# stckvrflw/pem-spgemm

Hardware: AMD Instinct MI355X
Metric: SpGEMM GFLOP/s (2*flop / t(step1+step2+step3)) (higher is better)
Workload: dtype f64

## Files before the change

### include/pem_spgemm.h

```cpp
#ifndef PEM_SPGEMM_H
#define PEM_SPGEMM_H
#include <stdint.h>

#ifdef __cplusplus
extern "C" {
#endif

typedef int pem_status;
enum {
    PEM_OK = 0,
    PEM_E_INVALID = -1,
    PEM_E_DUPLICATE = -2,
    PEM_E_NOMEM = -3,
    PEM_E_OVERFLOW = -4,
    PEM_E_HIP = -5,
    PEM_E_STATE = -6,
    PEM_E_NODEVICE = -7,
    PEM_E_IO = -8,
    PEM_E_STALE = -9
};

typedef struct pem_ctx pem_ctx;
typedef struct pem_tiled pem_tiled;
typedef struct pem_cplan pem_cplan;
// ... 80 lines not shown

pem_status pem_cplan_create(pem_ctx *ctx, const pem_tiled *A, const pem_tiled *B,
                            int32_t tile_row_begin, int32_t tile_row_end, pem_cplan **out);
pem_status pem_cplan_destroy(pem_ctx *ctx, pem_cplan *plan);

typedef enum { PEM_MASK_STRUCTURE = 0, PEM_MASK_COMPLEMENT = 1 } pem_mask_flags;
pem_status pem_cplan_create_masked(pem_ctx *ctx, const pem_tiled *A, const pem_tiled *B, const pem_tiled *M, int mask_flags,
                                   int32_t tile_row_begin, int32_t tile_row_end, pem_cplan **out);

typedef enum {
    PEM_SEMIRING_PLUS_TIMES = 0,
    PEM_SEMIRING_MIN_PLUS = 1,
    PEM_SEMIRING_MAX_PLUS = 2,
    PEM_SEMIRING_MAX_TIMES = 3,
    PEM_SEMIRING_PLUS_PAIR = 4,
    PEM_SEMIRING_LOR_LAND = 5
} pem_semiring;
pem_status pem_cplan_set_semiring(pem_cplan *plan, int semiring);
pem_status pem_cplan_get_semiring(const pem_cplan *plan, int *semiring);

pem_status pem_tiled_from_cplan(pem_ctx *ctx, const pem_cplan *plan, int transpose, pem_tiled **out);
pem_status pem_tiled_set_values_from_cplan(pem_ctx *ctx, pem_tiled *t, const pem_cplan *plan);

typedef enum { PEM_EWISE_UNION = 0, PEM_EWISE_INTERSECT = 1 } pem_ewise_pattern;
typedef enum {
    PEM_BINOP_PLUS = 0,
    PEM_BINOP_TIMES = 1,
    PEM_BINOP_MIN = 2,
    PEM_BINOP_MAX = 3,
    PEM_BINOP_LOR = 4,
    PEM_BINOP_LAND = 5
} pem_binop;
pem_status pem_tiled_ewise(pem_ctx *ctx, const pem_tiled *A, const pem_tiled *B, int pattern, int op, double alpha, double beta,
                           pem_tiled **out);
pem_status pem_tiled_set_values_from_ewise(pem_ctx *ctx, pem_tiled *t, const pem_tiled *A, const pem_tiled *B);

typedef enum {
    PEM_SELECT_TRIL = 0,
    PEM_SELECT_TRIU = 1,
    PEM_SELECT_DIAG = 2,
    PEM_SELECT_OFFDIAG = 3,
    PEM_SELECT_ROW_LE = 4,
    PEM_SELECT_ROW_GT = 5,
    PEM_SELECT_COL_LE = 6,
    PEM_SELECT_COL_GT = 7,
    PEM_SELECT_VALUE_EQ = 8, PEM_SELECT_VALUE_NE = 9, PEM_SELECT_VALUE_LT = 10,
    PEM_SELECT_VALUE_LE = 11, PEM_SELECT_VALUE_GT = 12, PEM_SELECT_VALUE_GE = 13,
    PEM_SELECT_ABS_GT = 14
} pem_select_op;
pem_status pem_tiled_select(pem_ctx *ctx, const pem_tiled *A, int op, double thunk, pem_tiled **out);
pem_status pem_tiled_set_values_from_select(pem_ctx *ctx, pem_tiled *t, const pem_tiled *A);

typedef enum { PEM_REDUCE_ROWS = 0, PEM_REDUCE_COLS = 1 } pem_reduce_dim;
pem_status pem_tiled_mxv(pem_ctx *ctx, const pem_tiled *A, int semiring, int transpose, const double *dx, double *dy, int accumulate);
pem_status pem_tiled_mxv_f32(pem_ctx *ctx, const pem_tiled *A, int semiring, int transpose, const float *dx, float *dy, int accumulate);
pem_status pem_tiled_reduce(pem_ctx *ctx, const pem_tiled *A, int op, int dim, double *dy, int accumulate);
pem_status pem_tiled_reduce_f32(pem_ctx *ctx, const pem_tiled *A, int op, int dim, float *dy, int accumulate);

pem_status pem_tiled_spmm(pem_ctx *ctx, const pem_tiled *A, int semiring, int transpose, int64_t k, const double *dX, int64_t ldx,
                          double *dY, int64_t ldy, int accumulate);
pem_status pem_tiled_spmm_f32(pem_ctx *ctx, const pem_tiled *A, int semiring, int transpose, int64_t k, const float *dX, int64_t ldx,
                              float *dY, int64_t ldy, int accumulate);

pem_status pem_tiled_set_values_sddmm(pem_ctx *ctx, pem_tiled *t, int semiring, int64_t k, const double *dX, int64_t ldx, const double *dY,
                                      int64_t ldy, int accumulate);
pem_status pem_tiled_set_values_sddmm_f32(pem_ctx *ctx, pem_tiled *t, int semiring, int64_t k, const float *dX, int64_t ldx, const float *dY,
                                          int64_t ldy, int accumulate);
pem_status pem_tiled_sddmm(pem_ctx *ctx, const pem_tiled *S, int semiring, int64_t k, const double *dX, int64_t ldx, const double *dY,
                           int64_t ldy, pem_tiled **out);
pem_status pem_tiled_sddmm_f32(pem_ctx *ctx, const pem_tiled *S, int semiring, int64_t k, const float *dX, int64_t ldx, const float *dY,
                               int64_t ldy, pem_tiled **out);

pem_status pem_tiled_export_csr(pem_ctx *ctx, const pem_tiled *t, int64_t *nnz, int32_t *rowptr, int32_t *colidx, double *vals);
pem_status pem_tiled_export_csr_f32(pem_ctx *ctx, const pem_tiled *t, int64_t *nnz, int32_t *rowptr, int32_t *colidx, float *vals);

typedef enum {
    PEM_OPT_PRUNE = 0,
    PEM_OPT_STEP1_GLOBAL_SORT = 1,
    PEM_OPT_WIDE = 2,
    PEM_OPT_WARM = 3,
    PEM_OPT_S3_BAND = 4,
    PEM_OPT_EXPORT_ROWS = 7,
    PEM_OPT__TEST_FIRST = 5,
    PEM_OPT__LAST = 18
} pem_option;
pem_status pem_cplan_set_option(pem_cplan *plan, pem_option which, int64_t value);
pem_status pem_cplan_get_option(const pem_cplan *plan, pem_option which, int64_t *value);

pem_status pem_spgemm_step1(pem_ctx *ctx, pem_cplan *plan);
pem_status pem_spgemm_step2(pem_ctx *ctx, pem_cplan *plan);
pem_status pem_spgemm_step3(pem_ctx *ctx, pem_cplan *plan);
pem_status pem_spgemm(pem_ctx *ctx, pem_cplan *plan);

typedef struct {
    int32_t tile_row_begin, tile_row_end;
    int32_t row_begin, row_end;
    int64_t ntiles_c;
    int64_t npairs;
    int64_t nnz_c;
    int64_t npairs_all;
} pem_cplan_info;
pem_status pem_cplan_get_info(const pem_cplan *plan, pem_cplan_info *info);

typedef enum {
    PEM_C_TILE_ROWPTR = 0,
    PEM_C_TILE_ROWIDX,
    PEM_C_TILE_COLIDX,
    PEM_C_PAIRS_OFFSET,
    PEM_C_PAIRS_A,
    PEM_C_PAIRS_B,
    PEM_C_MASK,
    PEM_C_TILE_NNZ_PTR,
    PEM_C_ROWPTR,
    PEM_C_ROWCOLIDX,
    PEM_C_VALS
} pem_cplan_array;
pem_status pem_cplan_get_array(pem_ctx *ctx, const pem_cplan *plan, pem_cplan_array which, void *host_dst, int64_t bytes);

pem_status pem_set_graph_replay(pem_ctx *ctx, int on);

pem_status pem_c_export_csr(pem_ctx *ctx, const pem_cplan *plan, int64_t *nnz, int32_t *rowptr,
                            int32_t *colidx, double *vals);
pem_status pem_c_export_csr_device(pem_ctx *ctx, const pem_cplan *plan, int32_t *d_rowptr,
                                   int32_t *d_colidx, double *d_vals);
pem_status pem_c_export_coo(pem_ctx *ctx, const pem_cplan *plan, int64_t *nnz, int32_t *rows,
                            int32_t *cols, double *vals);
pem_status pem_c_export_csr_f32(pem_ctx *ctx, const pem_cplan *plan, int64_t *nnz, int32_t *rowptr,
                                int32_t *colidx, float *vals);
pem_status pem_c_export_csr_device_f32(pem_ctx *ctx, const pem_cplan *plan, int32_t *d_rowptr,
                                       int32_t *d_colidx, float *d_vals);
pem_status pem_c_export_coo_f32(pem_ctx *ctx, const pem_cplan *plan, int64_t *nnz, int32_t *rows,
                                int32_t *cols, float *vals);

pem_status pem_split_tile_rows(pem_ctx *ctx, const pem_tiled *A, const pem_tiled *B, int nparts, int32_t *bounds);
pem_status pem_tile_row_weights(pem_ctx *ctx, const pem_tiled *A, const pem_tiled *B, double *weights);

typedef struct {
    double step1_ms, step2_ms, step3_ms;
    double spgemm_wall_ms;
    double export_ms;
} pem_timings;
pem_status pem_get_timings(pem_ctx *ctx, pem_timings *t);

pem_status pem_set_kernel_profiling(pem_ctx *ctx, int enabled);
pem_status pem_reset_kernel_stats(pem_ctx *ctx);
pem_status pem_kernel_stats_count(pem_ctx *ctx, int *n);
pem_status pem_kernel_stats_get(pem_ctx *ctx, int idx, char *name, int name_cap, int64_t *calls, double *total_ms);

#ifdef __cplusplus
}
#endif
#endif
```

### pem-spgemm_amd/__init__.py

```python
import ctypes as C
import os
import subprocess

import numpy as np

_HERE = os.path.dirname(os.path.abspath(__file__))
LIB_PATH = os.path.join(_HERE, "libpemspgemm_hip.so")

PEM_OK = 0
STATUS_NAMES = {0: "PEM_OK", -1: "PEM_E_INVALID", -2: "PEM_E_DUPLICATE", -3: "PEM_E_NOMEM", -4: "PEM_E_OVERFLOW",
                -5: "PEM_E_HIP", -6: "PEM_E_STATE", -7: "PEM_E_NODEVICE", -8: "PEM_E_IO", -9: "PEM_E_STALE"}

T_ARRAYS = dict(tile_keys=(0, np.int64), tile_nnz_ptr=(1, np.int32), masks=(2, np.uint16), rowptr=(3, np.uint8),
                rowcolidx=(4, np.uint8), vals=(5, np.float64), masks_t=(6, np.uint16), tile_rowptr=(7, np.int32),
                tile_colidx=(8, np.int32), tile_colptr=(9, np.int32), tile_rowidx=(10, np.int32), tile_offsets=(11, np.int32))
C_ARRAYS = dict(c_tile_rowptr=(0, np.int32), c_tile_rowidx=(1, np.int32), c_tile_colidx=(2, np.int32), pairs_offset=(3, np.int32),
                pairs_a=(4, np.int32), pairs_b=(5, np.int32), c_mask=(6, np.uint32), c_tile_nnz_ptr=(7, np.int32),
                c_rowptr=(8, np.uint8), c_rowcolidx=(9, np.uint8), c_vals=(10, np.float64))
C_TEST_ARRAYS = dict(c_mtile=(11, np.int32))

MASK_STRUCTURE, MASK_COMPLEMENT = 0, 1

SEMIRINGS = dict(plus_times=0, min_plus=1, max_plus=2, max_times=3, plus_pair=4, lor_land=5)

ABI_SYMBOLS = [
    "pem_last_error", "pem_version", "pem_ctx_create", "pem_ctx_create_on_stream", "pem_ctx_destroy", "pem_ctx_synchronize",
    "pem_tiled_from_coo", "pem_tiled_from_coo_device", "pem_tiled_from_csr", "pem_tiled_destroy", "pem_tiled_get_info",
    "pem_tiled_get_array", "pem_flop_count", "pem_cplan_create", "pem_cplan_destroy", "pem_spgemm_step1", "pem_spgemm_step2",
    "pem_spgemm_step3", "pem_spgemm", "pem_cplan_get_info", "pem_cplan_get_array", "pem_c_export_csr", "pem_c_export_csr_device",
    "pem_c_export_coo", "pem_split_tile_rows", "pem_tile_row_weights", "pem_get_timings", "pem_set_kernel_profiling", "pem_reset_kernel_stats",
    "pem_kernel_stats_count", "pem_kernel_stats_get", "pem_tiled_save", "pem_tiled_load",
    "pem_tiled_from_coo_f32", "pem_tiled_from_coo_device_f32", "pem_tiled_from_csr_f32", "pem_c_export_csr_f32",
    "pem_c_export_csr_device_f32", "pem_c_export_coo_f32", "pem_set_graph_replay",
    "pem_ctx_reserve", "pem_ctx_trim", "pem_ctx_memory_stats", "pem_cplan_set_option", "pem_cplan_get_option", "pem_debug_scan_i32",
    "pem_debug_refused_launch", "pem_tiled_set_values", "pem_tiled_set_values_device", "pem_tiled_set_values_f32",
    "pem_tiled_set_values_device_f32", "pem_cplan_create_masked", "pem_cplan_set_semiring", "pem_cplan_get_semiring",
    "pem_tiled_from_cplan", "pem_tiled_set_values_from_cplan", "pem_tiled_ewise", "pem_tiled_set_values_from_ewise",
    "pem_tiled_export_csr", "pem_tiled_export_csr_f32", "pem_tiled_select", "pem_tiled_set_values_from_select",
    "pem_tiled_mxv", "pem_tiled_mxv_f32", "pem_tiled_reduce", "pem_tiled_reduce_f32", "pem_tiled_spmm", "pem_tiled_spmm_f32",
    "pem_tiled_set_values_sddmm", "pem_tiled_set_values_sddmm_f32", "pem_tiled_sddmm", "pem_tiled_sddmm_f32",
]

EWISE_PATTERNS = dict(union=0, intersect=1)
BINOPS = dict(plus=0, times=1, min=2, max=3, lor=4, land=5)

SELECT_OPS = ("tril", "triu", "diag", "offdiag", "row_le", "row_gt", "col_le", "col_gt", "value_eq", "value_ne", "value_lt", "value_le",
              "value_gt", "value_ge", "abs_gt")
POSITIONAL_SELECT_OPS = SELECT_OPS[:8]

REDUCE_DIMS = dict(rows=0, cols=1)

VALUE_ORDERS = dict(row=0, col=1)

OPTIONS = dict(prune=0, step1_global_sort=1, wide=2, warm=3, s3_band=4, s1_force_key64=5, s1_xlcap=6, export_rows=7, s1_serial=8, s3_decode=9, s1_xl_global=10, s3_epw=11, s3_idx64=12, s3_mark=13, s3_xcd=14, s1_segments=15, s2_transposed=16, s3_poison=17)


class PemError(RuntimeError):
    def __init__(self, status, msg):
        super().__init__(f"{STATUS_NAMES.get(status, status)}: {msg}")
        self.status = status


class TiledInfo(C.Structure):
    _fields_ = [("rows", C.c_int32), ("cols", C.c_int32), ("nnz", C.c_int64), ("tile_rows", C.c_int32), ("tile_cols", C.c_int32),
                ("ntiles", C.c_int64), ("conv_ms", C.c_double), ("conv_tile_kernel_ms", C.c_double), ("value_bytes", C.c_int32),
                ("reserved", C.c_int32)]


class CPlanInfo(C.Structure):
    _fields_ = [("tile_row_begin", C.c_int32), ("tile_row_end", C.c_int32), ("row_begin", C.c_int32), ("row_end", C.c_int32),
                ("ntiles_c", C.c_int64), ("npairs", C.c_int64), ("nnz_c", C.c_int64), ("npairs_all", C.c_int64)]


class CacheKey(C.Structure):
    _fields_ = [("source_size", C.c_uint64), ("source_mtime_ns", C.c_int64), ("transpose", C.c_uint32), ("reserved", C.c_uint32)]

    @classmethod
    def of_file(cls, path, transpose=False):
        st = os.stat(path)
        return cls(st.st_size, st.st_mtime_ns, int(bool(transpose)), 0)


class MemoryStats(C.Structure):
    _fields_ = [("slab_bytes", C.c_int64), ("in_use_bytes", C.c_int64), ("peak_in_use_bytes", C.c_int64), ("largest_free_bytes", C.c_int64),
                ("driver_allocs", C.c_int64), ("block_allocs", C.c_int64)]


class Timings(C.Structure):
    _fields_ = [("step1_ms", C.c_double), ("step2_ms", C.c_double), ("step3_ms", C.c_double), ("spgemm_wall_ms", C.c_double),
                ("export_ms", C.c_double)]


def build(verbose=False):
    out = None if verbose else subprocess.DEVNULL
    subprocess.check_call(["make", "-C", os.path.join(_HERE, "csrc"), "-j4"], stdout=out)
    return LIB_PATH


_lib = None


def lib():
    global _lib
    if _lib is None:
        if not os.path.exists(LIB_PATH):
            raise ImportError(f"{LIB_PATH} is missing: run `python -c 'import __graft_entry__ as g; g.build()'` "
                              "(the product path has no CPU fallback)")
        L = C.CDLL(LIB_PATH)
        L.pem_last_error.restype = C.c_char_p
        L.pem_version.restype = C.c_char_p
        _lib = L
    return _lib


def _check(status):
    if status != PEM_OK:
        raise PemError(status, lib().pem_last_error().decode(errors="replace"))


def _p(a, ctype):
    return a.ctypes.data_as(C.POINTER(ctype))


class Context:

    def __init__(self, device=0, stream=None):
        self._h = C.c_void_p()
        _check(lib().pem_ctx_create_on_stream(int(device), C.c_void_p(stream or 0), C.byref(self._h)))
        self.device = device

    def synchronize(self):
        _check(lib().pem_ctx_synchronize(self._h))

    def timings(self):
        t = Timings()
        _check(lib().pem_get_timings(self._h, C.byref(t)))
        return {k: getattr(t, k) for k, _ in Timings._fields_}
# ... 406 lines not shown
```

### pem-spgemm_amd/csrc/pem_internal.h

```cpp
#pragma once
#include <hip/hip_runtime.h>
#include <atomic>
#include <cstdint>
#include <cstdio>
#include <cstring>
#include <initializer_list>
#include <map>
#include <memory>
#include <mutex>
#include <string>
#include <vector>
#include "../../include/pem_spgemm.h"
#include "../../include/pem_test.h"

namespace pem {

void set_error(const char *fmt, ...);

#define PEM_HIP(expr)                                                                          \
    do {                                                                                       \
        hipError_t _e = (expr);                                                                \
        if (_e != hipSuccess) {                                                                \
            pem::set_error("%s:%d: %s -> %s", __FILE__, __LINE__, #expr, hipGetErrorString(_e)); \
            return PEM_E_HIP;                                                                  \
// ... 243 lines not shown
    std::vector<int> h_tile_rowptr;
    pem::DevBuf vmap[2];
    pem::DevBuf vmap_t;
    bool vmap_ready[2] = {false, false}, vmap_t_ready = false;
    uint64_t value_version = 0;
    uint64_t serial = pem::next_tiled_serial();
    pem::Derivation derived;
    mutable pem::DevBuf mx_csc_off, mx_csc_base, mx_rci_t;
    mutable bool mx_cols_ready = false;
};

struct pem_cplan {
    const pem_tiled *A = nullptr, *B = nullptr;
    uint64_t serial = 0;
    const pem_tiled *M = nullptr;
    int mask_complement = 0;
    pem::DevBuf c_mtile;
    pem::DevBuf mf_tile_off, mf_tile_mt, mf_keep_t, mf_keep_p;
    pem::DevBuf mf_pair_col, mf_pairs_a, mf_pairs_b, mf_blk_heads;
    bool mf_swapped = false;
    int64_t w_Pm = 0, w_TCm = 0;
    int tr_lo = 0, tr_hi = 0;
    int a_lo = 0, a_hi = 0;
    int max_row_tiles = 0;
    int state = 0;
    int opt_prune = 1, opt_key64 = 0, opt_xlcap = 0;
    int opt_band = 1;
    int opt_step1_esc = 0, opt_wide = 1, opt_warm = 1, opt_export_rows = 0, opt_s1_serial = 0;
    int opt_xl_global = 0;
    int opt_idx64 = 0;
    int opt_mark = 1;
    int opt_s3_xcd = 1;
    int opt_epw = 0;
    int opt_decode = 1;
    int opt_s3_poison = 0;
    int64_t ntiles_c = 0, npairs = 0, nnz_c = 0;
    pem::DevBuf c_tile_rowptr, c_tile_colidx;
    mutable pem::DevBuf c_tile_rowidx;
    mutable bool c_rowidx_valid = false;
    pem::DevBuf pairs_offset, pairs_a, pairs_b;
    pem::DevBuf c_mask, c_tile_nnz_ptr, c_vals;
    mutable pem::DevBuf c_rowcolidx;
    mutable bool c_rowcolidx_valid = false;
    pem::DevBuf c_tile_cnt;
    bool s3_decode = false;
    pem::DevBuf s3_chunk_tile;
    mutable pem::DevBuf c_rowptr;
    mutable bool c_rowptr_valid = false;
    pem::DevBuf prod_a, prod_b, aprod_off;
    pem::DevBuf lprod_off;
    pem::DevBuf row_lbase;
    pem::DevBuf live_j, live_ab;
    pem::DevBuf aseg;
    pem::DevBuf chunk_seg, chunk_n;
    pem::DevBuf row_desc;
    int64_t w_ntotal = 0;
    int64_t npairs_all = 0;
    pem::DevBuf sk0, sk1, sv0, sv1;
    uint32_t *sorted_perm = nullptr;
    pem::DevBuf row_list, bin_count, xl_base, xl_rowstart;
    pem::DevBuf pair_col;
    pem::DevBuf blk_heads;
    bool pairs_ready = false;
    bool flags_mirrored = false;
    bool verify_folded = false;
    bool group_nnz_cleared = false;
    bool wide = true;
    bool compact_valid = false;
    pem::DevBuf group_nnz;
    uint64_t a_version = 0, b_version = 0;
    int semiring = 0;
    int c_semiring = 0;
    pem_ctx *owner = nullptr;
    hipGraphExec_t graph_exec = nullptr;
    unsigned long long graph_gen = 0;
    bool graph_failed = false;
    bool warm = false, warm_pass = false;
    int64_t w_P = 0, w_Pall = 0, w_TC = 0, w_nnz = 0;
    int w_counts[5] = {0, 0, 0, 0, 0};
    int w_nsegs = 0;
    pem::DevBuf seg_list;
    int opt_s2_transposed = 2;
    int opt_s1_segments = 0;
    int64_t w_nxl = 0;
    int w_nrows_xl = 0, w_max_xl = 0;
};
```

### pem-spgemm_amd/csrc/primitives.hip

```cpp
#include "pem_internal.h"
#include <algorithm>
#include <cstdarg>

namespace pem {

static thread_local char g_err[512] = "";
void set_error(const char *fmt, ...)
{
    va_list ap;
    va_start(ap, fmt);
    vsnprintf(g_err, sizeof g_err, fmt, ap);
    va_end(ap);
}
const char *last_error() { return g_err; }

std::shared_ptr<Arena> &current_arena()
{
    static thread_local std::shared_ptr<Arena> a;
    return a;
}

static constexpr size_t ARENA_ALIGN = 256;
static constexpr size_t ARENA_MIN_SLAB = size_t(64) << 20;
static constexpr size_t ARENA_MAX_GROWTH = size_t(4) << 30;

Arena::~Arena()
{
    (void)hipSetDevice(device);
    (void)hipDeviceSynchronize();
    for (auto &s : slabs) (void)hipFree(s.base);
}

pem_status Arena::add_slab(size_t bytes)
{
    void *p = nullptr;
    hipError_t e = hipMalloc(&p, bytes);
    if (e != hipSuccess) {
        (void)hipGetLastError();
        set_error("hipMalloc(%zu bytes) failed: %s (arena holds %zu bytes, %zu in use)", bytes, hipGetErrorString(e), slab_bytes, in_use);
        return PEM_E_NOMEM;
    }
    slabs.push_back(Slab{static_cast<char *>(p), bytes});
    slab_bytes += bytes;
    ++n_driver;
    free_blocks[static_cast<char *>(p)] = bytes;
    return PEM_OK;
}

void *Arena::take(size_t bytes)
{
    auto best = free_blocks.end();
    for (auto it = free_blocks.begin(); it != free_blocks.end(); ++it)
        if (it->second >= bytes && (best == free_blocks.end() || it->second < best->second)) best = it;
    if (best == free_blocks.end()) return nullptr;
    char *p = best->first;
    const size_t have = best->second;
    free_blocks.erase(best);
    if (have > bytes) free_blocks[p + bytes] = have - bytes;
    used_blocks[p] = bytes;
    in_use += bytes;
    if (in_use > peak) peak = in_use;
    ++n_block;
    return p;
}

void *Arena::alloc(size_t bytes)
{
    bytes = (bytes + ARENA_ALIGN - 1) & ~(ARENA_ALIGN - 1);
    if (bytes == 0) bytes = ARENA_ALIGN;
    std::lock_guard<std::mutex> lock(mu);
    if (void *p = take(bytes)) return p;
    size_t pad = slab_bytes / 2;
    if (pad > ARENA_MAX_GROWTH) pad = ARENA_MAX_GROWTH;
    size_t want = bytes + pad;
    if (want < ARENA_MIN_SLAB) want = ARENA_MIN_SLAB;
    if (add_slab(want) != PEM_OK) {
        if (want == bytes || add_slab(bytes) != PEM_OK) return nullptr;
    }
    return take(bytes);
}

void Arena::free(void *vp)
{
// ... 99 lines not shown
        ctx->event_pool.pop_back();
        return e;
    }
    hipEvent_t e = nullptr;
    (void)hipEventCreate(&e);
    return e;
}

KernelSpan::KernelSpan(pem_ctx *c, const char *name) : ctx(c)
{
    if (!ctx->profiling) return;
    for (size_t i = 0; i < ctx->stats.size(); ++i)
        if (ctx->stats[i].name == name) { stat = (int)i; break; }
    if (stat < 0) {
        ctx->stats.push_back(KernelStat{name, 0, 0.0});
        stat = (int)ctx->stats.size() - 1;
    }
    e0 = take_event(ctx);
    e1 = take_event(ctx);
    (void)hipEventRecord(e0, ctx->stream);
}
KernelSpan::~KernelSpan()
{
    if (stat < 0) return;
    (void)hipEventRecord(e1, ctx->stream);
    ctx->pending.push_back(PendingSpan{stat, e0, e1});
}

pem_status resolve_kernel_spans(pem_ctx *ctx)
{
    if (ctx->pending.empty()) return PEM_OK;
    PEM_HIP(hipStreamSynchronize(ctx->stream));
    for (auto &s : ctx->pending) {
        float ms = 0.f;
        if (hipEventElapsedTime(&ms, s.e0, s.e1) == hipSuccess) {
            ctx->stats[s.stat].calls += 1;
            ctx->stats[s.stat].total_ms += ms;
        }
        ctx->event_pool.push_back(s.e0);
        ctx->event_pool.push_back(s.e1);
    }
    ctx->pending.clear();
    return PEM_OK;
}

pem_status zero_flags(pem_ctx *ctx)
{
    PEM_HIP(hipMemsetAsync(ctx->d_flags, 0, sizeof(int) * NUM_FLAGS, ctx->stream));
    return PEM_OK;
}

pem_status launch_status(pem_ctx *ctx)
{
    if (ctx->launch_err == hipSuccess) return PEM_OK;
    set_error("kernel launch refused by the runtime: %s: %s", ctx->launch_name ? ctx->launch_name : "?", hipGetErrorString(ctx->launch_err));
    ctx->launch_err = hipSuccess;
    ctx->launch_name = nullptr;
    return PEM_E_HIP;
}

pem_status read_flags(pem_ctx *ctx, int *host_flags)
{
    PEM_TRY(launch_status(ctx));
    int *h = reinterpret_cast<int *>(ctx->h_scalars + 48);
    PEM_HIP(hipMemcpyAsync(h, ctx->d_flags, sizeof(int) * NUM_FLAGS, hipMemcpyDeviceToHost, ctx->stream));
    PEM_HIP(hipStreamSynchronize(ctx->stream));
    for (int i = 0; i < NUM_FLAGS; ++i) host_flags[i] = h[i];
    return PEM_OK;
}

pem_status read_scalars(pem_ctx *ctx, const int64_t *d_src, int count, int64_t *host_dst)
{
    PEM_HIP(hipMemcpyAsync(ctx->h_scalars, d_src, sizeof(int64_t) * count, hipMemcpyDeviceToHost, ctx->stream));
    PEM_HIP(hipStreamSynchronize(ctx->stream));
    for (int i = 0; i < count; ++i) host_dst[i] = ctx->h_scalars[i];
    return PEM_OK;
}

constexpr int SCAN_THREADS = 256;
constexpr int SCAN_TILE = SCAN_THREADS * 4;
constexpr int SCAN_TILES_PER_BLOCK = 8;
constexpr int SCAN_BLOCK_ITEMS = SCAN_TILE * SCAN_TILES_PER_BLOCK;

template <typename T> __device__ __forceinline__ T wave_inclusive_scan(T v)
{
    const int lane = threadIdx.x & 63;
#pragma unroll
    for (int d = 1; d < 64; d <<= 1) {
        T t = __shfl_up(v, d, 64);
        if (lane >= d) v += t;
    }
    return v;
}

template <typename T> __device__ __forceinline__ T wave_reduce_sum(T v)
{
#pragma unroll
    for (int d = 32; d > 0; d >>= 1) v += __shfl_xor(v, d, 64);
    return v;
}

__global__ void __launch_bounds__(SCAN_THREADS) scan_reduce_kernel(const int *__restrict__ in, size_t n,
                                                                   long long *__restrict__ bsum)
{
    __shared__ long long wsum[SCAN_THREADS / 64];
    size_t base = (size_t)blockIdx.x * SCAN_BLOCK_ITEMS;
    size_t end = base + SCAN_BLOCK_ITEMS < n ? base + SCAN_BLOCK_ITEMS : n;
    long long s = 0;
    if (end - base == (size_t)SCAN_BLOCK_ITEMS && (reinterpret_cast<uintptr_t>(in) & 15) == 0) {
        const int4 *in4 = reinterpret_cast<const int4 *>(in + base);
#pragma unroll
        for (int k = 0; k < SCAN_BLOCK_ITEMS / 4 / SCAN_THREADS; ++k) {
            const int4 q = in4[k * SCAN_THREADS + threadIdx.x];
            s += (long long)q.x + q.y + q.z + q.w;
        }
    } else {
        for (size_t i = base + threadIdx.x; i < end; i += SCAN_THREADS) s += in[i];
    }
    s = wave_reduce_sum(s);
    if ((threadIdx.x & 63) == 0) wsum[threadIdx.x >> 6] = s;
    __syncthreads();
    if (threadIdx.x == 0) {
        long long t = 0;
        for (int w = 0; w < SCAN_THREADS / 64; ++w) t += wsum[w];
        bsum[blockIdx.x] = t;
    }
}

__global__ void __launch_bounds__(1024) scan_bsums_kernel(long long *__restrict__ bsum, int nblk,
                                                          long long *__restrict__ total64, int *__restrict__ flags)
{
    __shared__ long long wsum[16];
    __shared__ long long carry_s;
    if (threadIdx.x == 0) carry_s = 0;
    __syncthreads();
    for (int base = 0; base < nblk; base += 1024) {
        int i = base + threadIdx.x;
        long long v = i < nblk ? bsum[i] : 0;
        long long inc = wave_inclusive_scan(v);
        if ((threadIdx.x & 63) == 63) wsum[threadIdx.x >> 6] = inc;
        __syncthreads();
        long long woff = 0;
        for (int w = 0; w < (int)(threadIdx.x >> 6); ++w) woff += wsum[w];
        long long carry = carry_s;
        if (i < nblk) bsum[i] = carry + woff + inc - v;
        __syncthreads();
        if (threadIdx.x == 1023) carry_s = carry + woff + inc;
        __syncthreads();
    }
    if (threadIdx.x == 0) {
        long long t = carry_s;
        bsum[nblk] = t;
        if (total64) *total64 = t;
        if (t > 0x7FFFFFFFLL) flags[FLAG_OVERFLOW] = 1;
    }
}

__global__ void __launch_bounds__(SCAN_THREADS) scan_apply_kernel(const int *in, int *out, size_t n,
                                                                  const long long *__restrict__ bsum, int nblk)
{
    __shared__ int wsum[SCAN_THREADS / 64];
    const int lane = threadIdx.x & 63, wave = threadIdx.x >> 6;
    long long carry = bsum[blockIdx.x];
    size_t base = (size_t)blockIdx.x * SCAN_BLOCK_ITEMS;
    for (int tile = 0; tile < SCAN_TILES_PER_BLOCK; ++tile, base += SCAN_TILE) {
        if (base >= n) break;
        size_t i0 = base + (size_t)threadIdx.x * 4;
        int v[4];
        if (i0 + 4 <= n) {
            int4 q = *reinterpret_cast<const int4 *>(in + i0);
            v[0] = q.x; v[1] = q.y; v[2] = q.z; v[3] = q.w;
        } else {
#pragma unroll
            for (int k = 0; k < 4; ++k) v[k] = (i0 + k < n) ? in[i0 + k] : 0;
        }
        int tsum = v[0] + v[1] + v[2] + v[3];
        int inc = wave_inclusive_scan(tsum);
        if (lane == 63) wsum[wave] = inc;
        __syncthreads();
        int woff = 0, btotal = 0;
#pragma unroll
        for (int w = 0; w < SCAN_THREADS / 64; ++w) {
            int s = wsum[w];
            if (w < wave) woff += s;
            btotal += s;
        }
        int ex = (int)carry + woff + inc - tsum;
        int o0 = ex, o1 = o0 + v[0], o2 = o1 + v[1], o3 = o2 + v[2];
        if (i0 + 4 <= n) {
            *reinterpret_cast<int4 *>(out + i0) = make_int4(o0, o1, o2, o3);
        } else {
            if (i0 < n) out[i0] = o0;
            if (i0 + 1 < n) out[i0 + 1] = o1;
            if (i0 + 2 < n) out[i0 + 2] = o2;
        }
        carry += btotal;
        __syncthreads();
    }
    if (blockIdx.x == nblk - 1 && threadIdx.x == 0) out[n] = (int)bsum[nblk];
}

__global__ void scan_empty_kernel(int *out, long long *total64)
{
    out[0] = 0;
    if (total64) *total64 = 0;
}

__global__ void __launch_bounds__(1024) scan_small_kernel(const int *in, int *out, size_t n, long long *__restrict__ total64,
                                                          int *__restrict__ flags)
{
    __shared__ long long wsum[16];
    const int lane = threadIdx.x & 63, wave = threadIdx.x >> 6;
    long long carry = 0;
    for (size_t base = 0; base < n; base += 8192) {
        const size_t i0 = base + (size_t)threadIdx.x * 8;
        int v[8];
        if (i0 + 8 <= n) {
            const int4 q0 = *reinterpret_cast<const int4 *>(in + i0), q1 = *reinterpret_cast<const int4 *>(in + i0 + 4);
            v[0] = q0.x; v[1] = q0.y; v[2] = q0.z; v[3] = q0.w;
            v[4] = q1.x; v[5] = q1.y; v[6] = q1.z; v[7] = q1.w;
        } else {
#pragma unroll
            for (int k = 0; k < 8; ++k) v[k] = (i0 + k < n) ? in[i0 + k] : 0;
        }
        long long tsum = 0;
#pragma unroll
        for (int k = 0; k < 8; ++k) tsum += v[k];
        const long long inc = wave_inclusive_scan(tsum);
        if (lane == 63) wsum[wave] = inc;
        __syncthreads();
        long long woff = 0, btotal = 0;
#pragma unroll
        for (int w = 0; w < 16; ++w) {
            const long long c = wsum[w];
            if (w < wave) woff += c;
            btotal += c;
        }
        int o[8];
        o[0] = (int)(carry + woff + inc - tsum);
#pragma unroll
        for (int k = 1; k < 8; ++k) o[k] = o[k - 1] + v[k - 1];
        if (i0 + 8 <= n) {
            *reinterpret_cast<int4 *>(out + i0) = make_int4(o[0], o[1], o[2], o[3]);
            *reinterpret_cast<int4 *>(out + i0 + 4) = make_int4(o[4], o[5], o[6], o[7]);
        } else {
#pragma unroll
            for (int k = 0; k < 8; ++k)
                if (i0 + k < n) out[i0 + k] = o[k];
        }
        carry += btotal;
        __syncthreads();
    }
    if (threadIdx.x == 0) {
        out[n] = (int)carry;
        if (total64) *total64 = carry;
        if (carry > 0x7FFFFFFFLL) flags[FLAG_OVERFLOW] = 1;
    }
}

constexpr int SCAN_MID_ITEMS = 2048, SCAN_MID_BLOCKS = 128;
constexpr unsigned long long SCAN_MID_VALID = 1ull << 63;

struct ScanMidArgs {
    const int *in[2];
    int *out[2];
    size_t n[2];
    long long *total64[2];
    int nblk[2];
};
__global__ void __launch_bounds__(256) scan_mid_kernel(ScanMidArgs args, unsigned long long *state_all, int *__restrict__ flags, int stall_ticket)
{
    __shared__ long long wsum[4];
    __shared__ long long s_excl;
    __shared__ int s_ticket;
    const int y = blockIdx.y;
    const int nblk = args.nblk[y];
    if ((int)blockIdx.x >= nblk) return;
    const int *in = args.in[y];
    int *out = args.out[y];
    const size_t n = args.n[y];
    long long *total64 = args.total64[y];
    unsigned long long *state = state_all + (size_t)y * (SCAN_MID_BLOCKS + 2);
    int *ctl = reinterpret_cast<int *>(state + SCAN_MID_BLOCKS);
    const int tid = threadIdx.x, lane = tid & 63, wave = tid >> 6;
    if (tid == 0) s_ticket = atomicAdd(&ctl[1], 1);
    __syncthreads();
    const int blk = s_ticket;
    const size_t i0 = (size_t)blk * SCAN_MID_ITEMS + (size_t)tid * 8;
    int v[8];
    if (i0 + 8 <= n) {
        const int4 q0 = *reinterpret_cast<const int4 *>(in + i0), q1 = *reinterpret_cast<const int4 *>(in + i0 + 4);
        v[0] = q0.x; v[1] = q0.y; v[2] = q0.z; v[3] = q0.w;
        v[4] = q1.x; v[5] = q1.y; v[6] = q1.z; v[7] = q1.w;
    } else {
#pragma unroll
        for (int k = 0; k < 8; ++k) v[k] = (i0 + k < n) ? in[i0 + k] : 0;
    }
    long long tsum = 0;
#pragma unroll
    for (int k = 0; k < 8; ++k) tsum += v[k];
    const long long inc = wave_inclusive_scan(tsum);
    if (lane == 63) wsum[wave] = inc;
    __syncthreads();
    long long woff = 0, btotal = 0;
#pragma unroll
    for (int w = 0; w < 4; ++w) {
        if (w < wave) woff += wsum[w];
        btotal += wsum[w];
    }
    if (wave == 0) {
        if (blk == stall_ticket)
            for (int k = 0; k < 50; ++k) __builtin_amdgcn_s_sleep(127);
        if (lane == 0) __hip_atomic_store(&state[blk], SCAN_MID_VALID | (unsigned long long)btotal, __ATOMIC_RELAXED, __HIP_MEMORY_SCOPE_AGENT);
        long long excl = 0;
        bool ok = false;
        for (long long polls = 0; polls < (1ll << 24) && !ok; ++polls) {
            const unsigned long long a = lane < blk ? __hip_atomic_load(&state[lane], __ATOMIC_RELAXED, __HIP_MEMORY_SCOPE_AGENT) : SCAN_MID_VALID;
            const unsigned long long b = 64 + lane < blk ? __hip_atomic_load(&state[64 + lane], __ATOMIC_RELAXED, __HIP_MEMORY_SCOPE_AGENT) : SCAN_MID_VALID;
            if (__ballot(!(a & SCAN_MID_VALID) || !(b & SCAN_MID_VALID)) == 0) {
                excl = wave_reduce_sum((long long)(a & ~SCAN_MID_VALID) + (long long)(b & ~SCAN_MID_VALID));
                ok = true;
            } else {
                __builtin_amdgcn_s_sleep(1);
            }
        }
        if (!ok && lane == 0) flags[FLAG_INTERNAL] = 1;
        if (lane == 0) s_excl = excl;
    }
    __syncthreads();
    const long long carry = s_excl;
    int o[8];
    o[0] = (int)(carry + woff + inc - tsum);
#pragma unroll
    for (int k = 1; k < 8; ++k) o[k] = o[k - 1] + v[k - 1];
    if (i0 + 8 <= n) {
        *reinterpret_cast<int4 *>(out + i0) = make_int4(o[0], o[1], o[2], o[3]);
        *reinterpret_cast<int4 *>(out + i0 + 4) = make_int4(o[4], o[5], o[6], o[7]);
    } else {
#pragma unroll
        for (int k = 0; k < 8; ++k)
            if (i0 + k < n) out[i0 + k] = o[k];
    }
    if (tid == 0) {
        if (blk == nblk - 1) {
            const long long total = carry + btotal;
            out[n] = (int)total;
            if (total64) *total64 = total;
            if (total > 0x7FFFFFFFLL) flags[FLAG_OVERFLOW] = 1;
        }
        if (atomicAdd(&ctl[0], 1) == nblk - 1) {
            for (int b = 0; b < nblk; ++b) __hip_atomic_store(&state[b], 0ull, __ATOMIC_RELAXED, __HIP_MEMORY_SCOPE_AGENT);
            __hip_atomic_store(&ctl[0], 0, __ATOMIC_RELAXED, __HIP_MEMORY_SCOPE_AGENT);
            __hip_atomic_store(&ctl[1], 0, __ATOMIC_RELAXED, __HIP_MEMORY_SCOPE_AGENT);
        }
    }
}

static pem_status scan_mid_state(pem_ctx *ctx)
{
    if (!ctx->scan_state.p) {
        PEM_TRY(ctx->scan_state.reserve(sizeof(unsigned long long) * 2 * (SCAN_MID_BLOCKS + 2)));
        PEM_HIP(hipMemsetAsync(ctx->scan_state.p, 0, sizeof(unsigned long long) * 2 * (SCAN_MID_BLOCKS + 2), ctx->stream));
    }
    return PEM_OK;
}

pem_status exclusive_scan_i32_two(pem_ctx *ctx, const int *in_a, int *out_a, size_t na, int64_t *d_total_a, const int *in_b, int *out_b, size_t nb,
                                  int64_t *d_total_b)
{
    auto mid = [](size_t n) { return n > 8192 && n <= (size_t)SCAN_MID_ITEMS * SCAN_MID_BLOCKS; };
    const bool aligned = !((reinterpret_cast<uintptr_t>(in_a) | reinterpret_cast<uintptr_t>(out_a) | reinterpret_cast<uintptr_t>(in_b) |
                            reinterpret_cast<uintptr_t>(out_b)) & 15);
    if (ctx->dbg_scan_force || !aligned || !mid(na) || !mid(nb)) {
        PEM_TRY(exclusive_scan_i32(ctx, in_a, out_a, na, d_total_a));
        return exclusive_scan_i32(ctx, in_b, out_b, nb, d_total_b);
    }
    PEM_TRY(scan_mid_state(ctx));
    ScanMidArgs a = {};
    a.in[0] = in_a;
    a.out[0] = out_a;
    a.n[0] = na;
    a.total64[0] = reinterpret_cast<long long *>(d_total_a);
    a.nblk[0] = (int)((na + SCAN_MID_ITEMS - 1) / SCAN_MID_ITEMS);
    a.in[1] = in_b;
    a.out[1] = out_b;
    a.n[1] = nb;
    a.total64[1] = reinterpret_cast<long long *>(d_total_b);
    a.nblk[1] = (int)((nb + SCAN_MID_ITEMS - 1) / SCAN_MID_ITEMS);
    PEM_LAUNCH(ctx, scan_mid_kernel, dim3((unsigned)std::max(a.nblk[0], a.nblk[1]), 2), 256, a, ctx->scan_state.as<unsigned long long>(), ctx->d_flags, -1);
    return PEM_OK;
}

pem_status exclusive_scan_i32(pem_ctx *ctx, const int *in, int *out, size_t n, int64_t *d_total64)
{
    if (n == 0) {
        PEM_LAUNCH(ctx, scan_empty_kernel, 1, 1, out, reinterpret_cast<long long *>(d_total64));
        return PEM_OK;
    }
    if ((reinterpret_cast<uintptr_t>(in) & 15) || (reinterpret_cast<uintptr_t>(out) & 15)) {
        set_error("exclusive_scan_i32: unaligned pointer");
        return PEM_E_INVALID;
    }
    const int force = ctx->dbg_scan_force;
    if (force == 2 && n > (size_t)SCAN_MID_ITEMS * SCAN_MID_BLOCKS) {
        set_error("exclusive_scan_i32: the chained scan takes at most %d items", SCAN_MID_ITEMS * SCAN_MID_BLOCKS);
        return PEM_E_INVALID;
    }
    if (force ? force == 1 : n <= 8192) {
        PEM_LAUNCH(ctx, scan_small_kernel, 1, 1024, in, out, n, reinterpret_cast<long long *>(d_total64), ctx->d_flags);
        return PEM_OK;
    }
    if (force ? force == 2 : n <= (size_t)SCAN_MID_ITEMS * SCAN_MID_BLOCKS) {
        PEM_TRY(scan_mid_state(ctx));
        ScanMidArgs a = {};
        a.in[0] = in;
        a.out[0] = out;
        a.n[0] = n;
        a.total64[0] = reinterpret_cast<long long *>(d_total64);
        a.nblk[0] = (int)((n + SCAN_MID_ITEMS - 1) / SCAN_MID_ITEMS);
        PEM_LAUNCH(ctx, scan_mid_kernel, (unsigned)a.nblk[0], 256, a, ctx->scan_state.as<unsigned long long>(), ctx->d_flags, ctx->dbg_scan_stall_ticket);
        return PEM_OK;
    }
    int nblk = (int)((n + SCAN_BLOCK_ITEMS - 1) / SCAN_BLOCK_ITEMS);
    PEM_TRY(ctx->scan_bsum.reserve(sizeof(long long) * ((size_t)nblk + 1)));
    long long *bsum = ctx->scan_bsum.as<long long>();
    PEM_LAUNCH(ctx, scan_reduce_kernel, nblk, SCAN_THREADS, in, n, bsum);
    PEM_LAUNCH(ctx, scan_bsums_kernel, 1, 1024, bsum, nblk, reinterpret_cast<long long *>(d_total64), ctx->d_flags);
    PEM_LAUNCH(ctx, scan_apply_kernel, nblk, SCAN_THREADS, in, out, n, bsum, nblk);
    return PEM_OK;
}

struct ScanPair {
    const int *in[2];
    int *out[2];
    long long *bsum[2];
    long long *total64[2];
};

__global__ void __launch_bounds__(SCAN_THREADS) scan2_reduce_kernel(ScanPair sp, size_t n)
{
    __shared__ long long wsum[SCAN_THREADS / 64];
    const int *in = sp.in[blockIdx.y];
    size_t base = (size_t)blockIdx.x * SCAN_BLOCK_ITEMS;
    size_t end = base + SCAN_BLOCK_ITEMS < n ? base + SCAN_BLOCK_ITEMS : n;
    long long s = 0;
// ... 323 lines not shown
```

### pem-spgemm_amd/csrc/spgemm.hip

```cpp
#include "spgemm_internal.h"

using namespace pem;

__global__ void warm_verify_kernel(const long long *__restrict__ d_scalars, const int *__restrict__ bin_count, WarmCheck wc, int *__restrict__ flags)
{
    warm_check(wc, d_scalars, bin_count, flags);
}

extern "C" pem_status pem_cplan_create(pem_ctx *ctx, const pem_tiled *A, const pem_tiled *B, int32_t tr_lo, int32_t tr_hi, pem_cplan **out)
{
    if (!ctx || !A || !B || !out) return PEM_E_INVALID;
    *out = nullptr;
    if (A->cols != B->rows) {
        set_error("pem_cplan_create: A is %d x %d but B is %d x %d", A->rows, A->cols, B->rows, B->cols);
        return PEM_E_INVALID;
    }
    if (A->value_bytes != B->value_bytes) {
        set_error("pem_cplan_create: A holds %s values, B %s; both operands must share one value type", A->value_bytes == 4 ? "fp32" : "fp64",
                  B->value_bytes == 4 ? "fp32" : "fp64");
        return PEM_E_INVALID;
    }
    if (tr_hi < 0) tr_hi = A->tile_rows;
    if (tr_lo < 0 || tr_lo > tr_hi || tr_hi > A->tile_rows) {
        set_error("pem_cplan_create: tile-row range [%d, %d) outside [0, %d]", tr_lo, tr_hi, A->tile_rows);
        return PEM_E_INVALID;
    }
    static std::atomic<uint64_t> s_plan_serial{0};
    pem_cplan *p = new pem_cplan();
    p->serial = ++s_plan_serial;
    p->owner = ctx;
    p->A = A;
    p->B = B;
    p->tr_lo = tr_lo;
    p->tr_hi = tr_hi;
    p->a_lo = A->h_tile_rowptr[(size_t)tr_lo];
    p->a_hi = A->h_tile_rowptr[(size_t)tr_hi];
    for (int i = tr_lo; i < tr_hi; ++i)
        p->max_row_tiles = std::max(p->max_row_tiles, A->h_tile_rowptr[(size_t)i + 1] - A->h_tile_rowptr[(size_t)i]);
    auto env_is = [](const char *name, const char *val) {
        const char *e = getenv(name);
        return e && !strcmp(e, val);
    };
    p->opt_prune = !env_is("PEM_PRUNE", "0");
    p->opt_key64 = env_is("PEM_S1_FORCE_KEY64", "1");
    {
        const char *e = getenv("PEM_S1_XLCAP");
        p->opt_xlcap = e ? atoi(e) : 0;
    }
    p->opt_band = !env_is("PEM_S3_BAND", "0");
    p->opt_step1_esc = env_is("PEM_STEP1", "esc");
    p->opt_wide = !env_is("PEM_WIDE", "0");
    p->opt_warm = !env_is("PEM_NO_WARM", "1");
    p->opt_export_rows = env_is("PEM_EXPORT", "rows");
    p->opt_s1_serial = getenv("PEM_S1_SERIAL") != nullptr;
    p->opt_decode = !env_is("PEM_S3_DECODE", "0");
    p->opt_xl_global = env_is("PEM_S1_XL_GLOBAL", "1");
    p->opt_s3_xcd = !env_is("PEM_S3_XCD", "0");
    p->opt_idx64 = env_is("PEM_S3_IDX64", "1");
    p->opt_mark = !env_is("PEM_S3_MARK", "0");
    p->opt_s1_segments = env_is("PEM_S1_SEGMENTS", "1");
    {
        const char *e = getenv("PEM_S3_EPW");
        p->opt_epw = e ? atoi(e) : 0;
    }
    *out = p;
    return PEM_OK;
}

extern "C" pem_status pem_cplan_create_masked(pem_ctx *ctx, const pem_tiled *A, const pem_tiled *B, const pem_tiled *M, int mask_flags, int32_t tr_lo,
                                              int32_t tr_hi, pem_cplan **out)
{
    if (!ctx || !A || !B || !out) return PEM_E_INVALID;
    *out = nullptr;
    if (!M) {
        set_error("pem_cplan_create_masked: the mask M is null");
        return PEM_E_INVALID;
    }
    if (mask_flags != PEM_MASK_STRUCTURE && mask_flags != PEM_MASK_COMPLEMENT) {
        set_error("pem_cplan_create_masked: unknown mask flags %d (PEM_MASK_STRUCTURE = 0 or PEM_MASK_COMPLEMENT = 1)", mask_flags);
        return PEM_E_INVALID;
    }
    PEM_TRY(pem_cplan_create(ctx, A, B, tr_lo, tr_hi, out));
    if (M->rows != A->rows || M->cols != B->cols) {
        set_error("pem_cplan_create_masked: M is %d x %d but C = A*B is %d x %d", M->rows, M->cols, A->rows, B->cols);
        delete *out;
        *out = nullptr;
        return PEM_E_INVALID;
    }
    pem_cplan *p = *out;
    p->M = M;
    p->mask_complement = mask_flags == PEM_MASK_COMPLEMENT;
    p->opt_step1_esc = 0;
    p->opt_wide = 1;
    return PEM_OK;
}

constexpr size_t S_RETIRE_MAX = 32;
void pem::retire_graph(pem_ctx *ctx, pem_cplan *plan)
{
    if (!plan->graph_exec) return;
    if (ctx && !ctx->dbg_destroy_graphs) {
        ctx->retired_graphs.push_back(plan->graph_exec);
        if (ctx->retired_graphs.size() >= S_RETIRE_MAX && !ctx->capturing) {
            (void)hipDeviceSynchronize();
            for (auto ge : ctx->retired_graphs) (void)hipGraphExecDestroy(ge);
            ctx->retired_graphs.clear();
        }
    } else {
        (void)hipGraphExecDestroy(plan->graph_exec);
    }
    plan->graph_exec = nullptr;
}

extern "C" pem_status pem_cplan_destroy(pem_ctx *ctx, pem_cplan *plan)
{
    if (ctx) {
        (void)hipSetDevice(ctx->device);
        (void)hipStreamSynchronize(ctx->stream);
    } else {
        (void)hipDeviceSynchronize();
    }
    if (plan) retire_graph(ctx, plan);
    delete plan;
    return PEM_OK;
}

extern "C" pem_status pem_cplan_get_info(const pem_cplan *p, pem_cplan_info *info)
{
    if (!p || !info) return PEM_E_INVALID;
    info->tile_row_begin = p->tr_lo;
    info->tile_row_end = p->tr_hi;
    info->row_begin = p->tr_lo * 16;
    info->row_end = p->tr_hi * 16 < p->A->rows ? p->tr_hi * 16 : p->A->rows;
    info->ntiles_c = p->ntiles_c;
    info->npairs = p->npairs;
    info->nnz_c = p->nnz_c;
    info->npairs_all = p->npairs_all;
    return PEM_OK;
}

static int *plan_option_slot(pem_cplan *p, pem_option which)
{
    switch ((int)which) {
    case PEM_OPT_PRUNE: return &p->opt_prune;
    case PEM_OPT_STEP1_GLOBAL_SORT: return &p->opt_step1_esc;
    case PEM_OPT_WIDE: return &p->opt_wide;
    case PEM_OPT_WARM: return &p->opt_warm;
    case PEM_OPT_S3_BAND: return &p->opt_band;
    case PEM_OPT_S1_FORCE_KEY64: return &p->opt_key64;
    case PEM_OPT_S1_XLCAP: return &p->opt_xlcap;
    case PEM_OPT_EXPORT_ROWS: return &p->opt_export_rows;
    case PEM_OPT_S1_SERIAL: return &p->opt_s1_serial;
    case PEM_OPT_S3_DECODE: return &p->opt_decode;
    case PEM_OPT_S1_XL_GLOBAL: return &p->opt_xl_global;
    case PEM_OPT_S3_EPW: return &p->opt_epw;
    case PEM_OPT_S3_XCD: return &p->opt_s3_xcd;
    case PEM_OPT_S3_IDX64: return &p->opt_idx64;
    case PEM_OPT_S3_MARK: return &p->opt_mark;
    case PEM_OPT_S1_SEGMENTS: return &p->opt_s1_segments;
    case PEM_OPT_S2_TRANSPOSED: return &p->opt_s2_transposed;
    case PEM_OPT_S3_POISON: return &p->opt_s3_poison;
    default: return nullptr;
    }
}

extern "C" pem_status pem_cplan_set_option(pem_cplan *plan, pem_option which, int64_t value)
{
    if (!plan) return PEM_E_INVALID;
    int *slot = plan_option_slot(plan, which);
    if (!slot || value < 0 || value > 0x7FFFFFFF) {
        set_error("pem_cplan_set_option: unknown option %d or value %lld out of range", (int)which, (long long)value);
        return PEM_E_INVALID;
    }
    if (plan->M && ((which == PEM_OPT_STEP1_GLOBAL_SORT && value != 0) || (which == PEM_OPT_WIDE && value == 0))) {
        set_error("pem_cplan_set_option: a masked plan runs the row-local step 1 and the fused step 2 (%s = %lld refused)",
                  which == PEM_OPT_WIDE ? "PEM_OPT_WIDE" : "PEM_OPT_STEP1_GLOBAL_SORT", (long long)value);
        return PEM_E_INVALID;
    }
    const int v = (which == PEM_OPT_S1_XLCAP || which == PEM_OPT_S3_EPW || which == PEM_OPT_S2_TRANSPOSED || which == PEM_OPT_S3_POISON) ? (int)value : (value != 0);
    if (*slot == v) return PEM_OK;
    *slot = v;
    plan->warm = false;
    int keep = 3;
    switch ((int)which) {
    case PEM_OPT_PRUNE: case PEM_OPT_STEP1_GLOBAL_SORT: case PEM_OPT_S1_FORCE_KEY64: case PEM_OPT_S1_XLCAP: case PEM_OPT_S1_XL_GLOBAL:
    case PEM_OPT_S1_SEGMENTS: keep = 0; break;
    case PEM_OPT_WIDE: case PEM_OPT_S3_DECODE: case PEM_OPT_S2_TRANSPOSED: keep = 1; break;
    case PEM_OPT_S3_BAND: case PEM_OPT_S3_EPW: case PEM_OPT_S3_IDX64: case PEM_OPT_S3_MARK: case PEM_OPT_S3_XCD:
    case PEM_OPT_S3_POISON: keep = 2; break;
    default: break;
    }
    if (plan->state > keep) plan->state = keep;
    if (keep == 0) {
        plan->pairs_ready = false;
        plan->compact_valid = plan->c_rowidx_valid = false;
    }
    if (keep <= 1) plan->c_rowptr_valid = plan->c_rowcolidx_valid = false;
    if (plan->graph_exec) {
        retire_graph(plan->owner, plan);
    }
    plan->graph_failed = false;
    return PEM_OK;
}

extern "C" pem_status pem_cplan_set_semiring(pem_cplan *plan, int semiring)
{
    if (!plan) return PEM_E_INVALID;
    if (semiring < PEM_SEMIRING_PLUS_TIMES || semiring > PEM_SEMIRING_LOR_LAND) {
        set_error("pem_cplan_set_semiring: unknown semiring %d (PEM_SEMIRING_PLUS_TIMES = 0 .. PEM_SEMIRING_LOR_LAND = 5)", semiring);
        return PEM_E_INVALID;
    }
    if (plan->semiring == semiring) return PEM_OK;
    plan->semiring = semiring;
    if (plan->graph_exec) retire_graph(plan->owner, plan);
    plan->graph_failed = false;
    return PEM_OK;
}

extern "C" pem_status pem_cplan_get_semiring(const pem_cplan *plan, int *semiring)
{
    if (!plan || !semiring) return PEM_E_INVALID;
    *semiring = plan->semiring;
    return PEM_OK;
}

extern "C" pem_status pem_cplan_get_option(const pem_cplan *plan, pem_option which, int64_t *value)
{
    if (!plan || !value) return PEM_E_INVALID;
    const int *slot = plan_option_slot(const_cast<pem_cplan *>(plan), which);
    if (!slot) {
        set_error("pem_cplan_get_option: unknown option %d", (int)which);
        return PEM_E_INVALID;
    }
    *value = *slot;
    return PEM_OK;
}

pem_status pem::check_internal(const int *hf)
{
    if (!hf[FLAG_INTERNAL]) return PEM_OK;
    set_error("internal: a device scan ran out of its poll budget; the pass's results are not valid");
    return PEM_E_HIP;
}

pem_status pem::step_elapsed(pem_ctx *ctx, int e0, int e1, double *dst)
{
    float ms = 0.f;
    PEM_HIP(hipEventElapsedTime(&ms, ctx->ev[e0], ctx->ev[e1]));
    *dst = ms;
    return PEM_OK;
}

extern "C" pem_status pem_spgemm_step1(pem_ctx *ctx, pem_cplan *plan)
{
    if (!ctx || !plan) return PEM_E_INVALID;
    PEM_ENTER(ctx);
    PEM_TRY(step1_impl(ctx, plan, false));
    PEM_TRY(ensure_compact(ctx, plan));
    PEM_HIP(hipStreamSynchronize(ctx->stream));
    PEM_TRY(launch_status(ctx));
    return step_elapsed(ctx, 0, 1, &ctx->timings.step1_ms);
}

extern "C" pem_status pem_spgemm_step2(pem_ctx *ctx, pem_cplan *plan)
{
    if (!ctx || !plan) return PEM_E_INVALID;
    PEM_ENTER(ctx);
    plan->warm_pass = false;
    PEM_TRY(step2_impl(ctx, plan));
    PEM_HIP(hipStreamSynchronize(ctx->stream));
    PEM_TRY(launch_status(ctx));
    return step_elapsed(ctx, 2, 3, &ctx->timings.step2_ms);
}

extern "C" pem_status pem_spgemm_step3(pem_ctx *ctx, pem_cplan *plan)
{
// ... 188 lines not shown
```

### pem-spgemm_amd/csrc/spgemm_internal.h

```cpp
#pragma once
#include "pem_internal.h"
#include <algorithm>
#include <chrono>

namespace pem {

constexpr int S3_CHUNK = 256;
constexpr int S2_GROUP = 256;

enum { BC_BIN0 = 0, BC_XL_ROWS = 5, BC_XL_TOTAL = 6, BC_XL_MAX = 7, BC_SEGS = 8 , BC_FAULT = 9, BC_BUMP = 10 , BC_INTS = 16 };

struct WarmCheck {
    int on;
    long long P, Pall, TC, nnz, nxl;
    int c[5];
    int nsegs;    int *host_flags;
    int masked;
    long long Pm, TCm;
};
__device__ __forceinline__ void warm_check(const WarmCheck &w, const long long *__restrict__ d_scalars, const int *__restrict__ bin_count,
                                           int *__restrict__ flags)
{
    if (d_scalars[0] != w.P || d_scalars[1] != w.TC || d_scalars[2] != w.nnz || d_scalars[3] != w.Pall || bin_count[0] != w.c[0] ||
        bin_count[1] != w.c[1] || bin_count[2] != w.c[2] || bin_count[3] != w.c[3] || bin_count[4] != w.c[4] || bin_count[BC_XL_TOTAL] != w.nxl || bin_count[BC_SEGS] != w.nsegs)
        flags[FLAG_CAPACITY] = 1;
    if (w.masked && (d_scalars[4] != w.Pm || d_scalars[5] != w.TCm)) flags[FLAG_CAPACITY] = 1;
    if (w.host_flags) {
        for (int i = 0; i < NUM_FLAGS; ++i) w.host_flags[i] = flags[i];
    }
}

inline WarmCheck warm_check_of(const pem_cplan *p)
{
    return WarmCheck{1, p->w_P, p->w_Pall, p->w_TC, p->w_nnz, p->w_nxl, {p->w_counts[0], p->w_counts[1], p->w_counts[2], p->w_counts[3], p->w_counts[4]},
                     p->w_nsegs, nullptr, p->M != nullptr, p->w_Pm, p->w_TCm};
}

__device__ __forceinline__ double pem_fma(double a, double b, double c) { return __builtin_fma(a, b, c); }
__device__ __forceinline__ float pem_fma(float a, float b, float c) { return __builtin_fmaf(a, b, c); }

template <typename VT> __device__ __forceinline__ VT pem_inf() { return sizeof(VT) == 8 ? (VT)__builtin_huge_val() : (VT)__builtin_huge_valf(); }
template <typename VT> __device__ __forceinline__ VT pem_fmin(VT x, VT y) { if constexpr (sizeof(VT) == 8) return __builtin_fmin(x, y); else return __builtin_fminf(x, y); }
template <typename VT> __device__ __forceinline__ VT pem_fmax(VT x, VT y) { if constexpr (sizeof(VT) == 8) return __builtin_fmax(x, y); else return __builtin_fmaxf(x, y); }
struct SrPlusTimes {
    static constexpr bool vals = true;
    template <typename VT> static __device__ __forceinline__ VT start() { return VT(0); }
    template <typename VT> static __device__ __forceinline__ VT combine(VT a, VT b, VT acc) { return pem_fma(a, b, acc); }
};
struct SrMinPlus {
    static constexpr bool vals = true;
    template <typename VT> static __device__ __forceinline__ VT start() { return pem_inf<VT>(); }
    template <typename VT> static __device__ __forceinline__ VT combine(VT a, VT b, VT acc) { return pem_fmin(acc, a + b); }
};
struct SrMaxPlus {
    static constexpr bool vals = true;
    template <typename VT> static __device__ __forceinline__ VT start() { return -pem_inf<VT>(); }
    template <typename VT> static __device__ __forceinline__ VT combine(VT a, VT b, VT acc) { return pem_fmax(acc, a + b); }
};
struct SrMaxTimes {
    static constexpr bool vals = true;
    template <typename VT> static __device__ __forceinline__ VT start() { return -pem_inf<VT>(); }
    template <typename VT> static __device__ __forceinline__ VT combine(VT a, VT b, VT acc) { return pem_fmax(acc, a * b); }
};
struct SrPlusPair {
    static constexpr bool vals = false;
    template <typename VT> static __device__ __forceinline__ VT start() { return VT(0); }
    template <typename VT> static __device__ __forceinline__ VT combine(VT, VT, VT acc) { return acc + VT(1); }
    template <typename VT> static __device__ __forceinline__ VT count(unsigned m, VT acc) { return acc + VT(__popc(m)); }
};
struct SrLorLand {
    static constexpr bool vals = true;
    template <typename VT> static __device__ __forceinline__ VT start() { return VT(0); }
    template <typename VT> static __device__ __forceinline__ VT combine(VT a, VT b, VT acc) { return (a != VT(0) && b != VT(0)) ? VT(1) : acc; }
};

pem_status step_elapsed(pem_ctx *ctx, int e0, int e1, double *dst);
void retire_graph(pem_ctx *ctx, pem_cplan *plan);
pem_status step1_impl(pem_ctx *ctx, pem_cplan *p, bool allow_warm);
pem_status step2_impl(pem_ctx *ctx, pem_cplan *p);
pem_status step3_impl(pem_ctx *ctx, pem_cplan *p);
void mask_restore_lists(pem_cplan *p);
pem_status mask_filter(pem_ctx *ctx, pem_cplan *p, int64_t *P, int64_t *TC);
pem_status ensure_compact(pem_ctx *ctx, const pem_cplan *cp);
pem_status ensure_c_rowidx(pem_ctx *ctx, const pem_cplan *p);
pem_status ensure_c_rowptr(pem_ctx *ctx, const pem_cplan *p);
pem_status ensure_c_rowcolidx(pem_ctx *ctx, const pem_cplan *cp);

inline pem_status c_values_current(const pem_cplan *p, const char *fn)
{
    if (p->c_semiring != p->semiring) {
        set_error("%s: the plan's semiring was changed (pem_cplan_set_semiring) after C was computed; run pem_spgemm_step3 or pem_spgemm first", fn);
        return PEM_E_STATE;
    }
    if (p->a_version == p->A->value_version && p->b_version == p->B->value_version) return PEM_OK;
    set_error("%s: the values of %s were refreshed (pem_tiled_set_values) after C was computed; run pem_spgemm_step3 or pem_spgemm first", fn,
              p->a_version != p->A->value_version ? "A" : "B");
    return PEM_E_STATE;
}
inline void note_c_values(pem_cplan *p)
{
    p->a_version = p->A->value_version;
    p->b_version = p->B->value_version;
    p->c_semiring = p->semiring;
}

}
```

### pem-spgemm_amd/csrc/step1.hip

```cpp
#include "spgemm_internal.h"

using namespace pem;

__global__ void __launch_bounds__(256) s1_aprod_kernel(const int *__restrict__ a_tile_colidx, const uint32_t *__restrict__ a_occ, int a_lo,
                                                       int nA, const int *__restrict__ b_tile_rowptr, const uint32_t *__restrict__ b_occ,
                                                       int prune, int *__restrict__ aprod, int *__restrict__ lprod)
{
    constexpr int G = 8;
    const int arel = (blockIdx.x * blockDim.x + threadIdx.x) / G;
    const int l = threadIdx.x & (G - 1);
    const bool in = arel < nA;
    int len = 0, cnt = 0;
    if (in) {
        const int k = a_tile_colidx[a_lo + arel];
        const int b0 = b_tile_rowptr[k];
        len = b_tile_rowptr[k + 1] - b0;
        if (prune) {
            const unsigned acol = a_occ[a_lo + arel] & 0xFFFFu;
#pragma unroll 4
            for (int q = l; q < len; q += G) cnt += (acol & (b_occ[b0 + q] >> 16)) != 0;
        }
    }
#pragma unroll
    for (int d = G / 2; d > 0; d >>= 1) cnt += __shfl_xor(cnt, d, G);
    if (!prune) cnt = len;
    if (in && l == 0) {
        aprod[arel] = len;
        lprod[arel] = cnt;
    }
}

__global__ void __launch_bounds__(256) s1_esc_expand_kernel(const long long *__restrict__ a_tile_keys, const uint32_t *__restrict__ a_occ, int a_lo,
                                                            int nA, int tr_lo, const int *__restrict__ lprod_off,
                                                            const int *__restrict__ b_tile_rowptr, const int *__restrict__ b_tile_colidx,
                                                            const uint32_t *__restrict__ b_occ, int prune, int bits_tc,
                                                            uint64_t *__restrict__ keys, uint32_t *__restrict__ perm, int *__restrict__ prod_a,
                                                            int *__restrict__ prod_b)
{
    const int arel = (blockIdx.x * blockDim.x + threadIdx.x) >> 4;
    const bool in = arel < nA;
    const int l = threadIdx.x & 15, grp = (threadIdx.x & 63) >> 4;
    int a = 0, i = 0, x0 = 0, b0 = 0, len = 0;
    unsigned acol = 0xFFFFu;
    if (in) {
        a = a_lo + arel;
        const long long ak = a_tile_keys[a];
        i = (int)(ak >> 32) - tr_lo;
        const int k = (int)(ak & 0xFFFFFFFFll);
        x0 = lprod_off[arel];
        b0 = b_tile_rowptr[k];
        len = b_tile_rowptr[k + 1] - b0;
        if (prune) acol = a_occ[a] & 0xFFFFu;
    }
    int maxlen = len;
#pragma unroll
    for (int d = 32; d > 0; d >>= 1) {
        const int o = __shfl_xor(maxlen, d, 64);
        maxlen = o > maxlen ? o : maxlen;
    }
    const uint64_t hi = (uint64_t)(unsigned)i << bits_tc;
    int run = 0;
    for (int q0 = 0; q0 < maxlen; q0 += 16) {
        const int q = q0 + l;
        const bool live = q < len && (!prune || (acol & (b_occ[b0 + q] >> 16)) != 0);
        const unsigned m16 = (unsigned)(__ballot(live) >> (16 * grp)) & 0xFFFFu;
        if (live) {
            const int x = x0 + run + __popc(m16 & ((1u << l) - 1u));
            keys[x] = hi | (uint64_t)(unsigned)b_tile_colidx[b0 + q];
            perm[x] = (uint32_t)x;
            prod_a[x] = a;
            prod_b[x] = b0 + q;
        }
        run += __popc(m16);
    }
}

__global__ void s1_heads_kernel(const uint64_t *__restrict__ keys, size_t n, int *__restrict__ head)
{
    size_t p = (size_t)blockIdx.x * blockDim.x + threadIdx.x;
    if (p >= n) return;
    head[p] = (p == 0) || (keys[p] != keys[p - 1]);
}

__global__ void s1_emit_ctiles_kernel(const uint64_t *__restrict__ keys, const int *__restrict__ headx, size_t n, int tr_lo, int bits_tc,
                                      int *__restrict__ c_rowidx, int *__restrict__ c_colidx, int *__restrict__ pairs_offset)
{
    size_t p = (size_t)blockIdx.x * blockDim.x + threadIdx.x;
    if (p >= n) return;
    int t = headx[p];
    if (headx[p + 1] != t) {
        uint64_t k = keys[p];
        c_rowidx[t] = (int)(k >> bits_tc) + tr_lo;
        c_colidx[t] = (int)(k & ((1ull << bits_tc) - 1ull));
        pairs_offset[t] = (int)p;
    }
    if (p == n - 1) pairs_offset[headx[n]] = (int)n;
}

__global__ void s1_c_rowptr_kernel(const int *__restrict__ c_rowidx, long long ntc, int tr_lo, int mt, int *__restrict__ c_rowptr)
{
    long long t = (long long)blockIdx.x * blockDim.x + threadIdx.x;
    if (t >= ntc) return;
    int tr = c_rowidx[t] - tr_lo;
    int prev = t > 0 ? c_rowidx[t - 1] - tr_lo : -1;
    for (int row = prev + 1; row <= tr; ++row) c_rowptr[row] = (int)t;
    if (t == ntc - 1)
        for (int row = tr + 1; row <= mt; ++row) c_rowptr[row] = (int)ntc;
}

constexpr int S1_CH = 512;
constexpr int S1_XW = 8;
constexpr int S1_XU = 4;
constexpr int S1_XTRIPS = 2048;
constexpr unsigned S1_SENT = 0xFFFFFFFFu;
constexpr int S1_CAP0 = 64, S1_CAP1 = 512, S1_CAP2 = 2048, S1_CAP3 = 8192, S1_CAP4 = 32768;
constexpr int S1_QB0 = 6, S1_QB1 = 9, S1_QB2 = 11, S1_QB3 = 13, S1_QB4 = 15;
constexpr int S1_NLIST = 6;
constexpr int S1_PC1 = 64, S1_PC2 = 256, S1_PC3 = 1024;
constexpr int S1_SEG_T = 1024;
constexpr int S1_XLL_MAX = 1 << 18;

__global__ void __launch_bounds__(256) s1_total_kernel(const int *__restrict__ a_tile_colidx, int a_lo, int nA, const int *__restrict__ b_tile_rowptr,
                                                       unsigned long long *__restrict__ total)
{
    const int arel = blockIdx.x * blockDim.x + threadIdx.x;
    long long len = 0;
    if (arel < nA) {
        const int k = a_tile_colidx[a_lo + arel];
        len = b_tile_rowptr[k + 1] - b_tile_rowptr[k];
    }
#pragma unroll
    for (int d = 32; d > 0; d >>= 1) len += __shfl_xor(len, d, 64);
    __shared__ long long wsum[4];
    if ((threadIdx.x & 63) == 0) wsum[threadIdx.x >> 6] = len;
    __syncthreads();
    if (threadIdx.x == 0) {
        const long long s = wsum[0] + wsum[1] + wsum[2] + wsum[3];
        if (s) atomicAdd(total, (unsigned long long)s);
    }
}

#ifdef PEM_S1_DEBUG
__device__ unsigned long long g_k1dbg[32768][8];
extern "C" void pem_debug_k1(unsigned long long *out) { (void)hipMemcpyFromSymbol(out, HIP_SYMBOL(g_k1dbg), sizeof(unsigned long long) * 32768 * 8); }
#endif

__device__ __forceinline__ int s1_wave_inclusive_scan_dpp(int v)
{
    v += __builtin_amdgcn_update_dpp(0, v, 0x111, 0xF, 0xF, true);
    v += __builtin_amdgcn_update_dpp(0, v, 0x112, 0xF, 0xF, true);
    v += __builtin_amdgcn_update_dpp(0, v, 0x114, 0xF, 0xF, true);
    v += __builtin_amdgcn_update_dpp(0, v, 0x118, 0xF, 0xF, true);
    v += __builtin_amdgcn_update_dpp(0, v, 0x142, 0xA, 0xF, false);
    v += __builtin_amdgcn_update_dpp(0, v, 0x143, 0xC, 0xF, false);
    return v;
}

__global__ void __launch_bounds__(64 * S1_XW, 8) s1_expand_kernel(const int *__restrict__ a_tile_colidx, const uint32_t *__restrict__ a_occ, int a_lo, int nA,
                                                               const int *__restrict__ b_tile_rowptr, const int2 *__restrict__ b_colocc, int prune,
                                                               int *__restrict__ bin_count, unsigned long long cap, int2 *__restrict__ aseg,
                                                               int2 *__restrict__ chunk_seg, long long *__restrict__ chunk_n, int *__restrict__ lj,
                                                               int2 *__restrict__ lab, int *__restrict__ flags, long long *__restrict__ scalars)
{
    static_assert(S1_CH == 64 * S1_XW, "one thread per A tile of the chunk");
    __shared__ unsigned t_end[S1_CH];
    __shared__ uint2 t_pay[S1_CH];
    __shared__ unsigned t_hist[S1_XW][64 * S1_XU];
    __shared__ unsigned long long t_bal[S1_XTRIPS];
    __shared__ unsigned t_cum[S1_XTRIPS + 1];
    __shared__ unsigned s_wsum[S1_XW];
    __shared__ unsigned long long s_base;
    const int tid = threadIdx.x, lane = tid & 63, wave = tid >> 6;
    const int c = (int)blockIdx.x;
    if (c == 0) {
        if (tid < NUM_FLAGS) flags[tid] = 0;
        if (tid < BC_FAULT) bin_count[tid] = 0;
        if (tid < 4) scalars[tid] = 0;
    }
#ifdef PEM_S1_DEBUG
    const unsigned long long dbg0 = wall_clock64();
#endif
    const int arel = c * S1_CH + tid;
    const bool in = arel < nA;
    int b0 = 0;
    unsigned len = 0, acol = 0xFFFFu;
    if (in) {
        const unsigned ao = a_occ[a_lo + arel];
        const int k = a_tile_colidx[a_lo + arel];
        b0 = b_tile_rowptr[k];
        len = (unsigned)(b_tile_rowptr[k + 1] - b0);
        if (prune) acol = ao & 0xFFFFu;
    }
    unsigned inc = len;
#pragma unroll
    for (int d = 1; d < 64; d <<= 1) {
        const unsigned o = (unsigned)__shfl_up((int)inc, d, 64);
        if (lane >= d) inc += o;
    }
    if (lane == 63) s_wsum[wave] = inc;
    __syncthreads();
    unsigned wpre = 0, N_b = 0;
#pragma unroll
// ... 64 lines not shown
            int2 co[S1_XU];
#pragma unroll
            for (int u = 0; u < S1_XU; ++u) co[u] = b_colocc[qb0 + 64u * (unsigned)u + (unsigned)lane < N_run ? bb[u] : 0];
            unsigned long long bal[S1_XU];
            int cnt[S1_XU];
#pragma unroll
            for (int u = 0; u < S1_XU; ++u) {
                const bool live = qb0 + 64u * (unsigned)u + (unsigned)lane < N_run && (!prune || (ac[u] & ((unsigned)co[u].y >> 16)) != 0);
                bal[u] = __ballot(live);
                cnt[u] = __popcll(bal[u]);
            }
#ifdef PEM_S1_DEBUG
            const unsigned long long dt2 = wall_clock64();
#endif
            unsigned before = 0;
            if (lane == 0) {
                while ((before = __hip_atomic_load(&t_cum[S1_XU * k], __ATOMIC_ACQUIRE, __HIP_MEMORY_SCOPE_WORKGROUP)) == S1_SENT) __builtin_amdgcn_s_sleep(1);
                unsigned run = before;
#pragma unroll
                for (int u = 0; u < S1_XU; ++u) {
                    if (S1_XU * k + u < ntr) {
                        t_bal[S1_XU * k + u] = bal[u];
                        run += (unsigned)cnt[u];
                        __hip_atomic_store(&t_cum[S1_XU * k + u + 1], run, __ATOMIC_RELEASE, __HIP_MEMORY_SCOPE_WORKGROUP);
                    }
                }
            }
            before = (unsigned)__builtin_amdgcn_readfirstlane((int)before);
#ifdef PEM_S1_DEBUG
            const unsigned long long dt3 = wall_clock64();
#endif
            unsigned x0 = base + before;
#pragma unroll
            for (int u = 0; u < S1_XU; ++u) {
                if ((bal[u] >> lane) & 1ull) {
                    const unsigned x = x0 + (unsigned)__popcll(bal[u] & lt);
                    lj[x] = co[u].x;
                    lab[x] = make_int2(a_lo + c * S1_CH + aa[u], bb[u]);
                }
                x0 += (unsigned)cnt[u];
            }
#ifdef PEM_S1_DEBUG
            if (lane == 0 && c < 32768) {
                const unsigned long long dt4 = wall_clock64();
                atomicAdd(&g_k1dbg[c][4], dt1 - dt0);
                atomicAdd(&g_k1dbg[c][5], dt2 - dt1);
                atomicAdd(&g_k1dbg[c][6], dt3 - dt2);
                atomicAdd(&g_k1dbg[c][7], dt4 - dt3);
            }
#endif
        }
        __syncthreads();
        const unsigned e1 = e0 + 64u * (unsigned)ntr;
        auto lp = [&](unsigned x) {
            const unsigned r = (x - e0) >> 6, o = (x - e0) & 63u;
            return t_cum[r] + (o ? (unsigned)__popcll(t_bal[r] & ((1ull << o) - 1ull)) : 0u);
        };
        const bool last_epoch = e1 >= N_run;
        if (st_a >= e0 && (st_a < e1 || (last_epoch && st_a == e1))) my_pos = lp(st_a < e1 ? st_a : e1);
        {
            const unsigned lo = st_a > e0 ? st_a : e0, hi = en_a < e1 ? en_a : e1;
            if (hi > lo) my_cnt += lp(hi) - lp(lo);
        }
        carry = t_cum[ntr];
        __syncthreads();
    }
    if (st_a > N_run) my_pos = carry;
    if (N_run == 0) my_pos = 0;
    if (in) aseg[arel] = make_int2((int)(base + my_pos), (int)my_cnt);
    if (tid == 0) {
        chunk_seg[c] = make_int2((int)base, (int)carry);
        chunk_n[c] = (long long)N_b;
#ifdef PEM_S1_DEBUG
        if (c < 32768) {
            g_k1dbg[c][0] = dbg0;
            g_k1dbg[c][1] = dbg1;
            g_k1dbg[c][2] = wall_clock64();
            g_k1dbg[c][3] = (unsigned long long)N_b;
        }
#endif
    }
}

__global__ void __launch_bounds__(256) s1_rowclass_kernel(const int *__restrict__ a_tile_rowptr, int tr_lo, int a_lo, int mt, int nchunks,
                                                          const int2 *__restrict__ aseg, const int2 *__restrict__ chunk_seg,
                                                          const long long *__restrict__ chunk_n, int tiny_ok, int cap4, int xlcap,
                                                          int *__restrict__ row_l, int4 *__restrict__ row_desc, int *__restrict__ row_list,
                                                          int *__restrict__ bin_count, int *__restrict__ xl_base, int *__restrict__ row_tc,
                                                          long long *__restrict__ scalars, int *__restrict__ flags, int *__restrict__ pairs_offset,
                                                          int *__restrict__ group_nnz, int ngroups, int *__restrict__ blk_heads, int nblk,
                                                          int seg_on, int2 *__restrict__ seg_list)
{
    const int i = blockIdx.x * blockDim.x + threadIdx.x;
    const int lane = threadIdx.x & 63;
    const unsigned long long lt = (1ull << lane) - 1ull;
    int nl = 0, np = 0;
    if (i < mt) {
        const int ra0 = a_tile_rowptr[tr_lo + i] - a_lo, ra1 = a_tile_rowptr[tr_lo + i + 1] - a_lo;
        unsigned pos0 = 0, pos1 = 0;
        int cnt0 = 0;
        if (ra1 > ra0) {
            const int c0 = ra0 / S1_CH, c1 = (ra1 - 1) / S1_CH;
            np = c1 - c0 + 1;
            const int2 f0 = aseg[ra0];
            pos0 = (unsigned)f0.x;
            if (np == 1) {
                const int2 e = aseg[ra1 - 1];
                cnt0 = (int)((unsigned)e.x + (unsigned)e.y - pos0);
                nl = cnt0;
            } else {
                const int2 e0 = aseg[c0 * S1_CH + S1_CH - 1], f1 = aseg[c1 * S1_CH], e1 = aseg[ra1 - 1];
                cnt0 = (int)((unsigned)e0.x + (unsigned)e0.y - pos0);
                pos1 = (unsigned)f1.x;
                long long tot = (long long)cnt0 + (long long)((unsigned)e1.x + (unsigned)e1.y - pos1);
                for (int c = c0 + 1; c < c1; ++c) tot += chunk_seg[c].y;
                nl = tot > 0x7FFFFFFFll ? 0x7FFFFFFF : (int)tot;
            }
        }
        row_l[i] = nl;
        row_desc[i] = make_int4((int)pos0, cnt0, (int)pos1, nl);
        xl_base[i] = -1;
        row_tc[i] = 0;
    }
    int bin = -1;
    if (nl > 0) {
        bin = 5;
        if (nl <= S1_CAP0 && np <= 2 && tiny_ok) bin = 0;
        else if (nl <= S1_CAP1 && np <= S1_PC1) bin = 1;
        else if (nl <= S1_CAP2 && np <= S1_PC2) bin = 2;
        else if (nl <= S1_CAP3 && np <= S1_PC3) bin = 3;
        else if (nl <= cap4 && np <= S1_PC3) bin = 4;
        if (seg_on && bin >= 4) bin = (nl <= S1_XLL_MAX && np <= S1_PC2) ? 4 : 5;
        if (nl > xlcap) bin = 5;
        if (seg_on && bin == 4) {
            const int G = (nl + S1_SEG_T - 1) / S1_SEG_T;
            const int s0 = atomicAdd(&bin_count[BC_SEGS], G);
            for (int g = 0; g < G; ++g) seg_list[s0 + g] = make_int2(i, g | (G << 16));
        }
    }
    __shared__ int blk_cnt[S1_NLIST], blk_base[S1_NLIST];
    __shared__ long long blk_all;
    if (threadIdx.x < S1_NLIST) blk_cnt[threadIdx.x] = 0;
    if (threadIdx.x == 0) blk_all = 0;
    __syncthreads();
    int wbase = 0, rank = 0;
#pragma unroll
    for (int b = 0; b < S1_NLIST; ++b) {
        const unsigned long long m = __ballot(bin == b);
        if (m == 0) continue;
        const int leader = __builtin_ctzll(m);
        int base = 0;
        if (lane == leader) base = atomicAdd(&blk_cnt[b], __popcll(m));
        base = __shfl(base, leader, 64);
        if (bin == b) {
            wbase = base;
            rank = __popcll(m & lt);
        }
    }
    {
        long long wn = i < nchunks ? chunk_n[i] : 0;
#pragma unroll
        for (int d = 32; d > 0; d >>= 1) wn += __shfl_xor(wn, d, 64);
        if (lane == 0 && wn) atomicAdd(reinterpret_cast<unsigned long long *>(&blk_all), (unsigned long long)wn);
    }
    __syncthreads();
    if (threadIdx.x < S1_NLIST) blk_base[threadIdx.x] = blk_cnt[threadIdx.x] ? atomicAdd(&bin_count[threadIdx.x], blk_cnt[threadIdx.x]) : 0;
    if (threadIdx.x == 0 && blk_all) atomicAdd(reinterpret_cast<unsigned long long *>(&scalars[3]), (unsigned long long)blk_all);
    __syncthreads();
    if (bin >= 0) row_list[(size_t)bin * mt + blk_base[bin] + wbase + rank] = i;
    if (bin == 5) {
        xl_base[i] = atomicAdd(&bin_count[BC_XL_TOTAL], nl);
        atomicMax(&bin_count[BC_XL_MAX], nl);
    }
    for (int g = i; g < ngroups; g += gridDim.x * blockDim.x) group_nnz[g] = 0;
    for (int g = i; g < nblk; g += gridDim.x * blockDim.x) blk_heads[g] = 0;
    if (i == 0) {
        pairs_offset[0] = 0;
        row_tc[mt] = 0;
        if (bin_count[BC_FAULT]) flags[FLAG_CAPACITY] = 1;
        bin_count[BC_FAULT] = 0;
        *reinterpret_cast<unsigned long long *>(bin_count + BC_BUMP) = 0ull;
    }
}

__device__ __forceinline__ int s1_find_a(const int *__restrict__ off, int lo, int hi, int x)
{
    while (hi - lo > 1) {
        int mid = (lo + hi) >> 1;
        if (off[mid] <= x) lo = mid; else hi = mid;
    }
    return lo;
}

template <typename KeyT> __device__ __forceinline__ KeyT s1_shfl_xor(KeyT v, int mask);
template <> __device__ __forceinline__ uint32_t s1_shfl_xor<uint32_t>(uint32_t v, int mask) { return (uint32_t)__shfl_xor((int)v, mask, 64); }
template <> __device__ __forceinline__ uint64_t s1_shfl_xor<uint64_t>(uint64_t v, int mask)
{
    return (uint64_t)__shfl_xor((unsigned long long)v, mask, 64);
}

template <typename KeyT, int THREADS, int EPT, int LOGT>
__device__ __forceinline__ void s1_bitonic_regs(KeyT (&v)[EPT], KeyT *lds, const int tid, const bool reverse = false)
{
    constexpr int LOGE = EPT == 1 ? 0 : EPT == 2 ? 1 : EPT == 4 ? 2 : EPT == 8 ? 3 : EPT == 16 ? 4 : 5;
    constexpr int LOGNP = LOGT + LOGE;
#pragma unroll
    for (int lk = 1; lk <= LOGNP; ++lk) {
        const int kk = 1 << lk;
#pragma unroll
        for (int lj = lk - 1; lj >= 0; --lj) {
            const int jj = 1 << lj;
            if (lj < LOGE) {
#pragma unroll
                for (int m = 0; m < EPT; ++m) {
                    if ((m & jj) == 0) {
                        const int m2 = m | jj;
                        const bool up = (((tid << LOGE) | m) & kk) == 0;
                        const KeyT x = v[m], y = v[m2];
                        const bool sw = (x > y) == up;
                        v[m] = sw ? y : x;
                        v[m2] = sw ? x : y;
                    }
                }
            } else if (lj < LOGE + 6) {
                const int lm = jj >> LOGE;
                const bool lower = (tid & lm) == 0;
                KeyT pv[EPT];
#pragma unroll
                for (int m = 0; m < EPT; ++m) pv[m] = s1_shfl_xor<KeyT>(v[m], lm);
#pragma unroll
                for (int m = 0; m < EPT; ++m) {
                    const bool up = (((tid << LOGE) | m) & kk) == 0;
                    v[m] = ((v[m] < pv[m]) == (lower == up)) ? v[m] : pv[m];
                }
            } else {
                const int tm = jj >> LOGE;
                const bool lower = (tid & tm) == 0;
#pragma unroll
                for (int m = 0; m < EPT; ++m) lds[m * THREADS + tid] = v[m];
                __syncthreads();
#pragma unroll
                for (int m = 0; m < EPT; ++m) {
                    const KeyT pv = lds[m * THREADS + (tid ^ tm)];
                    const bool up = (((tid << LOGE) | m) & kk) == 0;
                    v[m] = ((v[m] < pv) == (lower == up)) ? v[m] : pv;
                }
                __syncthreads();
            }
        }
    }
#pragma unroll
    for (int m = 0; m < EPT; ++m) lds[reverse ? (THREADS * EPT - 1 - ((tid << LOGE) | m)) : ((tid << LOGE) | m)] = v[m];
    __syncthreads();
}
__device__ __forceinline__ void s1_note_heads(int *__restrict__ blk_heads, const long long p0, const unsigned long long bal)
{
    if (!bal) return;
    const long long b0 = p0 >> 8;
    const int k = (int)(((b0 + 1) << 8) - p0);
    const unsigned long long m0 = k >= 64 ? ~0ull : (1ull << k) - 1ull;
    const int c0 = __popcll(bal & m0), c1 = __popcll(bal & ~m0);
    if (c0) atomicAdd(&blk_heads[b0], c0);
    if (c1) atomicAdd(&blk_heads[b0 + 1], c1);
}

__global__ void __launch_bounds__(256) s1_tiny_kernel(const int *__restrict__ row_list, int nrows_bin, const int4 *__restrict__ row_desc,
                                                      const int *__restrict__ row_lbase, const int *__restrict__ lj, const int2 *__restrict__ lab,
                                                      int *__restrict__ pairs_a, int *__restrict__ pairs_b, int *__restrict__ pair_col,
                                                      int *__restrict__ blk_heads, int *__restrict__ row_tc)
{
    const int lane = threadIdx.x & 63;
    const int li = (int)((blockIdx.x * blockDim.x + threadIdx.x) >> 6);
    if (li >= nrows_bin) return;
    const int i = __builtin_amdgcn_readfirstlane(row_list[li]);
    const int4 d = row_desc[i];
    const int lp0 = row_lbase[i], nl = d.w;
    const bool valid = lane < nl;
    unsigned key = 0xFFFFFFFFu;
    int2 ab = make_int2(0, 0);
    if (valid) {
        const unsigned src = lane < d.y ? (unsigned)d.x + (unsigned)lane : (unsigned)d.z + (unsigned)(lane - d.y);
        key = ((unsigned)lj[src] << S1_QB0) | (unsigned)lane;
        ab = lab[src];
    }
#pragma unroll
    for (int kk = 2; kk <= 64; kk <<= 1) {
#pragma unroll
        for (int jj = kk >> 1; jj > 0; jj >>= 1) {
            const unsigned o = (unsigned)__shfl_xor((int)key, jj, 64);
            const bool lower = (lane & jj) == 0, up = (lane & kk) == 0;
            key = ((key < o) == (lower == up)) ? key : o;
        }
    }
    const int j = (int)(key >> S1_QB0), from = (int)(key & 63u);
    const int a = __shfl(ab.x, from, 64), b = __shfl(ab.y, from, 64);
    const int jprev = __shfl_up(j, 1, 64);
    const bool head = valid && (lane == 0 || jprev != j);
    const unsigned long long bal = __ballot(head);
    if (valid) {
        pairs_a[lp0 + lane] = a;
        pairs_b[lp0 + lane] = b;
        pair_col[lp0 + lane] = j | (head ? (int)0x80000000 : 0);
    }
    if (lane == 0) {
        s1_note_heads(blk_heads, lp0, bal);
        row_tc[i] = __popcll(bal);
    }
}

template <typename KeyT, int CAP, int QB, int THREADS>
struct S1Row {
    KeyT *keys;
    static __device__ __forceinline__ unsigned long long match_digit(const bool valid, const unsigned d)
    {
        unsigned long long m = __ballot(valid);
#pragma unroll
        for (int b = 0; b < 8; ++b) {
            const bool bit = (d >> b) & 1u;
            const unsigned long long bal = __ballot(bit);
            m &= bit ? bal : ~bal;
        }
        return m;
    }
    template <int EPT> __device__ __forceinline__ void sort_radix(const int tid, const int n, unsigned *hist, int *wsum, const int first_bit,
                                                                  const int key_bits) const
    {
        static_assert(THREADS == 1024, "sized for 16 waves: 4096 counters, four per thread in the scan");
        constexpr int WAVES = THREADS / 64;
        const int lane = tid & 63, wave = tid >> 6;
        const unsigned long long lt = (1ull << lane) - 1ull;
        const int rpw = (n + THREADS - 1) / THREADS;
        const int e0 = wave * rpw * 64 + lane;
        unsigned *myhist = hist + wave * 256;
        for (int shift = first_bit; shift < key_bits; shift += 8) {
            for (int x = tid; x < WAVES * 256; x += THREADS) hist[x] = 0;
            __syncthreads();
#pragma unroll
            for (int r = 0; r < EPT; ++r) {
                const bool valid = r < rpw && e0 + r * 64 < n;
                const unsigned long long vm = __ballot(valid);
                if (vm != 0) {
                    const unsigned d = valid ? (unsigned)(keys[e0 + r * 64] >> shift) & 255u : 0u;
                    const unsigned d0 = (unsigned)__shfl((int)d, __builtin_ctzll(vm), 64);
                    if (__ballot(valid && d != d0) == 0) {
                        if (lane == 0) myhist[d0] += (unsigned)__popcll(vm);
                    } else if (valid) {
                        atomicAdd(&myhist[d], 1u);
                    }
                }
            }
            __syncthreads();
            {
                const int d = tid >> 2, w0 = (tid & 3) * 4;
                unsigned v[4];
#pragma unroll
                for (int j = 0; j < 4; ++j) v[j] = hist[(w0 + j) * 256 + d];
                const int tsum = (int)(v[0] + v[1] + v[2] + v[3]);
                int inc = tsum;
#pragma unroll
                for (int dd = 1; dd < 64; dd <<= 1) {
                    const int o = __shfl_up(inc, dd, 64);
                    if (lane >= dd) inc += o;
                }
                if (lane == 63) wsum[wave] = inc;
                __syncthreads();
                int ex = inc - tsum;
#pragma unroll
                for (int w = 0; w < WAVES; ++w)
                    if (w < wave) ex += wsum[w];
#pragma unroll
                for (int j = 0; j < 4; ++j) {
                    hist[(w0 + j) * 256 + d] = (unsigned)ex;
                    ex += (int)v[j];
                }
            }
            KeyT k[EPT];
#pragma unroll
            for (int r = 0; r < EPT; ++r) k[r] = (r < rpw && e0 + r * 64 < n) ? keys[e0 + r * 64] : KeyT(0);
            __syncthreads();
#pragma unroll
            for (int r = 0; r < EPT; ++r) {
                if (r < rpw) {
                    const bool valid = e0 + r * 64 < n;
                    const unsigned d = (unsigned)(k[r] >> shift) & 255u;
                    const unsigned long long m = match_digit(valid, d);
                    if (valid) {
                        const unsigned base = myhist[d];
                        const int rank = __popcll(m & lt);
                        keys[base + rank] = k[r];
                        if (rank == 0) myhist[d] = base + (unsigned)__popcll(m);
                    }
                }
                __builtin_amdgcn_sched_barrier(0);
            }
            __syncthreads();
        }
    }
    template <int EPT, int LOGT> __device__ __forceinline__ void sort_regs(const int tid) const
    {
        KeyT v[EPT];
#pragma unroll
        for (int m = 0; m < EPT; ++m) v[m] = keys[m * THREADS + tid];
        __syncthreads();
        s1_bitonic_regs<KeyT, THREADS, EPT, LOGT>(v, keys, tid);
    }
};

#ifdef PEM_S1_DEBUG
__device__ unsigned long long g_s1dbg[4][1024][8];
__device__ unsigned long long g_s1blk[4][1024][4];
extern "C" void pem_debug_s1_blocks(unsigned long long *out) { (void)hipMemcpyFromSymbol(out, HIP_SYMBOL(g_s1blk), sizeof(g_s1blk)); }
#define S1_DBG_MARK(k)                                                   \
    do {                                                                 \
        __syncthreads();                                                 \
        if (tid == 0) {                                                  \
            unsigned long long now = wall_clock64();                     \
            atomicAdd(&g_s1dbg[DBG_BIN][blockIdx.x & 1023][k], now - dbg_t); \
            dbg_t = now;                                                 \
        }                                                                \
    } while (0)
extern "C" void pem_debug_s1(unsigned long long *out32, int reset)
{
    static unsigned long long h[4][1024][8];
    if (reset) {
        memset(h, 0, sizeof(h));
        (void)hipMemcpyToSymbol(HIP_SYMBOL(g_s1dbg), h, sizeof(h));
    } else {
        (void)hipMemcpyFromSymbol(h, HIP_SYMBOL(g_s1dbg), sizeof(h));
        for (int b = 0; b < 4; ++b)
            for (int k = 0; k < 8; ++k) {
                unsigned long long acc = 0;
                for (int sl = 0; sl < 1024; ++sl) acc = k == 5 ? (h[b][sl][k] > acc ? h[b][sl][k] : acc) : acc + h[b][sl][k];
                out32[b * 8 + k] = acc;
            }
    }
}
#else
#define S1_DBG_MARK(k)
#endif

template <typename KeyT, int CAP, int QB, int THREADS>
__device__ __forceinline__ void s1_rowsort_row(KeyT *const keys, unsigned *const psrc, int *const pdst, int *const wsum, unsigned *const radix_hist,
                                               const int i, const int li, const int *__restrict__ a_tile_rowptr, const int tr_lo, const int a_lo,
                                               const int2 *__restrict__ aseg, const int *__restrict__ row_lbase, const int *__restrict__ lj,
                                               const int2 *__restrict__ lab, int *__restrict__ pairs_a, int *__restrict__ pairs_b,
                                               int *__restrict__ pair_col, int *__restrict__ blk_heads, int *__restrict__ row_tc, const int key_bits)
{
    constexpr int LOGT = THREADS == 64 ? 6 : THREADS == 256 ? 8 : 10;
    constexpr int EMAX = CAP / THREADS, WAVES = THREADS / 64;
    static_assert(EMAX == 8 || EMAX == 32, "a bin sorts up to 8 (or, for the largest, 32) keys per thread");
    static_assert(CAP <= (1 << QB), "the key's index field holds every position of the row's list");
    const int tid = threadIdx.x, lane = tid & 63, wave = tid >> 6;
    (void)li;
    (void)LOGT;
#ifdef PEM_S1_DEBUG
    constexpr int DBG_BIN = CAP == 512 ? 0 : CAP == 2048 ? 1 : CAP == 8192 ? 2 : 3;
    unsigned long long dbg_t = 0;
#endif
#ifdef PEM_S1_DEBUG
    if (tid == 0) dbg_t = wall_clock64();
    const unsigned long long dbg_row0 = dbg_t;
#endif
    const int ra0 = a_tile_rowptr[tr_lo + i] - a_lo, ra1 = a_tile_rowptr[tr_lo + i + 1] - a_lo;
    const int lp0 = row_lbase[i], nl = row_lbase[i + 1] - lp0;
    const int c0 = ra0 / S1_CH, np = (ra1 - 1) / S1_CH - c0 + 1;
    {
        unsigned src = 0;
        int cnt = 0;
        if (tid < np) {
            const int c = c0 + tid;
            const int first = ra0 > c * S1_CH ? ra0 : c * S1_CH, last = (ra1 < c * S1_CH + S1_CH ? ra1 : c * S1_CH + S1_CH) - 1;
            const int2 s = aseg[first], e = aseg[last];
            src = (unsigned)s.x;
            cnt = (int)((unsigned)e.x + (unsigned)e.y - src);
        }
        int inc = cnt;
#pragma unroll
        for (int d = 1; d < 64; d <<= 1) {
            const int o = __shfl_up(inc, d, 64);
            if (lane >= d) inc += o;
        }
        int ex = inc - cnt;
        if (THREADS > 64 && np > 64) {
            if (lane == 63) wsum[wave] = inc;
            __syncthreads();
#pragma unroll
            for (int w = 0; w < WAVES; ++w)
                if (w < wave) ex += wsum[w];
        }
        if (tid < np) {
            psrc[tid] = src;
            pdst[tid] = ex;
        }
        if (tid == 0) pdst[np] = nl;
    }
    __syncthreads();
    S1_DBG_MARK(0);
    for (int x0 = tid; x0 < nl; x0 += 4 * THREADS) {
        unsigned src[4];
#pragma unroll
        for (int u = 0; u < 4; ++u) {
            const int x = x0 + u * THREADS < nl ? x0 + u * THREADS : nl - 1;
            const int p = np == 1 ? 0 : s1_find_a(pdst, 0, np, x);
            src[u] = psrc[p] + (unsigned)(x - pdst[p]);
        }
        int jj[4];
#pragma unroll
        for (int u = 0; u < 4; ++u) jj[u] = lj[src[u]];
#pragma unroll
        for (int u = 0; u < 4; ++u)
            if (x0 + u * THREADS < nl) keys[x0 + u * THREADS] = (KeyT((unsigned)jj[u]) << QB) | KeyT(x0 + u * THREADS);
    }
    if constexpr (THREADS < 1024) {
        int upto = THREADS;
        while (upto < nl) upto <<= 1;
        for (int x = nl + tid; x < upto; x += THREADS) keys[x] = ~KeyT(0);
    }
    __syncthreads();
    S1_DBG_MARK(1);
    S1Row<KeyT, CAP, QB, THREADS> row;
    row.keys = keys;
    if constexpr (THREADS == 1024) {
        row.template sort_radix<EMAX>(tid, nl, radix_hist, wsum, QB, key_bits);
    } else if (nl <= THREADS)
        row.template sort_regs<1, LOGT>(tid);
    else if (nl <= THREADS * 2)
        row.template sort_regs<2, LOGT>(tid);
    else if (nl <= THREADS * 4)
        row.template sort_regs<4, LOGT>(tid);
    else
        row.template sort_regs<8, LOGT>(tid);
    S1_DBG_MARK(2);
    const int nseg = (nl + 63) >> 6;
    int mytiles = 0;

    for (int g0 = wave; g0 < nseg; g0 += 4 * WAVES) {
        int jv[4];
        int2 abv[4];
        bool hv[4];
#pragma unroll
        for (int u = 0; u < 4; ++u) {
            const int s = 64 * (g0 + u * WAVES) + lane;
            jv[u] = 0;
            abv[u] = make_int2(0, 0);
            hv[u] = false;
            if (s < nl) {
                const KeyT key = keys[s];
                const int idx = (int)(key & KeyT((1u << QB) - 1u));
                jv[u] = (int)(key >> QB);
                hv[u] = s == 0 || (int)(keys[s - 1] >> QB) != jv[u];
                const int p = np == 1 ? 0 : s1_find_a(pdst, 0, np, idx);
                abv[u] = lab[psrc[p] + (unsigned)(idx - pdst[p])];
            }
        }
#pragma unroll
        for (int u = 0; u < 4; ++u) {
            const int g = g0 + u * WAVES;
            if (g >= nseg) break;
            const int s = 64 * g + lane;
            const unsigned long long bal = __ballot(hv[u]);
            if (s < nl) {
                pairs_a[lp0 + s] = abv[u].x;
                pairs_b[lp0 + s] = abv[u].y;
                pair_col[lp0 + s] = jv[u] | (hv[u] ? (int)0x80000000 : 0);
            }
            if (lane == 0) {
                s1_note_heads(blk_heads, (long long)lp0 + 64 * g, bal);
                mytiles += __popcll(bal);
            }
        }
    }
    int base = mytiles;
    if constexpr (THREADS > 64) {
        if (lane == 0) wsum[wave] = mytiles;
        __syncthreads();
        base = 0;
#pragma unroll
        for (int w = 0; w < WAVES; ++w) base += wsum[w];
    }
    if (tid == 0) row_tc[i] = base;
    S1_DBG_MARK(3);
#ifdef PEM_S1_DEBUG
    if (tid == 0) {
        atomicAdd(&g_s1dbg[DBG_BIN][blockIdx.x & 1023][4], 1ull);
        atomicMax(&g_s1dbg[DBG_BIN][blockIdx.x & 1023][5], dbg_t - dbg_row0);
        if (li == (int)blockIdx.x && blockIdx.x < 1024) {
            unsigned hw, xcc;
            asm volatile("s_getreg_b32 %0, hwreg(HW_REG_HW_ID)" : "=s"(hw));
            asm volatile("s_getreg_b32 %0, hwreg(HW_REG_XCC_ID)" : "=s"(xcc));
            g_s1blk[DBG_BIN][blockIdx.x][0] = dbg_row0;
            g_s1blk[DBG_BIN][blockIdx.x][1] = dbg_t;
            g_s1blk[DBG_BIN][blockIdx.x][2] = hw;
            g_s1blk[DBG_BIN][blockIdx.x][3] = xcc;
        }
    }
#endif
    __syncthreads();
}

template <typename KeyT, int CAP, int QB, int THREADS>
__global__ void __launch_bounds__(THREADS, THREADS == 1024 ? (CAP > 8192 || sizeof(KeyT) == 8 ? 4 : 8) : (sizeof(KeyT) == 8 ? 1 : 8))
    s1_rowsort_kernel(const int *__restrict__ row_list, int nrows_bin, const int *__restrict__ a_tile_rowptr, int tr_lo, int a_lo,
                      const int2 *__restrict__ aseg, const int *__restrict__ row_lbase, const int *__restrict__ lj, const int2 *__restrict__ lab,
                      int *__restrict__ pairs_a, int *__restrict__ pairs_b, int *__restrict__ pair_col, int *__restrict__ blk_heads,
                      int *__restrict__ row_tc, int key_bits)
{
    __shared__ KeyT keys[CAP];
    __shared__ unsigned psrc[THREADS];
    __shared__ int pdst[THREADS + 1];
    __shared__ int wsum[THREADS / 64];
    __shared__ unsigned radix_hist[THREADS == 1024 ? (THREADS / 64) * 256 : 1];
    for (int li = blockIdx.x; li < nrows_bin; li += gridDim.x)
        s1_rowsort_row<KeyT, CAP, QB, THREADS>(keys, psrc, pdst, wsum, radix_hist, row_list[li], li, a_tile_rowptr, tr_lo, a_lo, aseg, row_lbase, lj, lab,
                                               pairs_a, pairs_b, pair_col, blk_heads, row_tc, key_bits);
}

__global__ void __launch_bounds__(1024, 4)
    s1_rowsort_big_kernel(const int *__restrict__ list4, int n4, const int *__restrict__ list3, int n3, const int *__restrict__ a_tile_rowptr, int tr_lo,
                          int a_lo, const int2 *__restrict__ aseg, const int *__restrict__ row_lbase, const int *__restrict__ lj,
                          const int2 *__restrict__ lab, int *__restrict__ pairs_a, int *__restrict__ pairs_b, int *__restrict__ pair_col,
                          int *__restrict__ blk_heads, int *__restrict__ row_tc, int key_bits4, int key_bits3)
{
    __shared__ uint32_t keys[S1_CAP4];
    __shared__ unsigned psrc[1024];
    __shared__ int pdst[1024 + 1];
    __shared__ int wsum[16];
    __shared__ unsigned radix_hist[16 * 256];
    const int b = blockIdx.x;
    if (b < n4)
        s1_rowsort_row<uint32_t, S1_CAP4, S1_QB4, 1024>(keys, psrc, pdst, wsum, radix_hist, list4[b], b, a_tile_rowptr, tr_lo, a_lo, aseg, row_lbase, lj, lab,
                                                        pairs_a, pairs_b, pair_col, blk_heads, row_tc, key_bits4);
    else if (b - n4 < n3)
        s1_rowsort_row<uint32_t, S1_CAP3, S1_QB3, 1024>(keys, psrc, pdst, wsum, radix_hist, list3[b - n4], b - n4, a_tile_rowptr, tr_lo, a_lo, aseg, row_lbase,
                                                        lj, lab, pairs_a, pairs_b, pair_col, blk_heads, row_tc, key_bits3);
}

template <typename KeyT>
__global__ void __launch_bounds__(1024) s1_rowseg_kernel(const int2 *__restrict__ seg_list, int nsegs, const int *__restrict__ a_tile_rowptr, int tr_lo,
                                                        int a_lo, const int2 *__restrict__ aseg, const int *__restrict__ row_lbase,
                                                        const int *__restrict__ lj, const int2 *__restrict__ lab, int tile_cols,
                                                        int *__restrict__ pairs_a, int *__restrict__ pairs_b, int *__restrict__ pair_col,
                                                        int *__restrict__ blk_heads, int *__restrict__ row_tc)
{
    constexpr int CAP = S1_CAP2, QB = S1_QB2, THREADS = 1024, WAVES = 16, LOGT = 10;
    __shared__ KeyT keys[CAP];
    __shared__ unsigned gidx[CAP];
    __shared__ unsigned psrc[S1_PC2];
    __shared__ int pdst[S1_PC2 + 1];
    __shared__ int wcnt[WAVES], wlow[WAVES], wsum[WAVES];
    const int tid = threadIdx.x, lane = tid & 63, wave = tid >> 6;
    const unsigned long long lt = (1ull << lane) - 1ull;
    for (int si = blockIdx.x; si < nsegs; si += gridDim.x) {
        const int2 sd = seg_list[si];
        const int i = sd.x, g = sd.y & 0xFFFF, G = sd.y >> 16;
        const int ra0 = a_tile_rowptr[tr_lo + i] - a_lo, ra1 = a_tile_rowptr[tr_lo + i + 1] - a_lo;
        const int lp0 = row_lbase[i], nl = row_lbase[i + 1] - lp0;
        const int c0 = ra0 / S1_CH, np = (ra1 - 1) / S1_CH - c0 + 1;
        {
            unsigned src = 0;
            int cnt = 0;
            if (tid < np) {
                const int c = c0 + tid;
                const int first = ra0 > c * S1_CH ? ra0 : c * S1_CH, last = (ra1 < c * S1_CH + S1_CH ? ra1 : c * S1_CH + S1_CH) - 1;
                const int2 s = aseg[first], e = aseg[last];
                src = (unsigned)s.x;
                cnt = (int)((unsigned)e.x + (unsigned)e.y - src);
            }
            int inc = cnt;
#pragma unroll
            for (int d = 1; d < 64; d <<= 1) {
                const int o = __shfl_up(inc, d, 64);
                if (lane >= d) inc += o;
            }
            int ex = inc - cnt;
            if (np > 64) {
                if (lane == 63) wsum[wave] = inc;
                __syncthreads();
#pragma unroll
                for (int w = 0; w < WAVES; ++w)
                    if (w < wave) ex += wsum[w];
            }
            if (tid < np) {
                psrc[tid] = src;
                pdst[tid] = ex;
            }
            if (tid == 0) pdst[np] = nl;
        }
        __syncthreads();
        auto list_src = [&](const int x) {
            const int p = np == 1 ? 0 : s1_find_a(pdst, 0, np, x);
            return psrc[p] + (unsigned)(x - pdst[p]);
        };
        const int per = (((nl + WAVES - 1) / WAVES) + 63) & ~63;
        const int x_lo = wave * per < nl ? wave * per : nl, x_hi = x_lo + per < nl ? x_lo + per : nl;
        int tiles = 0;
        const long long seg_lo = (long long)tile_cols * g / G, seg_hi = (long long)tile_cols * (g + 1) / G;
        long long r_lo = seg_lo, r_hi = seg_hi;
        while (r_lo < seg_hi) {
            int low = 0, cnt = 0;
            for (int x0 = x_lo; x0 < x_hi; x0 += 256) {
                int cc[4];
#pragma unroll
                for (int u = 0; u < 4; ++u) cc[u] = lj[list_src(x0 + 64 * u + lane < x_hi ? x0 + 64 * u + lane : x_lo)];
#pragma unroll
                for (int u = 0; u < 4; ++u) {
                    if (x0 + 64 * u + lane < x_hi) {
                        low += cc[u] < r_lo;
                        cnt += cc[u] >= r_lo && cc[u] < r_hi;
                    }
                }
            }
#pragma unroll
            for (int d = 32; d > 0; d >>= 1) {
                low += __shfl_xor(low, d, 64);
                cnt += __shfl_xor(cnt, d, 64);
            }
            __syncthreads();
            if (lane == 0) {
                wcnt[wave] = cnt;
                wlow[wave] = low;
            }
            __syncthreads();
            int below = 0, total = 0, wbase = 0;
#pragma unroll
            for (int w = 0; w < WAVES; ++w) {
                below += wlow[w];
                if (w < wave) wbase += wcnt[w];
                total += wcnt[w];
            }
            if (total > CAP && r_hi - r_lo > 1) {
                r_hi = r_lo + (r_hi - r_lo) / 2;
                continue;
            }
            if (total > 0) {
                const bool one_col = total > CAP;
                int run = wbase;
                for (int x0 = x_lo; x0 < x_hi; x0 += 256) {
                    unsigned ss[4];
                    int cc[4];
#pragma unroll
                    for (int u = 0; u < 4; ++u) ss[u] = list_src(x0 + 64 * u + lane < x_hi ? x0 + 64 * u + lane : x_lo);
#pragma unroll
                    for (int u = 0; u < 4; ++u) cc[u] = lj[ss[u]];
#pragma unroll
                    for (int u = 0; u < 4; ++u) {
                        const int x = x0 + 64 * u + lane;
                        const bool in = x < x_hi && cc[u] >= r_lo && cc[u] < r_hi;
                        const unsigned long long bal = __ballot(in);
                        if (in) {
                            const int pos = run + __popcll(bal & lt);
                            if (one_col) {
                                const int2 ab = lab[ss[u]];
                                const long long o = (long long)lp0 + below + pos;
                                pairs_a[o] = ab.x;
                                pairs_b[o] = ab.y;
                                pair_col[o] = cc[u] | (pos == 0 ? (int)0x80000000 : 0);
                            } else {
                                keys[pos] = (KeyT((unsigned)cc[u]) << QB) | KeyT(pos);
                                gidx[pos] = (unsigned)x;
                            }
                        }
                        run += __popcll(bal);
                    }
                }
                if (one_col) {
                    if (tid == 0) {
                        atomicAdd(&blk_heads[((long long)lp0 + below) >> 8], 1);
                        ++tiles;
                    }
                } else {
                    int upto = THREADS;
                    while (upto < total) upto <<= 1;
                    for (int x = total + tid; x < upto; x += THREADS) keys[x] = ~KeyT(0);
                    __syncthreads();
                    {
                        S1Row<KeyT, CAP, QB, THREADS> row;
                        row.keys = keys;
                        if (total <= THREADS)
                            row.template sort_regs<1, LOGT>(tid);
                        else
                            row.template sort_regs<2, LOGT>(tid);
                    }
                    const int nseg64 = (total + 63) >> 6;
                    for (int q = wave; q < nseg64; q += WAVES) {
                        const int s = 64 * q + lane;
                        const bool valid = s < total;
                        int j = 0;
                        int2 ab = make_int2(0, 0);
                        bool head = false;
                        if (valid) {
                            const KeyT key = keys[s];
                            j = (int)(key >> QB);
                            head = s == 0 || (int)(keys[s - 1] >> QB) != j;
                            ab = lab[list_src((int)gidx[(int)(key & KeyT((1u << QB) - 1u))])];
                        }
                        const unsigned long long bal = __ballot(head);
                        const long long o = (long long)lp0 + below + s;
                        if (valid) {
                            pairs_a[o] = ab.x;
                            pairs_b[o] = ab.y;
                            pair_col[o] = j | (head ? (int)0x80000000 : 0);
                        }
                        if (lane == 0) {
                            s1_note_heads(blk_heads, (long long)lp0 + below + 64 * q, bal);
                            tiles += __popcll(bal);
                        }
                    }
                }
            }
            r_lo = r_hi;
            r_hi = seg_hi;
        }
        if (lane == 0 && tiles) atomicAdd(&row_tc[i], tiles);
        __syncthreads();
    }
}

__global__ void __launch_bounds__(1024) s1_xl_gather_kernel(const int *__restrict__ xl_rows, int nrows_xl, const int *__restrict__ xl_base,
                                                            const int *__restrict__ a_tile_rowptr, int tr_lo, int a_lo,
                                                            const int2 *__restrict__ aseg, const int *__restrict__ lj, const int2 *__restrict__ lab,
                                                            int bits_tc, int local_keys, uint64_t *__restrict__ keys, uint32_t *__restrict__ perm,
                                                            int *__restrict__ prod_a, int *__restrict__ prod_b)
{
    constexpr int WAVES = 16;
    __shared__ unsigned psrc[1024];
    __shared__ int pdst[1025];
    __shared__ int wsum[WAVES];
    const int tid = threadIdx.x, lane = tid & 63, wave = tid >> 6;
    for (int li = blockIdx.x; li < nrows_xl; li += gridDim.x) {
        const int i = xl_rows[li];
        const int ra0 = a_tile_rowptr[tr_lo + i] - a_lo, ra1 = a_tile_rowptr[tr_lo + i + 1] - a_lo;
        const int c0 = ra0 / S1_CH, c1 = (ra1 - 1) / S1_CH;
        int run = xl_base[i];
        for (int pc0 = c0; pc0 <= c1; pc0 += 1024) {
            const int nb = c1 - pc0 + 1 < 1024 ? c1 - pc0 + 1 : 1024;
            unsigned src = 0;
            int cnt = 0;
            if (tid < nb) {
                const int c = pc0 + tid;
                const int first = ra0 > c * S1_CH ? ra0 : c * S1_CH, last = (ra1 < c * S1_CH + S1_CH ? ra1 : c * S1_CH + S1_CH) - 1;
                const int2 s = aseg[first], e = aseg[last];
                src = (unsigned)s.x;
                cnt = (int)((unsigned)e.x + (unsigned)e.y - src);
            }
            int inc = cnt;
#pragma unroll
            for (int d = 1; d < 64; d <<= 1) {
                const int o = __shfl_up(inc, d, 64);
                if (lane >= d) inc += o;
            }
            if (lane == 63) wsum[wave] = inc;
            __syncthreads();
            int ex = inc - cnt, tot = 0;
#pragma unroll
            for (int w = 0; w < WAVES; ++w) {
                if (w < wave) ex += wsum[w];
                tot += wsum[w];
            }
            if (tid < nb) {
                psrc[tid] = src;
                pdst[tid] = run + ex;
            }
            if (tid == 0) pdst[nb] = run + tot;
            __syncthreads();
            for (int p = wave; p < nb; p += WAVES) {
                const unsigned s = psrc[p];
                const int d0 = pdst[p], n = pdst[p + 1] - d0;
                for (int t = lane; t < n; t += 64) {
                    const int x = d0 + t;
                    const unsigned col = (unsigned)lj[s + (unsigned)t];
                    const int2 ab = lab[s + (unsigned)t];
                    keys[x] = local_keys ? ((uint64_t)col << 32) | (uint64_t)(unsigned)x : ((uint64_t)(unsigned)i << bits_tc) | (uint64_t)col;
                    perm[x] = (uint32_t)x;
                    prod_a[x] = ab.x;
                    prod_b[x] = ab.y;
                }
            }
            run += tot;
            __syncthreads();
        }
    }
}

__global__ void s1_xl_rowstart_kernel(const uint64_t *__restrict__ keys, size_t n, int bits_tc, int *__restrict__ xl_rowstart)
{
    size_t x = (size_t)blockIdx.x * blockDim.x + threadIdx.x;
    if (x >= n) return;
    int i = (int)(keys[x] >> bits_tc);
    if (x == 0 || (int)(keys[x - 1] >> bits_tc) != i) xl_rowstart[i] = (int)x;
}

__global__ void s1_xl_emit_kernel(const uint64_t *__restrict__ keys, const uint32_t *__restrict__ perm, const int *__restrict__ headx, size_t n,
                                  int bits_tc, const int *__restrict__ xl_rowstart, const int *__restrict__ row_lbase,
                                  const int *__restrict__ prod_a, const int *__restrict__ prod_b,
                                  int *__restrict__ pairs_a, int *__restrict__ pairs_b, int *__restrict__ pair_col, int *__restrict__ blk_heads,
                                  int *__restrict__ row_tc)
{
    size_t x = (size_t)blockIdx.x * blockDim.x + threadIdx.x;
    if (x >= n) return;
// ... 170 lines not shown
        PEM_LAUNCH(ctx, s1_aprod_kernel, grid_for((size_t)nA * 8, 256), 256, A->tile_colidx.as<int>(), A->tile_occ.as<uint32_t>(), p->a_lo, nA,
                   B->tile_rowptr.as<int>(), B->tile_occ.as<uint32_t>(), prune, p->aprod_off.as<int>(), p->lprod_off.as<int>());
    PEM_TRY(exclusive_scan_i32_pair(ctx, p->aprod_off.as<int>(), p->lprod_off.as<int>(), (size_t)nA, ctx->d_scalars + 3, ctx->d_scalars));
    int64_t P = 0, Pall = 0;
    {
        int64_t two[4];
        PEM_TRY(read_scalars(ctx, ctx->d_scalars, 4, two));
        P = two[0];
        Pall = two[3];
    }
    p->npairs_all = Pall;
    if (P > 0x7FFFFFFFll || Pall > 0x7FFFFFFFll) {
        set_error("step 1: %lld tile pairs exceed the int32 range of the reference's pair arrays", (long long)P);
        return PEM_E_OVERFLOW;
    }
    p->npairs = P;
    const size_t n = (size_t)P;
    PEM_TRY(p->pairs_offset.reserve(sizeof(int) * 4));
    int64_t TC = 0;
    if (n > 0) {
        PEM_TRY(p->prod_a.reserve(sizeof(int) * n));
        PEM_TRY(p->prod_b.reserve(sizeof(int) * n));
        PEM_TRY(p->sk0.reserve(sizeof(uint64_t) * n));
        PEM_TRY(p->sk1.reserve(sizeof(uint64_t) * n));
        PEM_TRY(p->sv0.reserve(sizeof(uint32_t) * n));
        PEM_TRY(p->sv1.reserve(sizeof(uint32_t) * n));
        PEM_LAUNCH(ctx, s1_esc_expand_kernel, grid_for((size_t)nA * 16, 256), 256, A->tile_keys.as<long long>(), A->tile_occ.as<uint32_t>(), p->a_lo,
                   nA, p->tr_lo, p->lprod_off.as<int>(), B->tile_rowptr.as<int>(), B->tile_colidx.as<int>(), B->tile_occ.as<uint32_t>(), prune,
                   bits_tc, p->sk0.as<uint64_t>(), p->sv0.as<uint32_t>(), p->prod_a.as<int>(), p->prod_b.as<int>());
        uint64_t *keys = nullptr;
        PEM_TRY(radix_sort_u64_u32(ctx, p->sk0.as<uint64_t>(), p->sk1.as<uint64_t>(), p->sv0.as<uint32_t>(), p->sv1.as<uint32_t>(), n,
                                   bits_tc + bits_row, &keys, &p->sorted_perm));
        DevBuf &head = ctx->tmp[2];
        PEM_TRY(head.reserve(sizeof(int) * (n + 4)));
        PEM_LAUNCH(ctx, s1_heads_kernel, grid_for(n, 256), 256, keys, n, head.as<int>());
        PEM_TRY(exclusive_scan_i32(ctx, head.as<int>(), head.as<int>(), n, ctx->d_scalars + 1));
        PEM_TRY(read_scalars(ctx, ctx->d_scalars + 1, 1, &TC));
        const size_t ntc = (size_t)TC;
        PEM_TRY(p->c_tile_rowidx.reserve(sizeof(int) * (ntc + 4)));
        PEM_TRY(p->c_tile_colidx.reserve(sizeof(int) * (ntc + 4)));
        PEM_TRY(p->pairs_offset.reserve(sizeof(int) * (ntc + 4)));
        PEM_LAUNCH(ctx, s1_emit_ctiles_kernel, grid_for(n, 256), 256, keys, head.as<int>(), n, p->tr_lo, bits_tc, p->c_tile_rowidx.as<int>(),
                   p->c_tile_colidx.as<int>(), p->pairs_offset.as<int>());
        p->c_rowidx_valid = true;
        p->compact_valid = true;
        PEM_LAUNCH(ctx, s1_c_rowptr_kernel, grid_for(ntc, 256), 256, p->c_tile_rowidx.as<int>(), (long long)TC, p->tr_lo, mt,
                   p->c_tile_rowptr.as<int>());
    } else {
        PEM_HIP(hipMemsetAsync(p->pairs_offset.p, 0, sizeof(int), st));
    }
    p->ntiles_c = TC;
    PEM_HIP(hipEventRecord(ctx->ev[1], st));
    p->state = 1;
    return PEM_OK;
}
struct S1Lanes {
    pem_ctx *ctx;
    hipStream_t main_stream;
    bool serial, forked[3] = {false, false, false};
    S1Lanes(pem_ctx *c, bool serial_) : ctx(c), main_stream(c->stream), serial(serial_) { (void)hipEventRecord(c->ev_fork, c->stream); }
    void on(int lane)
    {
        if (lane == 0 || serial) {
            ctx->stream = main_stream;
            return;
        }
        if (!forked[lane - 1]) {
            (void)hipStreamWaitEvent(ctx->aux[lane - 1], ctx->ev_fork, 0);
            forked[lane - 1] = true;
        }
        ctx->stream = ctx->aux[lane - 1];
    }
    void join()
    {
        ctx->stream = main_stream;
        for (int k = 0; k < 3; ++k)
            if (forked[k]) {
                (void)hipEventRecord(ctx->ev_join[k], ctx->aux[k]);
                (void)hipStreamWaitEvent(main_stream, ctx->ev_join[k], 0);
            }
    }
};

static void launch_rowsorts(pem_ctx *ctx, pem_cplan *p, S1Lanes &lanes, const int *counts, int mt, int bits_tc, bool force64, int nsegs)
{
    const pem_tiled *A = p->A;
    int *rl = p->row_list.as<int>();

#define PEM_ROWSORT_ARGS(BIN, QB)                                                                                                        \
    rl + (size_t)(BIN) * mt, counts[BIN], A->tile_rowptr.as<int>(), p->tr_lo, p->a_lo, p->aseg.as<int2>(), p->row_lbase.as<int>(),       \
        p->live_j.as<int>(), p->live_ab.as<int2>(), p->pairs_a.as<int>(), p->pairs_b.as<int>(), p->pair_col.as<int>(),                   \
        p->blk_heads.as<int>(), p->c_tile_rowptr.as<int>(), (QB) + bits_tc
#define PEM_ROWSORT(BIN, CAP, QB, THREADS)                                                                                               \
    do {                                                                                                                                 \
        if (bits_tc + (QB) <= 32 && !force64)                                                                                            \
            PEM_LAUNCH_NAMED(ctx, "s1_rowsort_kernel<" #CAP ">", (s1_rowsort_kernel<uint32_t, CAP, QB, THREADS>), counts[BIN], THREADS,    \
                             PEM_ROWSORT_ARGS(BIN, QB));                                                                                 \
        else                                                                                                                             \
            PEM_LAUNCH_NAMED(ctx, "s1_rowsort_kernel<" #CAP ",key64>", (s1_rowsort_kernel<uint64_t, CAP, QB, THREADS>), counts[BIN],      \
                             THREADS, PEM_ROWSORT_ARGS(BIN, QB));                                                                        \
    } while (0)
    const int ncu = ctx->cu_count > 0 ? ctx->cu_count : 256;
    const bool merge_big = !p->opt_s1_segments && !p->opt_s1_serial && counts[4] > 0 && counts[3] > 0 && counts[3] + counts[4] <= ncu &&
                           bits_tc + S1_QB4 <= 32 && !force64;
    if (p->opt_s1_segments) {
        if (nsegs > 0) {
            lanes.on(0);
            if (bits_tc + S1_QB2 <= 32 && !force64)
                PEM_LAUNCH_NAMED(ctx, "s1_rowseg_kernel", (s1_rowseg_kernel<uint32_t>), nsegs, 1024, p->seg_list.as<int2>(), nsegs, A->tile_rowptr.as<int>(),
                                 p->tr_lo, p->a_lo, p->aseg.as<int2>(), p->row_lbase.as<int>(), p->live_j.as<int>(), p->live_ab.as<int2>(),
                                 p->B->tile_cols, p->pairs_a.as<int>(), p->pairs_b.as<int>(), p->pair_col.as<int>(), p->blk_heads.as<int>(),
                                 p->c_tile_rowptr.as<int>());
            else
                PEM_LAUNCH_NAMED(ctx, "s1_rowseg_kernel<key64>", (s1_rowseg_kernel<uint64_t>), nsegs, 1024, p->seg_list.as<int2>(), nsegs,
                                 A->tile_rowptr.as<int>(), p->tr_lo, p->a_lo, p->aseg.as<int2>(), p->row_lbase.as<int>(), p->live_j.as<int>(),
                                 p->live_ab.as<int2>(), p->B->tile_cols, p->pairs_a.as<int>(), p->pairs_b.as<int>(), p->pair_col.as<int>(),
                                 p->blk_heads.as<int>(), p->c_tile_rowptr.as<int>());
        }
    } else if (merge_big) {
        lanes.on(0);
        PEM_LAUNCH_NAMED(ctx, "s1_rowsort_big_kernel", s1_rowsort_big_kernel, counts[4] + counts[3], 1024, rl + (size_t)4 * mt, counts[4],
                         rl + (size_t)3 * mt, counts[3], A->tile_rowptr.as<int>(), p->tr_lo, p->a_lo, p->aseg.as<int2>(), p->row_lbase.as<int>(),
                         p->live_j.as<int>(), p->live_ab.as<int2>(), p->pairs_a.as<int>(), p->pairs_b.as<int>(), p->pair_col.as<int>(),
                         p->blk_heads.as<int>(), p->c_tile_rowptr.as<int>(), S1_QB4 + bits_tc, S1_QB3 + bits_tc);
    } else if (counts[4] > 0) {
        lanes.on(0);
        PEM_LAUNCH_NAMED(ctx, "s1_rowsort_kernel<32768>", (s1_rowsort_kernel<uint32_t, S1_CAP4, S1_QB4, 1024>), counts[4], 1024,
                         PEM_ROWSORT_ARGS(4, S1_QB4));
    }
    if (counts[3] > 0 && !merge_big) {
        lanes.on(2);
        PEM_ROWSORT(3, 8192, S1_QB3, 1024);
    }
    if (counts[2] > 0) {
        lanes.on(3);
        PEM_ROWSORT(2, 2048, S1_QB2, 256);
    }
    if (counts[0] > 0) {
        lanes.on(1);
        PEM_LAUNCH(ctx, s1_tiny_kernel, grid_for((size_t)counts[0] * 64, 256), 256, rl, counts[0], p->row_desc.as<int4>(), p->row_lbase.as<int>(),
                   p->live_j.as<int>(), p->live_ab.as<int2>(), p->pairs_a.as<int>(), p->pairs_b.as<int>(), p->pair_col.as<int>(),
                   p->blk_heads.as<int>(), p->c_tile_rowptr.as<int>());
    }
    if (counts[1] > 0) {
        lanes.on(merge_big ? 2 : 1);
        PEM_ROWSORT(1, 512, S1_QB1, 64);
    }
    lanes.on(0);
#undef PEM_ROWSORT
#undef PEM_ROWSORT_ARGS
}

static pem_status step1_rows_impl(pem_ctx *ctx, pem_cplan *p)
{
    const pem_tiled *A = p->A, *B = p->B;
    hipStream_t st = ctx->stream;
    const int nA = p->a_hi - p->a_lo, mt = p->tr_hi - p->tr_lo;
    const int nchunks = (nA + S1_CH - 1) / S1_CH;
    const int bits_tc = bits_for((uint64_t)B->tile_cols), bits_row = bits_for((uint64_t)(mt > 0 ? mt : 1));
    const bool force64 = p->opt_key64 != 0;
    const int tiny_ok = bits_tc + S1_QB0 <= 32 && !force64;
    const int cap4 = (bits_tc + S1_QB4 <= 32 && !force64) ? S1_CAP4 : 0;
    const int xlcap = p->opt_xlcap > 0 ? p->opt_xlcap : 0x7FFFFFFF;
    p->state = 0;
    p->pairs_ready = false;
    p->c_rowidx_valid = false;
    p->compact_valid = false;
    p->ntiles_c = p->npairs = p->nnz_c = 0;
    if (p->M) mask_restore_lists(p);
    if (!ctx->capturing) PEM_HIP(hipEventRecord(ctx->ev[0], st));
    PEM_TRY(p->c_tile_rowptr.reserve(sizeof(int) * ((size_t)mt + 4)));
    PEM_TRY(p->row_list.reserve(sizeof(int) * (S1_NLIST * (size_t)mt + 4)));
    PEM_TRY(p->bin_count.reserve(sizeof(int) * BC_INTS));
    PEM_TRY(p->xl_base.reserve(sizeof(int) * ((size_t)mt + 4)));
    PEM_TRY(p->pairs_offset.reserve(sizeof(int) * 4));
    PEM_TRY(p->row_lbase.reserve(sizeof(int) * ((size_t)mt + 4)));
    PEM_TRY(p->row_desc.reserve(sizeof(int4) * ((size_t)mt + 1)));
    PEM_TRY(p->aseg.reserve(sizeof(int2) * ((size_t)nA + 4)));
    PEM_TRY(p->chunk_seg.reserve(sizeof(int2) * ((size_t)nchunks + 1)));
    PEM_TRY(p->chunk_n.reserve(sizeof(long long) * ((size_t)nchunks + 1)));
    if (!p->warm_pass) {
        PEM_HIP(hipMemsetAsync(p->bin_count.as<int>() + BC_FAULT, 0, sizeof(int) * (BC_INTS - BC_FAULT), st));
        PEM_HIP(hipMemsetAsync(ctx->d_scalars + 8, 0, sizeof(int64_t), st));
        if (nA > 0)
            PEM_LAUNCH(ctx, s1_total_kernel, grid_for((size_t)nA, 256), 256, A->tile_colidx.as<int>(), p->a_lo, nA, B->tile_rowptr.as<int>(),
                       reinterpret_cast<unsigned long long *>(ctx->d_scalars + 8));
        int64_t ntotal = 0;
        PEM_TRY(read_scalars(ctx, ctx->d_scalars + 8, 1, &ntotal));
        if (ntotal >= 0xFFFFFFFFll - 64) {
            set_error("step 1: %lld tile-level products in this row block exceed the 32-bit positions of the live-product list; split the rows "
                      "(pem_split_tile_rows) or use PEM_OPT_STEP1_GLOBAL_SORT", (long long)ntotal);
            return PEM_E_OVERFLOW;
        }
        p->w_ntotal = ntotal;
    }
    const size_t ncap = (size_t)p->w_ntotal;
    PEM_TRY(arena_phase(ctx->arena, {{&p->live_j, sizeof(int) * (ncap + 64)}, {&p->live_ab, sizeof(int2) * (ncap + 64)}}));
    PEM_TRY(p->live_j.reserve(sizeof(int) * (ncap + 64)));
    PEM_TRY(p->live_ab.reserve(sizeof(int2) * (ncap + 64)));
    int ngroups_reset = 0;
    p->group_nnz_cleared = false;
    if (p->warm_pass && p->w_TC > 0) {
        ngroups_reset = (int)((p->w_TC + S2_GROUP - 1) / S2_GROUP) + 4;
        PEM_TRY(p->group_nnz.reserve(sizeof(int) * (size_t)ngroups_reset));
        p->group_nnz_cleared = true;
    }
    const int nblk_reset = p->warm_pass ? (int)(p->w_P / 256 + 1) : 0;
    const int seg_on = p->opt_s1_segments != 0;
    PEM_TRY(p->seg_list.reserve(sizeof(int2) * (ncap / S1_SEG_T + (size_t)mt + 16)));
    const int prune = p->opt_prune;
    PEM_LAUNCH(ctx, s1_expand_kernel, (unsigned)(nchunks > 0 ? nchunks : 1), 64 * S1_XW, A->tile_colidx.as<int>(), A->tile_occ.as<uint32_t>(),
               p->a_lo, nA, B->tile_rowptr.as<int>(), B->tile_colocc.as<int2>(), prune, p->bin_count.as<int>(), (unsigned long long)ncap,
               p->aseg.as<int2>(), p->chunk_seg.as<int2>(), p->chunk_n.as<long long>(), p->live_j.as<int>(), p->live_ab.as<int2>(), ctx->d_flags,
               reinterpret_cast<long long *>(ctx->d_scalars));
    {
        const size_t span = std::max(std::max((size_t)mt, (size_t)nchunks), (size_t)1);
        PEM_LAUNCH(ctx, s1_rowclass_kernel, grid_for(span, 256), 256, A->tile_rowptr.as<int>(), p->tr_lo, p->a_lo, mt, nchunks, p->aseg.as<int2>(),
                   p->chunk_seg.as<int2>(), p->chunk_n.as<long long>(), tiny_ok, cap4, xlcap, p->row_lbase.as<int>(), p->row_desc.as<int4>(),
                   p->row_list.as<int>(), p->bin_count.as<int>(), p->xl_base.as<int>(), p->c_tile_rowptr.as<int>(),
                   reinterpret_cast<long long *>(ctx->d_scalars), ctx->d_flags, p->pairs_offset.as<int>(), p->group_nnz.as<int>(), ngroups_reset,
                   p->blk_heads.as<int>(), nblk_reset, seg_on, p->seg_list.as<int2>());
    }
    PEM_TRY(exclusive_scan_i32(ctx, p->row_lbase.as<int>(), p->row_lbase.as<int>(), (size_t)mt, ctx->d_scalars));
    int64_t P = 0, Pall = 0;
    int counts[5];
    size_t n_xl;
    int nrows_xl = 0, max_xl = 0, nsegs = 0;
    if (p->warm_pass) {
        nsegs = p->w_nsegs;
        max_xl = p->w_max_xl;
        P = p->w_P;
        Pall = p->w_Pall;
        for (int b = 0; b < 5; ++b) counts[b] = p->w_counts[b];
        n_xl = (size_t)p->w_nxl;
        nrows_xl = p->w_nrows_xl;
    } else {
        int *hb = reinterpret_cast<int *>(ctx->h_scalars + 32);
        PEM_HIP(hipMemcpyAsync(hb, p->bin_count.p, sizeof(int) * BC_FAULT, hipMemcpyDeviceToHost, st));
        int64_t sc[4];
        PEM_TRY(read_scalars(ctx, ctx->d_scalars, 4, sc));
        P = sc[0];
        Pall = sc[3];
        for (int b = 0; b < 5; ++b) counts[b] = p->w_counts[b] = hb[b];
        nrows_xl = p->w_nrows_xl = hb[BC_XL_ROWS];
        n_xl = (size_t)hb[BC_XL_TOTAL];
        max_xl = p->w_max_xl = hb[BC_XL_MAX];
        nsegs = p->w_nsegs = hb[BC_SEGS];
        p->w_nxl = (int64_t)n_xl;
        p->w_P = P;
        p->w_Pall = Pall;
    }
    p->npairs_all = Pall;
    if (P > 0x7FFFFFFFll) {
        set_error("step 1: %lld live tile pairs exceed the int32 range of the reference's pair arrays", (long long)P);
        return PEM_E_OVERFLOW;
    }
    p->npairs = P;
    const size_t n = (size_t)P;
    int64_t TC = 0;
    if (n > 0) {
        const size_t nblk = n / 256 + 1;
        PEM_TRY(arena_phase(ctx->arena, {{&p->pairs_a, sizeof(int) * (n + 4)}, {&p->pairs_b, sizeof(int) * (n + 4)},
                                         {&p->pair_col, sizeof(int) * (n + 4)}, {&p->blk_heads, sizeof(int) * (nblk + 4)}}));
        PEM_TRY(p->pairs_a.reserve(sizeof(int) * (n + 4)));
        PEM_TRY(p->pairs_b.reserve(sizeof(int) * (n + 4)));
        PEM_TRY(p->pair_col.reserve(sizeof(int) * (n + 4)));
        PEM_TRY(p->blk_heads.reserve(sizeof(int) * (nblk + 4)));
        if (!p->warm_pass) PEM_HIP(hipMemsetAsync(p->blk_heads.p, 0, sizeof(int) * (nblk + 4), st));
        const bool xl_local = n_xl > 0 && !p->opt_xl_global && max_xl <= S1_XLL_MAX;
        if (n_xl > 0) {
            PEM_TRY(p->prod_a.reserve(sizeof(int) * n_xl));
            PEM_TRY(p->prod_b.reserve(sizeof(int) * n_xl));
            PEM_TRY(p->sk0.reserve(sizeof(uint64_t) * n_xl));
            PEM_TRY(p->sk1.reserve(sizeof(uint64_t) * n_xl));
            PEM_TRY(p->sv0.reserve(sizeof(uint32_t) * n_xl));
            PEM_TRY(p->sv1.reserve(sizeof(uint32_t) * n_xl));
            PEM_TRY(p->xl_rowstart.reserve(sizeof(int) * ((size_t)mt + 4)));
        }
        const int *xl_rows = p->row_list.as<int>() + (size_t)5 * mt;
        auto xl_gather = [&](int local) {
            PEM_LAUNCH(ctx, s1_xl_gather_kernel, (unsigned)(nrows_xl > 0 ? nrows_xl : 1), 1024, xl_rows, nrows_xl, p->xl_base.as<int>(),
                       A->tile_rowptr.as<int>(), p->tr_lo, p->a_lo, p->aseg.as<int2>(), p->live_j.as<int>(), p->live_ab.as<int2>(), bits_tc, local,
                       p->sk0.as<uint64_t>(), p->sv0.as<uint32_t>(), p->prod_a.as<int>(), p->prod_b.as<int>());
        };
        S1Lanes lanes(ctx, p->opt_s1_serial != 0 || (ctx->capturing && ctx->hw_queues < 4));
        launch_rowsorts(ctx, p, lanes, counts, mt, bits_tc, force64, nsegs);
        if (xl_local) {
            lanes.on(3);
            xl_gather(1);
            PEM_LAUNCH(ctx, s1_xl_rowsort_kernel, (unsigned)(nrows_xl > 0 ? nrows_xl : 1), 1024, xl_rows, nrows_xl, p->xl_base.as<int>(),
                       p->row_lbase.as<int>(), p->sk0.as<uint64_t>(), p->sk1.as<uint64_t>(), bits_tc, p->prod_a.as<int>(), p->prod_b.as<int>(),
                       p->pairs_a.as<int>(), p->pairs_b.as<int>(), p->pair_col.as<int>(), p->blk_heads.as<int>(), p->c_tile_rowptr.as<int>());
        }
        lanes.join();
        if (n_xl > 0 && !xl_local) {
            xl_gather(0);
            uint64_t *keys = nullptr;
            uint32_t *perm = nullptr;
            PEM_TRY(radix_sort_u64_u32(ctx, p->sk0.as<uint64_t>(), p->sk1.as<uint64_t>(), p->sv0.as<uint32_t>(), p->sv1.as<uint32_t>(), n_xl,
                                       bits_tc + bits_row, &keys, &perm));
            DevBuf &head = ctx->tmp[2];
            PEM_TRY(head.reserve(sizeof(int) * (n_xl + 4)));
            PEM_LAUNCH(ctx, s1_heads_kernel, grid_for(n_xl, 256), 256, keys, n_xl, head.as<int>());
            PEM_TRY(exclusive_scan_i32(ctx, head.as<int>(), head.as<int>(), n_xl, nullptr));
            PEM_LAUNCH(ctx, s1_xl_rowstart_kernel, grid_for(n_xl, 256), 256, keys, n_xl, bits_tc, p->xl_rowstart.as<int>());
            PEM_LAUNCH(ctx, s1_xl_emit_kernel, grid_for(n_xl, 256), 256, keys, perm, head.as<int>(), n_xl, bits_tc, p->xl_rowstart.as<int>(),
                       p->row_lbase.as<int>(), p->prod_a.as<int>(), p->prod_b.as<int>(),
                       p->pairs_a.as<int>(), p->pairs_b.as<int>(), p->pair_col.as<int>(), p->blk_heads.as<int>(), p->c_tile_rowptr.as<int>());
        }
        PEM_TRY(exclusive_scan_i32_two(ctx, p->blk_heads.as<int>(), p->blk_heads.as<int>(), nblk, nullptr, p->c_tile_rowptr.as<int>(),
                                       p->c_tile_rowptr.as<int>(), (size_t)mt, ctx->d_scalars + 1));
        if (p->warm_pass) {
            TC = p->w_TC;
        } else {
            PEM_TRY(read_scalars(ctx, ctx->d_scalars + 1, 1, &TC));
            p->w_TC = TC;
        }
        p->pairs_ready = true;
    }
    if (p->M) {
        PEM_TRY(mask_filter(ctx, p, &P, &TC));
        p->npairs = P;
    }
    p->ntiles_c = TC;
    if (!ctx->capturing) PEM_HIP(hipEventRecord(ctx->ev[1], st));
    p->state = 1;
    return PEM_OK;
}


pem_status pem::ensure_compact(pem_ctx *ctx, const pem_cplan *cp)
{
    pem_cplan *p = const_cast<pem_cplan *>(cp);
    if (p->compact_valid || !p->pairs_ready || p->state < 1) return PEM_OK;
    const size_t ntc = (size_t)p->ntiles_c, n = (size_t)p->npairs;
    PEM_ENTER(ctx);
    PEM_TRY(p->c_tile_colidx.reserve(sizeof(int) * (ntc + 4)));
    PEM_TRY(p->pairs_offset.reserve(sizeof(int) * (ntc + 4)));
    if (n > 0)
        PEM_LAUNCH(ctx, s1_compact_kernel, (unsigned)((n + 255) / 256), 256, p->pair_col.as<int>(), (long long)n, p->blk_heads.as<int>(), (long long)ntc,
                   p->c_tile_colidx.as<int>(), p->pairs_offset.as<int>());
    p->compact_valid = true;
    return PEM_OK;
}

pem_status pem::step1_impl(pem_ctx *ctx, pem_cplan *p, bool allow_warm)
{
    p->warm_pass = false;
    if (p->opt_step1_esc) {
        p->warm = false;
        return step1_esc_impl(ctx, p);
    }
    p->warm_pass = allow_warm && p->warm && p->opt_warm;
    return step1_rows_impl(ctx, p);
}

pem_status pem::ensure_c_rowidx(pem_ctx *ctx, const pem_cplan *p)
{
    if (p->c_rowidx_valid || p->state < 1) return PEM_OK;
    const int mt = p->tr_hi - p->tr_lo;
    PEM_ENTER(ctx);
    PEM_TRY(p->c_tile_rowidx.reserve(sizeof(int) * ((size_t)p->ntiles_c + 4)));
    if (mt > 0 && p->ntiles_c > 0)
        PEM_LAUNCH(ctx, s1_crowidx_kernel, grid_for((size_t)mt * 64, 256), 256, p->c_tile_rowptr.as<int>(), mt, p->tr_lo, p->c_tile_rowidx.as<int>());
    p->c_rowidx_valid = true;
    return PEM_OK;
}
```

### pem-spgemm_amd/csrc/step2.hip

```cpp
#include "spgemm_internal.h"

using namespace pem;

__global__ void s2_pairs_kernel(const uint32_t *__restrict__ perm, const int *__restrict__ prod_a, const int *__restrict__ prod_b, size_t n,
                                int *__restrict__ pairs_a, int *__restrict__ pairs_b)
{
    size_t p = (size_t)blockIdx.x * blockDim.x + threadIdx.x;
    if (p >= n) return;
    uint32_t q = perm[p];
    pairs_a[p] = prod_a[q];
    pairs_b[p] = prod_b[q];
}

__global__ void __launch_bounds__(256) s2_cmask_kernel(const int *__restrict__ pairs_offset, const int *__restrict__ pairs_a,
                                                       const int *__restrict__ pairs_b, long long ntc,
                                                       const uint16_t *__restrict__ a_masks, const uint16_t *__restrict__ b_masks,
                                                       uint16_t *__restrict__ c_mask16, int *__restrict__ c_tile_nnz)
{
    long long t = ((long long)blockIdx.x * blockDim.x + threadIdx.x) >> 4;
    const int r = threadIdx.x & 15;
    const bool live = t < ntc;
    unsigned cm = 0;
    if (live) {
        int p0 = pairs_offset[t], p1 = pairs_offset[t + 1];
// ... 234 lines not shown
            c_j = __builtin_amdgcn_readlane(col, hl) & 0x7FFFFFFF;
            c_p0 = (int)(pb + hl);
#pragma unroll
            for (int q = 0; q < 8; ++q) ccw[q] = (unsigned)__builtin_amdgcn_readlane((int)cw[q], hl);
            open = true;
            t_next += __popcll(Hv);
        }
    };
    int pc[4], pia[4], pib[4];
#pragma unroll
    for (int j = 0; j < 4; ++j) {
        const long long p = p_lo + 64 * j + lane;
        const bool valid = p < npairs;
        pc[j] = valid ? pair_col[p] : (int)0x80000000;
        pia[j] = valid ? pairs_a[p] : 0;
        pib[j] = valid ? pairs_b[p] : 0;
    }
#pragma unroll
    for (int j = 0; j < 4; ++j)
        if (p_lo + 64 * j < npairs) trip(p_lo + 64 * j, pc[j], pia[j], pib[j], false);
    for (long long pb = p_lo + 256; pb < npairs && open; pb += 64) {
        const long long p = pb + lane;
        const bool valid = p < npairs;
        trip(pb, valid ? pair_col[p] : (int)0x80000000, valid ? pairs_a[p] : 0, valid ? pairs_b[p] : 0, true);
    }
    if (open && lane == 0) store_tile(c_t, c_j, c_p0, ccw);
#pragma unroll
    for (int d = 32; d > 0; d >>= 1) {
        gs0 += __shfl_xor(gs0, d, 64);
        gs1 += __shfl_xor(gs1, d, 64);
    }
    if (lane == 0) {
        if (gs0) atomicAdd(&group_nnz[g0], gs0);
        if (gs1) atomicAdd(&group_nnz[g0 + 1], gs1);
    }
}

__global__ void __launch_bounds__(S2_GROUP) s2_entries_kernel(const uint32_t *__restrict__ c_mask, long long ntc, const int *__restrict__ group_base,
                                                              long long cap_nnz, int *__restrict__ c_tile_nnz_ptr, uint8_t *__restrict__ c_rowcolidx,
                                                              int *__restrict__ chunk_tile, int *__restrict__ flags, WarmCheck wc,
                                                              const long long *__restrict__ d_scalars, const int *__restrict__ bin_count)
{
    __shared__ int w_nnz[S2_GROUP / 64];
    const int tid = threadIdx.x, lane = tid & 63, wave = tid >> 6;
    if (wc.on && blockIdx.x == 0 && tid == 0) warm_check(wc, d_scalars, bin_count, flags);
    const long long t = (long long)blockIdx.x * S2_GROUP + tid;
    unsigned cw[8] = {0, 0, 0, 0, 0, 0, 0, 0};
    if (t < ntc) {
        const uint4 M0 = *reinterpret_cast<const uint4 *>(c_mask + 8 * t);
        const uint4 M1 = *reinterpret_cast<const uint4 *>(c_mask + 8 * t + 4);
        const unsigned w[8] = {M0.x, M0.y, M0.z, M0.w, M1.x, M1.y, M1.z, M1.w};
#pragma unroll
        for (int q = 0; q < 8; ++q) cw[q] = (w[q] << 16) | (w[q] >> 16);
    }
    int nnz_t = 0;
#pragma unroll
    for (int q = 0; q < 8; ++q) nnz_t += __popc(cw[q]);
    int inc = nnz_t;
#pragma unroll
    for (int d = 1; d < 64; d <<= 1) {
        const int o = __shfl_up(inc, d, 64);
        if (lane >= d) inc += o;
    }
    if (lane == 63) w_nnz[wave] = inc;
    __syncthreads();
    long long off = (long long)group_base[blockIdx.x] + inc - nnz_t;
#pragma unroll
    for (int w = 0; w < S2_GROUP / 64; ++w)
        if (w < wave) off += w_nnz[w];
    if (t > ntc) return;
    if (t == ntc) {
        c_tile_nnz_ptr[ntc] = (int)off;
        return;
    }
    c_tile_nnz_ptr[t] = (int)off;
    if (off + nnz_t > cap_nnz) {
        flags[FLAG_CAPACITY] = 1;
        return;
    }
    for (long long ch = (off + S3_CHUNK - 1) / S3_CHUNK; ch * S3_CHUNK < off + nnz_t; ++ch) chunk_tile[ch] = (int)t;
    s2_emit_rowcol(cw, c_rowcolidx + off);
}

__global__ void __launch_bounds__(256) s2_offsets_kernel(const uint16_t *__restrict__ c_cnt, long long ntc, const int *__restrict__ group_base,
                                                         int *__restrict__ c_tile_nnz_ptr, int *__restrict__ chunk_tile, int *__restrict__ flags,
                                                         WarmCheck wc, const long long *__restrict__ d_scalars, const int *__restrict__ bin_count)
{
    static_assert(S2_GROUP == 256, "four tiles per lane of one wave");
    const int lane = threadIdx.x & 63;
    const long long g = ((long long)blockIdx.x * blockDim.x + threadIdx.x) >> 6;
    if (wc.on && g == 0 && lane == 0) warm_check(wc, d_scalars, bin_count, flags);
    const long long t = g * S2_GROUP + 4 * lane;
    if (t > ntc) return;
    int n[4] = {0, 0, 0, 0};
    if (t + 4 <= ntc) {
        const uint2 q = *reinterpret_cast<const uint2 *>(c_cnt + t);
        n[0] = (int)(q.x & 0xFFFFu);
        n[1] = (int)(q.x >> 16);
        n[2] = (int)(q.y & 0xFFFFu);
        n[3] = (int)(q.y >> 16);
    } else {
#pragma unroll
        for (int k = 0; k < 4; ++k) n[k] = t + k < ntc ? (int)c_cnt[t + k] : 0;
    }
    const int tsum = n[0] + n[1] + n[2] + n[3];
    int inc = tsum;
#pragma unroll
    for (int d = 1; d < 64; d <<= 1) {
        const int o = __shfl_up(inc, d, 64);
        if (lane >= d) inc += o;
    }
    int o4[4];
    o4[0] = group_base[g] + inc - tsum;
    o4[1] = o4[0] + n[0];
    o4[2] = o4[1] + n[1];
    o4[3] = o4[2] + n[2];
    if (t + 4 <= ntc) {
        *reinterpret_cast<int4 *>(c_tile_nnz_ptr + t) = make_int4(o4[0], o4[1], o4[2], o4[3]);
    } else {
#pragma unroll
        for (int k = 0; k < 4; ++k)
            if (t + k <= ntc) c_tile_nnz_ptr[t + k] = o4[k];
    }
#pragma unroll
    for (int k = 0; k < 4; ++k) {
        if (t + k >= ntc) break;
        const long long off = o4[k];
        for (long long ch = (off + S3_CHUNK - 1) / S3_CHUNK; ch * S3_CHUNK < off + n[k]; ++ch) chunk_tile[ch] = (int)(t + k);
    }
}

__global__ void __launch_bounds__(256) s2_crowptr_kernel(const uint32_t *__restrict__ c_mask, long long ntc, uint8_t *__restrict__ c_rowptr)
{
    long long t = (long long)blockIdx.x * blockDim.x + threadIdx.x;
    if (t >= ntc) return;
    const uint4 M0 = *reinterpret_cast<const uint4 *>(c_mask + 8 * t);
    const uint4 M1 = *reinterpret_cast<const uint4 *>(c_mask + 8 * t + 4);
    const unsigned w[8] = {M0.x, M0.y, M0.z, M0.w, M1.x, M1.y, M1.z, M1.w};
    unsigned rp[4] = {0, 0, 0, 0};
    int run = 0;
#pragma unroll
    for (int q = 0; q < 8; ++q) {
        rp[q >> 1] |= (unsigned)run << (16 * (q & 1));
        run += __popc(w[q] >> 16);
        rp[q >> 1] |= (unsigned)run << (16 * (q & 1) + 8);
        run += __popc(w[q] & 0xFFFFu);
    }
    *reinterpret_cast<uint4 *>(c_rowptr + 16 * t) = make_uint4(rp[0], rp[1], rp[2], rp[3]);
}

pem_status pem::step2_impl(pem_ctx *ctx, pem_cplan *p)
{
    if (p->state < 1) {
        set_error("pem_spgemm_step2 called before step 1");
        return PEM_E_STATE;
    }
    const pem_tiled *A = p->A, *B = p->B;
    hipStream_t st = ctx->stream;
    const size_t n = (size_t)p->npairs, ntc = (size_t)p->ntiles_c;
    if (!ctx->chain_events) PEM_HIP(hipEventRecord(ctx->ev[2], st));
    PEM_TRY(arena_phase(ctx->arena, {{&p->pairs_a, sizeof(int) * (n + 4)}, {&p->pairs_b, sizeof(int) * (n + 4)},
                                     {&p->c_mask, sizeof(uint32_t) * 8 * (ntc + 1)}, {&p->c_tile_nnz_ptr, sizeof(int) * (ntc + 4)},
                                     {&p->c_tile_colidx, sizeof(int) * (ntc + 4)}, {&p->pairs_offset, sizeof(int) * (ntc + 4)},
                                     {&p->group_nnz, sizeof(int) * ((ntc + S2_GROUP - 1) / S2_GROUP + 4)}}));
    PEM_TRY(p->pairs_a.reserve(sizeof(int) * (n + 4)));
    PEM_TRY(p->pairs_b.reserve(sizeof(int) * (n + 4)));
    PEM_TRY(p->c_mask.reserve(sizeof(uint32_t) * 8 * (ntc + 1)));
    PEM_TRY(p->c_tile_nnz_ptr.reserve(sizeof(int) * (ntc + 4)));
    p->c_rowptr_valid = false;
    const bool fused = p->pairs_ready && p->opt_wide;
    p->wide = fused;
    p->verify_folded = false;
    p->flags_mirrored = false;
    p->s3_decode = false;
    p->c_rowcolidx_valid = false;
    int64_t nnzc = 0;
    if (fused) {
        PEM_TRY(p->c_tile_colidx.reserve(sizeof(int) * (ntc + 4)));
        PEM_TRY(p->pairs_offset.reserve(sizeof(int) * (ntc + 4)));
        if (n > 0) {
            const size_t ngroups = (ntc + S2_GROUP - 1) / S2_GROUP;
            PEM_TRY(p->group_nnz.reserve(sizeof(int) * (ngroups + 4)));
            if (!p->group_nnz_cleared) PEM_HIP(hipMemsetAsync(p->group_nnz.p, 0, sizeof(int) * (ngroups + 4), st));
            p->group_nnz_cleared = false;
            int *group_nnz = p->group_nnz.as<int>();
            const bool deep = p->npairs >= 2 * p->ntiles_c;
            const bool decode = p->opt_decode && !deep;
            p->s3_decode = decode;
            if (decode) PEM_TRY(p->c_tile_cnt.reserve(sizeof(uint16_t) * (ntc + 8)));
            const bool transposed = p->opt_s2_transposed == 1 || (p->opt_s2_transposed == 2 && p->warm_pass && p->w_P >= 2 * p->w_TC);
            const uint16_t *a_m = transposed ? A->masks_t.as<uint16_t>() : A->masks.as<uint16_t>();
            uint16_t *c_cnt = decode ? p->c_tile_cnt.as<uint16_t>() : (uint16_t *)nullptr;
            const int *c_mtile = p->M ? p->c_mtile.as<int>() : (const int *)nullptr;
            const uint16_t *m_masks = p->M ? p->M->masks.as<uint16_t>() : (const uint16_t *)nullptr;
            const unsigned m_inv = p->mask_complement ? ~0u : 0u;
#define PEM_S2_TILES(NAME, ...)                                                                                                      \
    PEM_LAUNCH_NAMED(ctx, NAME, (s2_tiles_kernel<__VA_ARGS__>), (unsigned)((n + 1023) / 1024), 256, p->pair_col.as<int>(), p->pairs_a.as<int>(), \
                     p->pairs_b.as<int>(), (long long)n, p->blk_heads.as<int>(), a_m, B->masks.as<uint16_t>(), A->tile_occ.as<uint32_t>(),     \
                     B->tile_occ.as<uint32_t>(), (long long)ntc, p->c_tile_colidx.as<int>(), p->pairs_offset.as<int>(), p->c_mask.as<uint32_t>(), \
                     group_nnz, c_cnt, c_mtile, m_masks, m_inv)
            if (p->M && transposed)
                PEM_S2_TILES("s2_tiles_kernel<transposed, masked>", true, true);
            else if (p->M)
                PEM_S2_TILES("s2_tiles_kernel<masked>", false, true);
            else if (transposed)
                PEM_S2_TILES("s2_tiles_kernel<transposed>", true);
            else
                PEM_S2_TILES("s2_tiles_kernel", false);
#undef PEM_S2_TILES
            PEM_TRY(exclusive_scan_i32(ctx, group_nnz, group_nnz, ngroups, ctx->d_scalars + 2));
            if (p->warm_pass) {
                nnzc = p->w_nnz;
            } else {
                int64_t sc[1];
                PEM_TRY(read_scalars(ctx, ctx->d_scalars + 2, 1, sc));
                int hf[NUM_FLAGS];
                PEM_TRY(read_flags(ctx, hf));
                PEM_TRY(check_internal(hf));
                if (hf[FLAG_OVERFLOW] || sc[0] > 0x7FFFFFFFll) {
                    set_error("step 2: C has more than 2^31-1 nonzeros, beyond the int32 range of the reference's offsets");
                    return PEM_E_OVERFLOW;
                }
                nnzc = sc[0];
            }
            PEM_TRY(arena_phase(ctx->arena, {{&p->c_rowcolidx, decode ? (size_t)0 : (size_t)nnzc + 16},
                                             {&p->s3_chunk_tile, sizeof(int) * ((size_t)nnzc / S3_CHUNK + 4)},
                                             {&p->c_vals, (size_t)A->value_bytes * ((size_t)nnzc + 1)}}));
            PEM_TRY(p->s3_chunk_tile.reserve(sizeof(int) * ((size_t)nnzc / S3_CHUNK + 4)));
            WarmCheck wc = {};
            if (p->warm_pass) wc = warm_check_of(p);
            p->verify_folded = p->warm_pass;
            if (p->warm_pass && decode && ctx->h_flags_dev) {
                wc.host_flags = ctx->h_flags_dev;
                p->flags_mirrored = true;
            }
            if (decode) {
                PEM_LAUNCH(ctx, s2_offsets_kernel, grid_for(((ntc + S2_GROUP) / S2_GROUP) * 64, 256), 256, p->c_tile_cnt.as<uint16_t>(), (long long)ntc,
                           group_nnz, p->c_tile_nnz_ptr.as<int>(), p->s3_chunk_tile.as<int>(), ctx->d_flags, wc,
                           reinterpret_cast<const long long *>(ctx->d_scalars), p->bin_count.as<int>());
                p->c_rowcolidx_valid = false;
            } else {
                PEM_TRY(p->c_rowcolidx.reserve((size_t)nnzc + 16));
                PEM_LAUNCH(ctx, s2_entries_kernel, (unsigned)((ntc + S2_GROUP) / S2_GROUP), S2_GROUP, p->c_mask.as<uint32_t>(), (long long)ntc, group_nnz,
                           (long long)nnzc, p->c_tile_nnz_ptr.as<int>(), p->c_rowcolidx.as<uint8_t>(), p->s3_chunk_tile.as<int>(), ctx->d_flags, wc,
                           reinterpret_cast<const long long *>(ctx->d_scalars), p->bin_count.as<int>());
                p->c_rowcolidx_valid = true;
            }
            p->compact_valid = true;
        } else {
            PEM_TRY(exclusive_scan_i32(ctx, p->c_tile_nnz_ptr.as<int>(), p->c_tile_nnz_ptr.as<int>(), 0, ctx->d_scalars + 2));
            p->compact_valid = true;
            p->c_rowcolidx_valid = true;
        }
    } else {
        PEM_TRY(ensure_compact(ctx, p));
        if (n > 0 && !p->pairs_ready)
            PEM_LAUNCH(ctx, s2_pairs_kernel, grid_for(n, 256), 256, p->sorted_perm, p->prod_a.as<int>(), p->prod_b.as<int>(), n, p->pairs_a.as<int>(),
                       p->pairs_b.as<int>());
        if (ntc > 0)
            PEM_LAUNCH(ctx, s2_cmask_kernel, grid_for(ntc * 16, 256), 256, p->pairs_offset.as<int>(), p->pairs_a.as<int>(), p->pairs_b.as<int>(),
                       (long long)ntc, A->masks.as<uint16_t>(), B->masks.as<uint16_t>(), p->c_mask.as<uint16_t>(), p->c_tile_nnz_ptr.as<int>());
        PEM_TRY(exclusive_scan_i32(ctx, p->c_tile_nnz_ptr.as<int>(), p->c_tile_nnz_ptr.as<int>(), ntc, ctx->d_scalars + 2));
        if (p->warm_pass) {
            nnzc = p->w_nnz;
        } else {
            PEM_TRY(read_scalars(ctx, ctx->d_scalars + 2, 1, &nnzc));
        }
    }
    if (!p->warm_pass) {
        if (!fused) {
            int hf[NUM_FLAGS];
            PEM_TRY(read_flags(ctx, hf));
            if (hf[FLAG_OVERFLOW] || nnzc > 0x7FFFFFFFll) {
                set_error("step 2: C has more than 2^31-1 nonzeros, beyond the int32 range of the reference's offsets");
                return PEM_E_OVERFLOW;
            }
        }
        p->w_nnz = nnzc;
    }
    p->nnz_c = nnzc;
    if (!(fused && p->s3_decode)) {
        PEM_TRY(p->c_rowcolidx.reserve((size_t)nnzc + 16));
        p->c_rowcolidx_valid = fused;
    }
    PEM_TRY(p->s3_chunk_tile.reserve(sizeof(int) * ((size_t)nnzc / S3_CHUNK + 4)));
    PEM_TRY(p->c_vals.reserve((size_t)A->value_bytes * ((size_t)nnzc + 1)));
    if (ntc > 0 && !fused) {
        PEM_TRY(p->c_rowptr.reserve(16 * (ntc + 1)));
        PEM_LAUNCH(ctx, s2_crowcol_kernel, grid_for(ntc * 16, 256), 256, p->c_mask.as<uint16_t>(), p->c_tile_nnz_ptr.as<int>(), (long long)ntc,
                   p->c_rowptr.as<uint8_t>(), p->c_rowcolidx.as<uint8_t>());
        p->c_rowptr_valid = true;
        p->c_rowcolidx_valid = true;
    }
    if (!ctx->capturing) PEM_HIP(hipEventRecord(ctx->ev[3], st));
    p->state = 2;
    return PEM_OK;
}

pem_status pem::ensure_c_rowptr(pem_ctx *ctx, const pem_cplan *p)
{
    if (p->c_rowptr_valid || p->state < 2) return PEM_OK;
    const size_t ntc = (size_t)p->ntiles_c;
    PEM_ENTER(ctx);
    PEM_TRY(p->c_rowptr.reserve(16 * (ntc + 1)));
    if (ntc > 0) PEM_LAUNCH(ctx, s2_crowptr_kernel, grid_for(ntc, 256), 256, p->c_mask.as<uint32_t>(), (long long)ntc, p->c_rowptr.as<uint8_t>());
    p->c_rowptr_valid = true;
    return PEM_OK;
}

pem_status pem::ensure_c_rowcolidx(pem_ctx *ctx, const pem_cplan *cp)
{
    pem_cplan *p = const_cast<pem_cplan *>(cp);
    if (p->c_rowcolidx_valid || p->state < 2) return PEM_OK;
    const size_t ntc = (size_t)p->ntiles_c;
    PEM_ENTER(ctx);
    PEM_TRY(p->c_rowcolidx.reserve((size_t)p->nnz_c + 16));
    if (ntc > 0) {
        WarmCheck wc = {};
        PEM_LAUNCH(ctx, s2_entries_kernel, (unsigned)((ntc + S2_GROUP) / S2_GROUP), S2_GROUP, p->c_mask.as<uint32_t>(), (long long)ntc,
                   p->group_nnz.as<int>(), (long long)p->nnz_c, p->c_tile_nnz_ptr.as<int>(), p->c_rowcolidx.as<uint8_t>(), p->s3_chunk_tile.as<int>(),
                   ctx->d_flags, wc, reinterpret_cast<const long long *>(ctx->d_scalars), p->bin_count.as<int>());
    }
    p->c_rowcolidx_valid = true;
    return PEM_OK;
}
```

Before: 203.7.

## Fold scans into rowclass and offsets kernels, add single-launch step1 mode

```diff
diff --git a/include/pem_spgemm.h b/include/pem_spgemm.h
--- a/include/pem_spgemm.h
+++ b/include/pem_spgemm.h
@@ -186,7 +186,7 @@
     PEM_OPT_S3_BAND = 4,
     PEM_OPT_EXPORT_ROWS = 7,
     PEM_OPT__TEST_FIRST = 5,
-    PEM_OPT__LAST = 18
+    PEM_OPT__LAST = 21
 } pem_option;
 pem_status pem_cplan_set_option(pem_cplan *plan, pem_option which, int64_t value);
 pem_status pem_cplan_get_option(const pem_cplan *plan, pem_option which, int64_t *value);
diff --git a/pem-spgemm_amd/__init__.py b/pem-spgemm_amd/__init__.py
--- a/pem-spgemm_amd/__init__.py
+++ b/pem-spgemm_amd/__init__.py
@@ -52,7 +52,8 @@
 
 VALUE_ORDERS = dict(row=0, col=1)
 
-OPTIONS = dict(prune=0, step1_global_sort=1, wide=2, warm=3, s3_band=4, s1_force_key64=5, s1_xlcap=6, export_rows=7, s1_serial=8, s3_decode=9, s1_xl_global=10, s3_epw=11, s3_idx64=12, s3_mark=13, s3_xcd=14, s1_segments=15, s2_transposed=16, s3_poison=17)
+OPTIONS = dict(prune=0, step1_global_sort=1, wide=2, warm=3, s3_band=4, s1_force_key64=5, s1_xlcap=6, export_rows=7, s1_serial=8, s3_decode=9, s1_xl_global=10, s3_epw=11, s3_idx64=12, s3_mark=13, s3_xcd=14, s1_segments=15, s2_transposed=16, s3_poison=17,
+               s1_class_scan=18, s2_tail_fold=19, s1_one_launch=20)
 
 
 class PemError(RuntimeError):
diff --git a/pem-spgemm_amd/csrc/pem_internal.h b/pem-spgemm_amd/csrc/pem_internal.h
--- a/pem-spgemm_amd/csrc/pem_internal.h
+++ b/pem-spgemm_amd/csrc/pem_internal.h
@@ -349,6 +349,11 @@
     pem::DevBuf seg_list;
     int opt_s2_transposed = 2;
     int opt_s1_segments = 0;
+    int opt_s1_class_scan = 1;
+    int opt_s2_tail_fold = 1;
+    bool group_nnz_scanned = false;
+    int opt_s1_one_launch = 2;
+    int s1_one = -1;
     int64_t w_nxl = 0;
     int w_nrows_xl = 0, w_max_xl = 0;
 };
diff --git a/pem-spgemm_amd/csrc/primitives.hip b/pem-spgemm_amd/csrc/primitives.hip
--- a/pem-spgemm_amd/csrc/primitives.hip
+++ b/pem-spgemm_amd/csrc/primitives.hip
@@ -1,4 +1,5 @@
 #include "pem_internal.h"
+#include "scan_chain.h"
 #include <algorithm>
 #include <cstdarg>
 
@@ -264,24 +265,6 @@
 constexpr int SCAN_TILES_PER_BLOCK = 8;
 constexpr int SCAN_BLOCK_ITEMS = SCAN_TILE * SCAN_TILES_PER_BLOCK;
 
-template <typename T> __device__ __forceinline__ T wave_inclusive_scan(T v)
-{
-    const int lane = threadIdx.x & 63;
-#pragma unroll
-    for (int d = 1; d < 64; d <<= 1) {
-        T t = __shfl_up(v, d, 64);
-        if (lane >= d) v += t;
-    }
-    return v;
-}
-
-template <typename T> __device__ __forceinline__ T wave_reduce_sum(T v)
-{
-#pragma unroll
-    for (int d = 32; d > 0; d >>= 1) v += __shfl_xor(v, d, 64);
-    return v;
-}
-
 __global__ void __launch_bounds__(SCAN_THREADS) scan_reduce_kernel(const int *__restrict__ in, size_t n,
                                                                    long long *__restrict__ bsum)
 {
@@ -440,8 +423,7 @@
     }
 }
 
-constexpr int SCAN_MID_ITEMS = 2048, SCAN_MID_BLOCKS = 128;
-constexpr unsigned long long SCAN_MID_VALID = 1ull << 63;
+constexpr int SCAN_MID_ITEMS = 2048;
 
 struct ScanMidArgs {
     const int *in[2];
@@ -462,10 +444,9 @@
     int *out = args.out[y];
     const size_t n = args.n[y];
     long long *total64 = args.total64[y];
-    unsigned long long *state = state_all + (size_t)y * (SCAN_MID_BLOCKS + 2);
-    int *ctl = reinterpret_cast<int *>(state + SCAN_MID_BLOCKS);
+    unsigned long long *state = state_all + (size_t)y * SCAN_MID_SET_WORDS;
     const int tid = threadIdx.x, lane = tid & 63, wave = tid >> 6;
-    if (tid == 0) s_ticket = atomicAdd(&ctl[1], 1);
+    if (tid == 0) s_ticket = scan_chain_ticket(state);
     __syncthreads();
     const int blk = s_ticket;
     const size_t i0 = (size_t)blk * SCAN_MID_ITEMS + (size_t)tid * 8;
@@ -493,20 +474,8 @@
     if (wave == 0) {
         if (blk == stall_ticket)
             for (int k = 0; k < 50; ++k) __builtin_amdgcn_s_sleep(127);
-        if (lane == 0) __hip_atomic_store(&state[blk], SCAN_MID_VALID | (unsigned long long)btotal, __ATOMIC_RELAXED, __HIP_MEMORY_SCOPE_AGENT);
-        long long excl = 0;
-        bool ok = false;
-        for (long long polls = 0; polls < (1ll << 24) && !ok; ++polls) {
-            const unsigned long long a = lane < blk ? __hip_atomic_load(&state[lane], __ATOMIC_RELAXED, __HIP_MEMORY_SCOPE_AGENT) : SCAN_MID_VALID;
-            const unsigned long long b = 64 + lane < blk ? __hip_atomic_load(&state[64 + lane], __ATOMIC_RELAXED, __HIP_MEMORY_SCOPE_AGENT) : SCAN_MID_VALID;
-            if (__ballot(!(a & SCAN_MID_VALID) || !(b & SCAN_MID_VALID)) == 0) {
-                excl = wave_reduce_sum((long long)(a & ~SCAN_MID_VALID) + (long long)(b & ~SCAN_MID_VALID));
-                ok = true;
-            } else {
-                __builtin_amdgcn_s_sleep(1);
-            }
-        }
-        if (!ok && lane == 0) flags[FLAG_INTERNAL] = 1;
+        if (lane == 0) scan_chain_publish(state, blk, btotal);
+        const long long excl = scan_chain_lookback(state, blk, lane, flags);
         if (lane == 0) s_excl = excl;
     }
     __syncthreads();
@@ -530,19 +499,15 @@
             if (total64) *total64 = total;
             if (total > 0x7FFFFFFFLL) flags[FLAG_OVERFLOW] = 1;
         }
-        if (atomicAdd(&ctl[0], 1) == nblk - 1) {
-            for (int b = 0; b < nblk; ++b) __hip_atomic_store(&state[b], 0ull, __ATOMIC_RELAXED, __HIP_MEMORY_SCOPE_AGENT);
-            __hip_atomic_store(&ctl[0], 0, __ATOMIC_RELAXED, __HIP_MEMORY_SCOPE_AGENT);
-            __hip_atomic_store(&ctl[1], 0, __ATOMIC_RELAXED, __HIP_MEMORY_SCOPE_AGENT);
-        }
-    }
-}
-
-static pem_status scan_mid_state(pem_ctx *ctx)
+        scan_chain_done(state, nblk);
+    }
+}
+
+pem_status scan_mid_state(pem_ctx *ctx)
 {
     if (!ctx->scan_state.p) {
-        PEM_TRY(ctx->scan_state.reserve(sizeof(unsigned long long) * 2 * (SCAN_MID_BLOCKS + 2)));
-        PEM_HIP(hipMemsetAsync(ctx->scan_state.p, 0, sizeof(unsigned long long) * 2 * (SCAN_MID_BLOCKS + 2), ctx->stream));
+        PEM_TRY(ctx->scan_state.reserve(sizeof(unsigned long long) * SCAN_MID_SETS * SCAN_MID_SET_WORDS));
+        PEM_HIP(hipMemsetAsync(ctx->scan_state.p, 0, sizeof(unsigned long long) * SCAN_MID_SETS * SCAN_MID_SET_WORDS, ctx->stream));
     }
     return PEM_OK;
 }
diff --git a/pem-spgemm_amd/csrc/scan_chain.h b/pem-spgemm_amd/csrc/scan_chain.h
--- /dev/null
+++ b/pem-spgemm_amd/csrc/scan_chain.h
@@ -0,0 +1,68 @@
+#pragma once
+#include "pem_internal.h"
+
+namespace pem {
+
+constexpr int SCAN_MID_BLOCKS = 128;
+constexpr int SCAN_MID_SETS = 3;
+constexpr unsigned long long SCAN_MID_VALID = 1ull << 63;
+constexpr size_t SCAN_MID_SET_WORDS = SCAN_MID_BLOCKS + 2;
+
+template <typename T> __device__ __forceinline__ T wave_inclusive_scan(T v)
+{
+    const int lane = threadIdx.x & 63;
+#pragma unroll
+    for (int d = 1; d < 64; d <<= 1) {
+        T t = __shfl_up(v, d, 64);
+        if (lane >= d) v += t;
+    }
+    return v;
+}
+
+template <typename T> __device__ __forceinline__ T wave_reduce_sum(T v)
+{
+#pragma unroll
+    for (int d = 32; d > 0; d >>= 1) v += __shfl_xor(v, d, 64);
+    return v;
+}
+
+__device__ __forceinline__ int *scan_chain_ctl(unsigned long long *state) { return reinterpret_cast<int *>(state + SCAN_MID_BLOCKS); }
+
+__device__ __forceinline__ int scan_chain_ticket(unsigned long long *state) { return atomicAdd(&scan_chain_ctl(state)[1], 1); }
+
+__device__ __forceinline__ void scan_chain_publish(unsigned long long *state, const int blk, const long long btotal)
+{
+    __hip_atomic_store(&state[blk], SCAN_MID_VALID | (unsigned long long)btotal, __ATOMIC_RELAXED, __HIP_MEMORY_SCOPE_AGENT);
+}
+
+__device__ __forceinline__ long long scan_chain_lookback(unsigned long long *state, const int blk, const int lane, int *__restrict__ flags)
+{
+    long long excl = 0;
+    bool ok = false;
+    for (long long polls = 0; polls < (1ll << 24) && !ok; ++polls) {
+        const unsigned long long a = lane < blk ? __hip_atomic_load(&state[lane], __ATOMIC_RELAXED, __HIP_MEMORY_SCOPE_AGENT) : SCAN_MID_VALID;
+        const unsigned long long b = 64 + lane < blk ? __hip_atomic_load(&state[64 + lane], __ATOMIC_RELAXED, __HIP_MEMORY_SCOPE_AGENT) : SCAN_MID_VALID;
+        if (__ballot(!(a & SCAN_MID_VALID) || !(b & SCAN_MID_VALID)) == 0) {
+            excl = wave_reduce_sum((long long)(a & ~SCAN_MID_VALID) + (long long)(b & ~SCAN_MID_VALID));
+            ok = true;
+        } else {
+            __builtin_amdgcn_s_sleep(1);
+        }
+    }
+    if (!ok && lane == 0) flags[FLAG_INTERNAL] = 1;
+    return excl;
+}
+
+__device__ __forceinline__ void scan_chain_done(unsigned long long *state, const int nblk)
+{
+    int *ctl = scan_chain_ctl(state);
+    if (atomicAdd(&ctl[0], 1) == nblk - 1) {
+        for (int b = 0; b < nblk; ++b) __hip_atomic_store(&state[b], 0ull, __ATOMIC_RELAXED, __HIP_MEMORY_SCOPE_AGENT);
+        __hip_atomic_store(&ctl[0], 0, __ATOMIC_RELAXED, __HIP_MEMORY_SCOPE_AGENT);
+        __hip_atomic_store(&ctl[1], 0, __ATOMIC_RELAXED, __HIP_MEMORY_SCOPE_AGENT);
+    }
+}
+
+pem_status scan_mid_state(pem_ctx *ctx);
+
+}
diff --git a/pem-spgemm_amd/csrc/spgemm.hip b/pem-spgemm_amd/csrc/spgemm.hip
--- a/pem-spgemm_amd/csrc/spgemm.hip
+++ b/pem-spgemm_amd/csrc/spgemm.hip
@@ -59,6 +59,12 @@
     p->opt_idx64 = env_is("PEM_S3_IDX64", "1");
     p->opt_mark = !env_is("PEM_S3_MARK", "0");
     p->opt_s1_segments = env_is("PEM_S1_SEGMENTS", "1");
+    p->opt_s1_class_scan = !env_is("PEM_S1_CLASS_SCAN", "0");
+    p->opt_s2_tail_fold = !env_is("PEM_S2_TAIL_FOLD", "0");
+    {
+        const char *e = getenv("PEM_S1_ONE_LAUNCH");
+        p->opt_s1_one_launch = e ? atoi(e) : 2;
+    }
     {
         const char *e = getenv("PEM_S3_EPW");
         p->opt_epw = e ? atoi(e) : 0;
@@ -160,6 +166,9 @@
     case PEM_OPT_S1_SEGMENTS: return &p->opt_s1_segments;
     case PEM_OPT_S2_TRANSPOSED: return &p->opt_s2_transposed;
     case PEM_OPT_S3_POISON: return &p->opt_s3_poison;
+    case PEM_OPT_S1_CLASS_SCAN: return &p->opt_s1_class_scan;
+    case PEM_OPT_S2_TAIL_FOLD: return &p->opt_s2_tail_fold;
+    case PEM_OPT_S1_ONE_LAUNCH: return &p->opt_s1_one_launch;
     default: return nullptr;
     }
 }
@@ -177,21 +186,22 @@
                   which == PEM_OPT_WIDE ? "PEM_OPT_WIDE" : "PEM_OPT_STEP1_GLOBAL_SORT", (long long)value);
         return PEM_E_INVALID;
     }
-    const int v = (which == PEM_OPT_S1_XLCAP || which == PEM_OPT_S3_EPW || which == PEM_OPT_S2_TRANSPOSED || which == PEM_OPT_S3_POISON) ? (int)value : (value != 0);
+    const int v = (which == PEM_OPT_S1_XLCAP || which == PEM_OPT_S3_EPW || which == PEM_OPT_S2_TRANSPOSED || which == PEM_OPT_S3_POISON || which == PEM_OPT_S1_ONE_LAUNCH) ? (int)value : (value != 0);
     if (*slot == v) return PEM_OK;
     *slot = v;
     plan->warm = false;
     int keep = 3;
     switch ((int)which) {
     case PEM_OPT_PRUNE: case PEM_OPT_STEP1_GLOBAL_SORT: case PEM_OPT_S1_FORCE_KEY64: case PEM_OPT_S1_XLCAP: case PEM_OPT_S1_XL_GLOBAL:
-    case PEM_OPT_S1_SEGMENTS: keep = 0; break;
-    case PEM_OPT_WIDE: case PEM_OPT_S3_DECODE: case PEM_OPT_S2_TRANSPOSED: keep = 1; break;
+    case PEM_OPT_S1_SEGMENTS: case PEM_OPT_S1_CLASS_SCAN: case PEM_OPT_S1_ONE_LAUNCH: keep = 0; break;
+    case PEM_OPT_WIDE: case PEM_OPT_S3_DECODE: case PEM_OPT_S2_TRANSPOSED: case PEM_OPT_S2_TAIL_FOLD: keep = 1; break;
     case PEM_OPT_S3_BAND: case PEM_OPT_S3_EPW: case PEM_OPT_S3_IDX64: case PEM_OPT_S3_MARK: case PEM_OPT_S3_XCD:
     case PEM_OPT_S3_POISON: keep = 2; break;
     default: break;
     }
     if (plan->state > keep) plan->state = keep;
     if (keep == 0) {
+        plan->s1_one = -1;
         plan->pairs_ready = false;
         plan->compact_valid = plan->c_rowidx_valid = false;
     }
diff --git a/pem-spgemm_amd/csrc/spgemm_internal.h b/pem-spgemm_amd/csrc/spgemm_internal.h
--- a/pem-spgemm_amd/csrc/spgemm_internal.h
+++ b/pem-spgemm_amd/csrc/spgemm_internal.h
@@ -7,6 +7,7 @@
 
 constexpr int S3_CHUNK = 256;
 constexpr int S2_GROUP = 256;
+constexpr int S2_FOLD_GROUPS = 8192;
 
 enum { BC_BIN0 = 0, BC_XL_ROWS = 5, BC_XL_TOTAL = 6, BC_XL_MAX = 7, BC_SEGS = 8 , BC_FAULT = 9, BC_BUMP = 10 , BC_INTS = 16 };
 
@@ -19,15 +20,20 @@
     long long Pm, TCm;
 };
 __device__ __forceinline__ void warm_check(const WarmCheck &w, const long long *__restrict__ d_scalars, const int *__restrict__ bin_count,
-                                           int *__restrict__ flags)
+                                           int *__restrict__ flags, const long long nnz_now)
 {
-    if (d_scalars[0] != w.P || d_scalars[1] != w.TC || d_scalars[2] != w.nnz || d_scalars[3] != w.Pall || bin_count[0] != w.c[0] ||
+    if (d_scalars[0] != w.P || d_scalars[1] != w.TC || nnz_now != w.nnz || d_scalars[3] != w.Pall || bin_count[0] != w.c[0] ||
         bin_count[1] != w.c[1] || bin_count[2] != w.c[2] || bin_count[3] != w.c[3] || bin_count[4] != w.c[4] || bin_count[BC_XL_TOTAL] != w.nxl || bin_count[BC_SEGS] != w.nsegs)
         flags[FLAG_CAPACITY] = 1;
     if (w.masked && (d_scalars[4] != w.Pm || d_scalars[5] != w.TCm)) flags[FLAG_CAPACITY] = 1;
     if (w.host_flags) {
         for (int i = 0; i < NUM_FLAGS; ++i) w.host_flags[i] = flags[i];
     }
+}
+__device__ __forceinline__ void warm_check(const WarmCheck &w, const long long *__restrict__ d_scalars, const int *__restrict__ bin_count,
+                                           int *__restrict__ flags)
+{
+    warm_check(w, d_scalars, bin_count, flags, d_scalars[2]);
 }
 
 inline WarmCheck warm_check_of(const pem_cplan *p)
diff --git a/pem-spgemm_amd/csrc/step1.hip b/pem-spgemm_amd/csrc/step1.hip
--- a/pem-spgemm_amd/csrc/step1.hip
+++ b/pem-spgemm_amd/csrc/step1.hip
@@ -1,4 +1,5 @@
 #include "spgemm_internal.h"
+#include "scan_chain.h"
 
 using namespace pem;
 
@@ -118,6 +119,7 @@
 constexpr int S1_NLIST = 6;
 constexpr int S1_PC1 = 64, S1_PC2 = 256, S1_PC3 = 1024;
 constexpr int S1_SEG_T = 1024;
+constexpr int S1_NOSEG = 1 << 30;
 constexpr int S1_XLL_MAX = 1 << 18;
 
 __global__ void __launch_bounds__(256) s1_total_kernel(const int *__restrict__ a_tile_colidx, int a_lo, int nA, const int *__restrict__ b_tile_rowptr,
@@ -348,16 +350,27 @@
     }
 }
 
-__global__ void __launch_bounds__(256) s1_rowclass_kernel(const int *__restrict__ a_tile_rowptr, int tr_lo, int a_lo, int mt, int nchunks,
+constexpr int S1_RC_SCAN_THREADS = 512;
+template <int THREADS, bool SCAN>
+__global__ void __launch_bounds__(THREADS) s1_rowclass_kernel(const int *__restrict__ a_tile_rowptr, int tr_lo, int a_lo, int mt, int nchunks,
                                                           const int2 *__restrict__ aseg, const int2 *__restrict__ chunk_seg,
                                                           const long long *__restrict__ chunk_n, int tiny_ok, int cap4, int xlcap,
                                                           int *__restrict__ row_l, int4 *__restrict__ row_desc, int *__restrict__ row_list,
                                                           int *__restrict__ bin_count, int *__restrict__ xl_base, int *__restrict__ row_tc,
                                                           long long *__restrict__ scalars, int *__restrict__ flags, int *__restrict__ pairs_offset,
                                                           int *__restrict__ group_nnz, int ngroups, int *__restrict__ blk_heads, int nblk,
-                                                          int seg_on, int2 *__restrict__ seg_list)
-{
-    const int i = blockIdx.x * blockDim.x + threadIdx.x;
+                                                          int seg_on, int2 *__restrict__ seg_list, unsigned long long *__restrict__ chain)
+{
+    __shared__ int s_ticket;
+    __shared__ long long rc_wsum[THREADS / 64];
+    __shared__ long long s_excl;
+    int blk = blockIdx.x;
+    if constexpr (SCAN) {
+        if (threadIdx.x == 0) s_ticket = scan_chain_ticket(chain);
+        __syncthreads();
+        blk = s_ticket;
+    }
+    const int i = blk * THREADS + threadIdx.x;
     const int lane = threadIdx.x & 63;
     const unsigned long long lt = (1ull << lane) - 1ull;
     int nl = 0, np = 0;
@@ -383,7 +396,7 @@
                 nl = tot > 0x7FFFFFFFll ? 0x7FFFFFFF : (int)tot;
             }
         }
-        row_l[i] = nl;
+        if constexpr (!SCAN) row_l[i] = nl;
         row_desc[i] = make_int4((int)pos0, cnt0, (int)pos1, nl);
         xl_base[i] = -1;
         row_tc[i] = 0;
@@ -396,19 +409,34 @@
         else if (nl <= S1_CAP2 && np <= S1_PC2) bin = 2;
         else if (nl <= S1_CAP3 && np <= S1_PC3) bin = 3;
         else if (nl <= cap4 && np <= S1_PC3) bin = 4;
-        if (seg_on && bin >= 4) bin = (nl <= S1_XLL_MAX && np <= S1_PC2) ? 4 : 5;
+        if (seg_on == 1 && bin >= 4) bin = (nl <= S1_XLL_MAX && np <= S1_PC2) ? 4 : 5;
         if (nl > xlcap) bin = 5;
         if (seg_on && bin == 4) {
-            const int G = (nl + S1_SEG_T - 1) / S1_SEG_T;
-            const int s0 = atomicAdd(&bin_count[BC_SEGS], G);
-            for (int g = 0; g < G; ++g) seg_list[s0 + g] = make_int2(i, g | (G << 16));
+            if (seg_on == 2 && np > S1_PC2) {
+                atomicOr(&bin_count[BC_SEGS], S1_NOSEG);
+            } else {
+                const int G = (nl + S1_SEG_T - 1) / S1_SEG_T;
+                const int s0 = atomicAdd(&bin_count[BC_SEGS], G) & (S1_NOSEG - 1);
+                for (int g = 0; g < G; ++g) seg_list[s0 + g] = make_int2(i, g | (G << 16));
+            }
         }
     }
     __shared__ int blk_cnt[S1_NLIST], blk_base[S1_NLIST];
     __shared__ long long blk_all;
     if (threadIdx.x < S1_NLIST) blk_cnt[threadIdx.x] = 0;
     if (threadIdx.x == 0) blk_all = 0;
+    long long rc_inc = 0;
+    if constexpr (SCAN) {
+        rc_inc = wave_inclusive_scan((long long)nl);
+        if (lane == 63) rc_wsum[threadIdx.x >> 6] = rc_inc;
+    }
     __syncthreads();
+    long long rc_btotal = 0;
+    if constexpr (SCAN) {
+#pragma unroll
+        for (int w = 0; w < THREADS / 64; ++w) rc_btotal += rc_wsum[w];
+        if (threadIdx.x == 0) scan_chain_publish(chain, blk, rc_btotal);
+    }
     int wbase = 0, rank = 0;
 #pragma unroll
     for (int b = 0; b < S1_NLIST; ++b) {
@@ -432,7 +460,30 @@
     __syncthreads();
     if (threadIdx.x < S1_NLIST) blk_base[threadIdx.x] = blk_cnt[threadIdx.x] ? atomicAdd(&bin_count[threadIdx.x], blk_cnt[threadIdx.x]) : 0;
     if (threadIdx.x == 0 && blk_all) atomicAdd(reinterpret_cast<unsigned long long *>(&scalars[3]), (unsigned long long)blk_all);
+    if constexpr (SCAN) {
+        if ((threadIdx.x >> 6) == THREADS / 64 - 1) {
+            const long long excl = scan_chain_lookback(chain, blk, lane, flags);
+            if (lane == 0) s_excl = excl;
+        }
+    }
     __syncthreads();
+    if constexpr (SCAN) {
+        const long long carry = s_excl;
+        long long woff = 0;
+#pragma unroll
+        for (int w = 0; w < THREADS / 64; ++w)
+            if (w < (int)(threadIdx.x >> 6)) woff += rc_wsum[w];
+        if (i < mt) row_l[i] = (int)(carry + woff + rc_inc - nl);
+        if (threadIdx.x == 0) {
+            if (blk == (int)gridDim.x - 1) {
+                const long long total = carry + rc_btotal;
+                row_l[mt] = (int)total;
+                scalars[0] = total;
+                if (total > 0x7FFFFFFFLL) flags[FLAG_OVERFLOW] = 1;
+            }
+            scan_chain_done(chain, (int)gridDim.x);
+        }
+    }
     if (bin >= 0) row_list[(size_t)bin * mt + blk_base[bin] + wbase + rank] = i;
     if (bin == 5) {
         xl_base[i] = atomicAdd(&bin_count[BC_XL_TOTAL], nl);
@@ -465,6 +516,15 @@
     return (uint64_t)__shfl_xor((unsigned long long)v, mask, 64);
 }
 
+template <int THREADS> __device__ __forceinline__ void s1_sync()
+{
+    if constexpr (THREADS == 64) {
+        __builtin_amdgcn_fence(__ATOMIC_ACQ_REL, "wavefront");
+        __builtin_amdgcn_wave_barrier();
+    } else {
+        __syncthreads();
+    }
+}
 template <typename KeyT, int THREADS, int EPT, int LOGT>
 __device__ __forceinline__ void s1_bitonic_regs(KeyT (&v)[EPT], KeyT *lds, const int tid, const bool reverse = false)
 {
@@ -504,20 +564,20 @@
                 const bool lower = (tid & tm) == 0;
 #pragma unroll
                 for (int m = 0; m < EPT; ++m) lds[m * THREADS + tid] = v[m];
-                __syncthreads();
+                s1_sync<THREADS>();
 #pragma unroll
                 for (int m = 0; m < EPT; ++m) {
                     const KeyT pv = lds[m * THREADS + (tid ^ tm)];
                     const bool up = (((tid << LOGE) | m) & kk) == 0;
                     v[m] = ((v[m] < pv) == (lower == up)) ? v[m] : pv;
                 }
-                __syncthreads();
+                s1_sync<THREADS>();
             }
         }
     }
 #pragma unroll
     for (int m = 0; m < EPT; ++m) lds[reverse ? (THREADS * EPT - 1 - ((tid << LOGE) | m)) : ((tid << LOGE) | m)] = v[m];
-    __syncthreads();
+    s1_sync<THREADS>();
 }
 __device__ __forceinline__ void s1_note_heads(int *__restrict__ blk_heads, const long long p0, const unsigned long long bal)
 {
@@ -530,15 +590,12 @@
     if (c1) atomicAdd(&blk_heads[b0 + 1], c1);
 }
 
-__global__ void __launch_bounds__(256) s1_tiny_kernel(const int *__restrict__ row_list, int nrows_bin, const int4 *__restrict__ row_desc,
-                                                      const int *__restrict__ row_lbase, const int *__restrict__ lj, const int2 *__restrict__ lab,
-                                                      int *__restrict__ pairs_a, int *__restrict__ pairs_b, int *__restrict__ pair_col,
-                                                      int *__restrict__ blk_heads, int *__restrict__ row_tc)
+__device__ __forceinline__ void s1_tiny_row(const int i, const int4 *__restrict__ row_desc, const int *__restrict__ row_lbase,
+                                            const int *__restrict__ lj, const int2 *__restrict__ lab, int *__restrict__ pairs_a,
+                                            int *__restrict__ pairs_b, int *__restrict__ pair_col, int *__restrict__ blk_heads,
+                                            int *__restrict__ row_tc)
 {
     const int lane = threadIdx.x & 63;
-    const int li = (int)((blockIdx.x * blockDim.x + threadIdx.x) >> 6);
-    if (li >= nrows_bin) return;
-    const int i = __builtin_amdgcn_readfirstlane(row_list[li]);
     const int4 d = row_desc[i];
     const int lp0 = row_lbase[i], nl = d.w;
     const bool valid = lane < nl;
@@ -572,6 +629,15 @@
         s1_note_heads(blk_heads, lp0, bal);
         row_tc[i] = __popcll(bal);
     }
+}
+__global__ void __launch_bounds__(256) s1_tiny_kernel(const int *__restrict__ row_list, int nrows_bin, const int4 *__restrict__ row_desc,
+                                                      const int *__restrict__ row_lbase, const int *__restrict__ lj, const int2 *__restrict__ lab,
+                                                      int *__restrict__ pairs_a, int *__restrict__ pairs_b, int *__restrict__ pair_col,
+                                                      int *__restrict__ blk_heads, int *__restrict__ row_tc)
+{
+    const int li = (int)((blockIdx.x * blockDim.x + threadIdx.x) >> 6);
+    if (li >= nrows_bin) return;
+    s1_tiny_row(__builtin_amdgcn_readfirstlane(row_list[li]), row_desc, row_lbase, lj, lab, pairs_a, pairs_b, pair_col, blk_heads, row_tc);
 }
 
 template <typename KeyT, int CAP, int QB, int THREADS>
@@ -667,7 +733,7 @@
         KeyT v[EPT];
 #pragma unroll
         for (int m = 0; m < EPT; ++m) v[m] = keys[m * THREADS + tid];
-        __syncthreads();
+        s1_sync<THREADS>();
         s1_bitonic_regs<KeyT, THREADS, EPT, LOGT>(v, keys, tid);
     }
 };
@@ -714,9 +780,9 @@
 {
     constexpr int LOGT = THREADS == 64 ? 6 : THREADS == 256 ? 8 : 10;
     constexpr int EMAX = CAP / THREADS, WAVES = THREADS / 64;
-    static_assert(EMAX == 8 || EMAX == 32, "a bin sorts up to 8 (or, for the largest, 32) keys per thread");
+    static_assert(EMAX == 8 || EMAX == 32 || (EMAX == 2 && THREADS == 1024), "a bin sorts up to 8 (or, for the largest, 32) keys per thread; 2048-key rows on sixteen waves: 2");
     static_assert(CAP <= (1 << QB), "the key's index field holds every position of the row's list");
-    const int tid = threadIdx.x, lane = tid & 63, wave = tid >> 6;
+    const int tid = THREADS == 64 ? (int)(threadIdx.x & 63) : (int)threadIdx.x, lane = tid & 63, wave = tid >> 6;
     (void)li;
     (void)LOGT;
 #ifdef PEM_S1_DEBUG
@@ -749,7 +815,7 @@
         int ex = inc - cnt;
         if (THREADS > 64 && np > 64) {
             if (lane == 63) wsum[wave] = inc;
-            __syncthreads();
+            s1_sync<THREADS>();
 #pragma unroll
             for (int w = 0; w < WAVES; ++w)
                 if (w < wave) ex += wsum[w];
@@ -760,7 +826,7 @@
         }
         if (tid == 0) pdst[np] = nl;
     }
-    __syncthreads();
+    s1_sync<THREADS>();
     S1_DBG_MARK(0);
     for (int x0 = tid; x0 < nl; x0 += 4 * THREADS) {
         unsigned src[4];
@@ -782,7 +848,7 @@
         while (upto < nl) upto <<= 1;
         for (int x = nl + tid; x < upto; x += THREADS) keys[x] = ~KeyT(0);
     }
-    __syncthreads();
+    s1_sync<THREADS>();
     S1_DBG_MARK(1);
     S1Row<KeyT, CAP, QB, THREADS> row;
     row.keys = keys;
@@ -839,7 +905,7 @@
     int base = mytiles;
     if constexpr (THREADS > 64) {
         if (lane == 0) wsum[wave] = mytiles;
-        __syncthreads();
+        s1_sync<THREADS>();
         base = 0;
 #pragma unroll
         for (int w = 0; w < WAVES; ++w) base += wsum[w];
@@ -861,7 +927,7 @@
         }
     }
 #endif
-    __syncthreads();
+    s1_sync<THREADS>();
 }
 
 template <typename KeyT, int CAP, int QB, int THREADS>
@@ -902,22 +968,17 @@
 }
 
 template <typename KeyT>
-__global__ void __launch_bounds__(1024) s1_rowseg_kernel(const int2 *__restrict__ seg_list, int nsegs, const int *__restrict__ a_tile_rowptr, int tr_lo,
-                                                        int a_lo, const int2 *__restrict__ aseg, const int *__restrict__ row_lbase,
-                                                        const int *__restrict__ lj, const int2 *__restrict__ lab, int tile_cols,
-                                                        int *__restrict__ pairs_a, int *__restrict__ pairs_b, int *__restrict__ pair_col,
-                                                        int *__restrict__ blk_heads, int *__restrict__ row_tc)
+__device__ __forceinline__ void s1_rowseg_one(KeyT *const keys, unsigned *const gidx, unsigned *const psrc, int *const pdst, int *const wcnt,
+                                              int *const wlow, int *const wsum, const int2 sd, const int *__restrict__ a_tile_rowptr, int tr_lo,
+                                              int a_lo, const int2 *__restrict__ aseg, const int *__restrict__ row_lbase,
+                                              const int *__restrict__ lj, const int2 *__restrict__ lab, int tile_cols,
+                                              int *__restrict__ pairs_a, int *__restrict__ pairs_b, int *__restrict__ pair_col,
+                                              int *__restrict__ blk_heads, int *__restrict__ row_tc)
 {
     constexpr int CAP = S1_CAP2, QB = S1_QB2, THREADS = 1024, WAVES = 16, LOGT = 10;
-    __shared__ KeyT keys[CAP];
-    __shared__ unsigned gidx[CAP];
-    __shared__ unsigned psrc[S1_PC2];
-    __shared__ int pdst[S1_PC2 + 1];
-    __shared__ int wcnt[WAVES], wlow[WAVES], wsum[WAVES];
     const int tid = threadIdx.x, lane = tid & 63, wave = tid >> 6;
     const unsigned long long lt = (1ull << lane) - 1ull;
-    for (int si = blockIdx.x; si < nsegs; si += gridDim.x) {
-        const int2 sd = seg_list[si];
+    {
         const int i = sd.x, g = sd.y & 0xFFFF, G = sd.y >> 16;
         const int ra0 = a_tile_rowptr[tr_lo + i] - a_lo, ra1 = a_tile_rowptr[tr_lo + i + 1] - a_lo;
         const int lp0 = row_lbase[i], nl = row_lbase[i + 1] - lp0;
@@ -1081,6 +1142,88 @@
         __syncthreads();
     }
 }
+template <typename KeyT>
+__global__ void __launch_bounds__(1024) s1_rowseg_kernel(const int2 *__restrict__ seg_list, int nsegs, const int *__restrict__ a_tile_rowptr, int tr_lo,
+                                                        int a_lo, const int2 *__restrict__ aseg, const int *__restrict__ row_lbase,
+                                                        const int *__restrict__ lj, const int2 *__restrict__ lab, int tile_cols,
+                                                        int *__restrict__ pairs_a, int *__restrict__ pairs_b, int *__restrict__ pair_col,
+                                                        int *__restrict__ blk_heads, int *__restrict__ row_tc)
+{
+    __shared__ KeyT keys[S1_CAP2];
+    __shared__ unsigned gidx[S1_CAP2];
+    __shared__ unsigned psrc[S1_PC2];
+    __shared__ int pdst[S1_PC2 + 1];
+    __shared__ int wcnt[16], wlow[16], wsum[16];
+    for (int si = blockIdx.x; si < nsegs; si += gridDim.x)
+        s1_rowseg_one<KeyT>(keys, gidx, psrc, pdst, wcnt, wlow, wsum, seg_list[si], a_tile_rowptr, tr_lo, a_lo, aseg, row_lbase, lj, lab, tile_cols,
+                            pairs_a, pairs_b, pair_col, blk_heads, row_tc);
+}
+
+struct S1BinsArgs {
+    const int *row_list;
+    int mt, n0, n1, n2, n3, nsegs;
+    const int2 *seg_list;
+    const int *a_tile_rowptr;
+    int tr_lo, a_lo;
+    const int2 *aseg;
+    const int *row_lbase;
+    const int4 *row_desc;
+    const int *lj;
+    const int2 *lab;
+    int tile_cols, bits_tc;
+    int *pairs_a, *pairs_b, *pair_col, *blk_heads, *row_tc;
+};
+constexpr int S1_BINS_LDS = 4 * S1_CAP3 + 4 * 1024 + 4 * 1028 + 4 * 16 + 4 * 16 * 256;
+constexpr int S1_BINS_W1 = 4 * S1_CAP1 + 4 * S1_PC1 + 4 * (S1_PC1 + 4) + 16;
+static_assert(16 * S1_BINS_W1 <= S1_BINS_LDS && 8 * S1_CAP2 + 8 * S1_PC2 + 16 + 3 * 64 <= S1_BINS_LDS, "every role fits the 8192-key role's LDS");
+__global__ void __launch_bounds__(1024, 8) s1_bins_kernel(const S1BinsArgs a)
+{
+    __shared__ __attribute__((aligned(16))) unsigned char smem[S1_BINS_LDS];
+    const int wave = threadIdx.x >> 6;
+    int b = blockIdx.x;
+    if (b < a.nsegs) {
+        uint32_t *keys = reinterpret_cast<uint32_t *>(smem);
+        unsigned *gidx = keys + S1_CAP2, *psrc = gidx + S1_CAP2;
+        int *pdst = reinterpret_cast<int *>(psrc + S1_PC2), *wcnt = pdst + S1_PC2 + 4, *wlow = wcnt + 16, *wsum = wlow + 16;
+        s1_rowseg_one<uint32_t>(keys, gidx, psrc, pdst, wcnt, wlow, wsum, a.seg_list[b], a.a_tile_rowptr, a.tr_lo, a.a_lo, a.aseg, a.row_lbase, a.lj,
+                                a.lab, a.tile_cols, a.pairs_a, a.pairs_b, a.pair_col, a.blk_heads, a.row_tc);
+        return;
+    }
+    b -= a.nsegs;
+    if (b < a.n3 + a.n2) {
+        uint32_t *keys = reinterpret_cast<uint32_t *>(smem);
+        unsigned *psrc = keys + S1_CAP3;
+        int *pdst = reinterpret_cast<int *>(psrc + 1024), *wsum = pdst + 1028;
+        unsigned *hist = reinterpret_cast<unsigned *>(wsum + 16);
+        if (b < a.n3)
+            s1_rowsort_row<uint32_t, S1_CAP3, S1_QB3, 1024>(keys, psrc, pdst, wsum, hist, a.row_list[(size_t)3 * a.mt + b], b, a.a_tile_rowptr, a.tr_lo,
+                                                            a.a_lo, a.aseg, a.row_lbase, a.lj, a.lab, a.pairs_a, a.pairs_b, a.pair_col, a.blk_heads,
+                                                            a.row_tc, S1_QB3 + a.bits_tc);
+        else
+            s1_rowsort_row<uint32_t, S1_CAP2, S1_QB2, 1024>(keys, psrc, pdst, wsum, hist, a.row_list[(size_t)2 * a.mt + b - a.n3], b - a.n3,
+                                                            a.a_tile_rowptr, a.tr_lo, a.a_lo, a.aseg, a.row_lbase, a.lj, a.lab, a.pairs_a, a.pairs_b,
+                                                            a.pair_col, a.blk_heads, a.row_tc, S1_QB2 + a.bits_tc);
+        return;
+    }
+    b -= a.n3 + a.n2;
+    const int nb1 = (a.n1 + 15) >> 4;
+    if (b < nb1) {
+        const int li = b * 16 + wave;
+        if (li >= a.n1) return;
+        uint32_t *keys = reinterpret_cast<uint32_t *>(smem + (size_t)wave * S1_BINS_W1);
+        unsigned *psrc = keys + S1_CAP1;
+        int *pdst = reinterpret_cast<int *>(psrc + S1_PC1), *wsum = pdst + S1_PC1 + 4;
+        s1_rowsort_row<uint32_t, S1_CAP1, S1_QB1, 64>(keys, psrc, pdst, wsum, nullptr, __builtin_amdgcn_readfirstlane(a.row_list[(size_t)a.mt + li]), li,
+                                                      a.a_tile_rowptr, a.tr_lo, a.a_lo, a.aseg, a.row_lbase, a.lj, a.lab, a.pairs_a, a.pairs_b,
+                                                      a.pair_col, a.blk_heads, a.row_tc, S1_QB1 + a.bits_tc);
+        return;
+    }
+    b -= nb1;
+    const int li = b * 16 + wave;
+    if (li < a.n0)
+        s1_tiny_row(__builtin_amdgcn_readfirstlane(a.row_list[li]), a.row_desc, a.row_lbase, a.lj, a.lab, a.pairs_a, a.pairs_b, a.pair_col, a.blk_heads,
+                    a.row_tc);
+}
 
 __global__ void __launch_bounds__(1024) s1_xl_gather_kernel(const int *__restrict__ xl_rows, int nrows_xl, const int *__restrict__ xl_base,
                                                             const int *__restrict__ a_tile_rowptr, int tr_lo, int a_lo,
@@ -1417,10 +1560,41 @@
     }
 };
 
-static void launch_rowsorts(pem_ctx *ctx, pem_cplan *p, S1Lanes &lanes, const int *counts, int mt, int bits_tc, bool force64, int nsegs)
+static void launch_rowsorts(pem_ctx *ctx, pem_cplan *p, S1Lanes &lanes, const int *counts, int mt, int bits_tc, bool force64, int nsegs, bool seg_on,
+                            bool one_launch)
 {
     const pem_tiled *A = p->A;
     int *rl = p->row_list.as<int>();
+    if (one_launch) {
+        S1BinsArgs a;
+        a.row_list = rl;
+        a.mt = mt;
+        a.n0 = counts[0];
+        a.n1 = counts[1];
+        a.n2 = counts[2];
+        a.n3 = counts[3];
+        a.nsegs = nsegs;
+        a.seg_list = p->seg_list.as<int2>();
+        a.a_tile_rowptr = A->tile_rowptr.as<int>();
+        a.tr_lo = p->tr_lo;
+        a.a_lo = p->a_lo;
+        a.aseg = p->aseg.as<int2>();
+        a.row_lbase = p->row_lbase.as<int>();
+        a.row_desc = p->row_desc.as<int4>();
+        a.lj = p->live_j.as<int>();
+        a.lab = p->live_ab.as<int2>();
+        a.tile_cols = p->B->tile_cols;
+        a.bits_tc = bits_tc;
+        a.pairs_a = p->pairs_a.as<int>();
+        a.pairs_b = p->pairs_b.as<int>();
+        a.pair_col = p->pair_col.as<int>();
+        a.blk_heads = p->blk_heads.as<int>();
+        a.row_tc = p->c_tile_rowptr.as<int>();
+        const size_t grid = (size_t)nsegs + counts[3] + counts[2] + (counts[1] + 15) / 16 + (counts[0] + 15) / 16;
+        lanes.on(0);
+        if (grid > 0) PEM_LAUNCH(ctx, s1_bins_kernel, (unsigned)grid, 1024, a);
+        return;
+    }
 
 #define PEM_ROWSORT_ARGS(BIN, QB)                                                                                                        \
     rl + (size_t)(BIN) * mt, counts[BIN], A->tile_rowptr.as<int>(), p->tr_lo, p->a_lo, p->aseg.as<int2>(), p->row_lbase.as<int>(),       \
@@ -1436,9 +1610,9 @@
                              THREADS, PEM_ROWSORT_ARGS(BIN, QB));                                                                        \
     } while (0)
     const int ncu = ctx->cu_count > 0 ? ctx->cu_count : 256;
-    const bool merge_big = !p->opt_s1_segments && !p->opt_s1_serial && counts[4] > 0 && counts[3] > 0 && counts[3] + counts[4] <= ncu &&
+    const bool merge_big = !seg_on && !p->opt_s1_serial && counts[4] > 0 && counts[3] > 0 && counts[3] + counts[4] <= ncu &&
                            bits_tc + S1_QB4 <= 32 && !force64;
-    if (p->opt_s1_segments) {
+    if (seg_on) {
         if (nsegs > 0) {
             lanes.on(0);
             if (bits_tc + S1_QB2 <= 32 && !force64)
@@ -1541,7 +1715,11 @@
         p->group_nnz_cleared = true;
     }
     const int nblk_reset = p->warm_pass ? (int)(p->w_P / 256 + 1) : 0;
-    const int seg_on = p->opt_s1_segments != 0;
+    const int ncu_bins = ctx->cu_count > 0 ? ctx->cu_count : 256;
+    const bool one_allowed = p->opt_s1_one_launch != 0 && !force64 && bits_tc + S1_QB3 <= 32 && !p->opt_s1_serial &&
+                             (p->opt_s1_segments == 0 || p->opt_s1_one_launch == 1);
+    const int seg_on = p->opt_s1_segments != 0 ? 1 : (one_allowed ? 2 : 0);
+    if (!one_allowed) p->s1_one = 0;
     PEM_TRY(p->seg_list.reserve(sizeof(int2) * (ncap / S1_SEG_T + (size_t)mt + 16)));
     const int prune = p->opt_prune;
     PEM_LAUNCH(ctx, s1_expand_kernel, (unsigned)(nchunks > 0 ? nchunks : 1), 64 * S1_XW, A->tile_colidx.as<int>(), A->tile_occ.as<uint32_t>(),
@@ -1550,13 +1728,21 @@
                reinterpret_cast<long long *>(ctx->d_scalars));
     {
         const size_t span = std::max(std::max((size_t)mt, (size_t)nchunks), (size_t)1);
-        PEM_LAUNCH(ctx, s1_rowclass_kernel, grid_for(span, 256), 256, A->tile_rowptr.as<int>(), p->tr_lo, p->a_lo, mt, nchunks, p->aseg.as<int2>(),
-                   p->chunk_seg.as<int2>(), p->chunk_n.as<long long>(), tiny_ok, cap4, xlcap, p->row_lbase.as<int>(), p->row_desc.as<int4>(),
-                   p->row_list.as<int>(), p->bin_count.as<int>(), p->xl_base.as<int>(), p->c_tile_rowptr.as<int>(),
-                   reinterpret_cast<long long *>(ctx->d_scalars), ctx->d_flags, p->pairs_offset.as<int>(), p->group_nnz.as<int>(), ngroups_reset,
-                   p->blk_heads.as<int>(), nblk_reset, seg_on, p->seg_list.as<int2>());
-    }
-    PEM_TRY(exclusive_scan_i32(ctx, p->row_lbase.as<int>(), p->row_lbase.as<int>(), (size_t)mt, ctx->d_scalars));
+#define PEM_ROWCLASS(NAME, THREADS, SCAN, CHAIN)                                                                                                  \
+    PEM_LAUNCH_NAMED(ctx, NAME, (s1_rowclass_kernel<THREADS, SCAN>), grid_for(span, THREADS), THREADS, A->tile_rowptr.as<int>(), p->tr_lo, p->a_lo, mt, \
+                     nchunks, p->aseg.as<int2>(), p->chunk_seg.as<int2>(), p->chunk_n.as<long long>(), tiny_ok, cap4, xlcap, p->row_lbase.as<int>(), \
+                     p->row_desc.as<int4>(), p->row_list.as<int>(), p->bin_count.as<int>(), p->xl_base.as<int>(), p->c_tile_rowptr.as<int>(),       \
+                     reinterpret_cast<long long *>(ctx->d_scalars), ctx->d_flags, p->pairs_offset.as<int>(), p->group_nnz.as<int>(), ngroups_reset, \
+                     p->blk_heads.as<int>(), nblk_reset, seg_on, p->seg_list.as<int2>(), CHAIN)
+        if (p->opt_s1_class_scan && span <= (size_t)S1_RC_SCAN_THREADS * SCAN_MID_BLOCKS) {
+            PEM_TRY(scan_mid_state(ctx));
+            PEM_ROWCLASS("s1_rowclass_kernel<scan>", S1_RC_SCAN_THREADS, true, ctx->scan_state.as<unsigned long long>() + 2 * SCAN_MID_SET_WORDS);
+        } else {
+            PEM_ROWCLASS("s1_rowclass_kernel", 256, false, (unsigned long long *)nullptr);
+            PEM_TRY(exclusive_scan_i32(ctx, p->row_lbase.as<int>(), p->row_lbase.as<int>(), (size_t)mt, ctx->d_scalars));
+        }
+#undef PEM_ROWCLASS
+    }
     int64_t P = 0, Pall = 0;
     int counts[5];
     size_t n_xl;
@@ -1585,6 +1771,9 @@
         p->w_P = P;
         p->w_Pall = Pall;
     }
+    if (!p->warm_pass && one_allowed)
+        p->s1_one = nrows_xl == 0 && n_xl == 0 && nsegs < S1_NOSEG && (nsegs <= ncu_bins || p->opt_s1_one_launch == 1) ? 1 : 0;
+    const bool one_mode = p->s1_one == 1;
     p->npairs_all = Pall;
     if (P > 0x7FFFFFFFll) {
         set_error("step 1: %lld live tile pairs exceed the int32 range of the reference's pair arrays", (long long)P);
@@ -1618,8 +1807,8 @@
                        A->tile_rowptr.as<int>(), p->tr_lo, p->a_lo, p->aseg.as<int2>(), p->live_j.as<int>(), p->live_ab.as<int2>(), bits_tc, local,
                        p->sk0.as<uint64_t>(), p->sv0.as<uint32_t>(), p->prod_a.as<int>(), p->prod_b.as<int>());
         };
-        S1Lanes lanes(ctx, p->opt_s1_serial != 0 || (ctx->capturing && ctx->hw_queues < 4));
-        launch_rowsorts(ctx, p, lanes, counts, mt, bits_tc, force64, nsegs);
+        S1Lanes lanes(ctx, p->opt_s1_serial != 0 || one_mode || (ctx->capturing && ctx->hw_queues < 4));
+        launch_rowsorts(ctx, p, lanes, counts, mt, bits_tc, force64, nsegs, seg_on == 1, one_mode);
         if (xl_local) {
             lanes.on(3);
             xl_gather(1);
diff --git a/pem-spgemm_amd/csrc/step2.hip b/pem-spgemm_amd/csrc/step2.hip
--- a/pem-spgemm_amd/csrc/step2.hip
+++ b/pem-spgemm_amd/csrc/step2.hip
@@ -340,14 +340,35 @@
     s2_emit_rowcol(cw, c_rowcolidx + off);
 }
 
+template <bool FOLD>
 __global__ void __launch_bounds__(256) s2_offsets_kernel(const uint16_t *__restrict__ c_cnt, long long ntc, const int *__restrict__ group_base,
                                                          int *__restrict__ c_tile_nnz_ptr, int *__restrict__ chunk_tile, int *__restrict__ flags,
-                                                         WarmCheck wc, const long long *__restrict__ d_scalars, const int *__restrict__ bin_count)
+                                                         WarmCheck wc, long long *d_scalars, const int *__restrict__ bin_count)
 {
     static_assert(S2_GROUP == 256, "four tiles per lane of one wave");
     const int lane = threadIdx.x & 63;
     const long long g = ((long long)blockIdx.x * blockDim.x + threadIdx.x) >> 6;
-    if (wc.on && g == 0 && lane == 0) warm_check(wc, d_scalars, bin_count, flags);
+    int gbase = 0;
+    if constexpr (FOLD) {
+        __shared__ int f_wsum[4];
+        const int wave = threadIdx.x >> 6;
+        const int4 *cnt4 = reinterpret_cast<const int4 *>(group_base);
+        const int nq = (int)blockIdx.x;
+        int s = 0;
+#pragma unroll 8
+        for (int k = threadIdx.x; k < nq; k += 256) {
+            const int4 q = cnt4[k];
+            s += q.x + q.y + q.z + q.w;
+        }
+#pragma unroll
+        for (int d = 32; d > 0; d >>= 1) s += __shfl_xor(s, d, 64);
+        if (lane == 0) f_wsum[wave] = s;
+        __syncthreads();
+        gbase = f_wsum[0] + f_wsum[1] + f_wsum[2] + f_wsum[3];
+        for (int w = 0; w < wave; ++w) gbase += group_base[4 * nq + w];
+    } else {
+        if (wc.on && g == 0 && lane == 0) warm_check(wc, d_scalars, bin_count, flags);
+    }
     const long long t = g * S2_GROUP + 4 * lane;
     if (t > ntc) return;
     int n[4] = {0, 0, 0, 0};
@@ -369,7 +390,8 @@
         if (lane >= d) inc += o;
     }
     int o4[4];
-    o4[0] = group_base[g] + inc - tsum;
+    if constexpr (!FOLD) gbase = group_base[g];
+    o4[0] = gbase + inc - tsum;
     o4[1] = o4[0] + n[0];
     o4[2] = o4[1] + n[1];
     o4[3] = o4[2] + n[2];
@@ -379,6 +401,14 @@
 #pragma unroll
         for (int k = 0; k < 4; ++k)
             if (t + k <= ntc) c_tile_nnz_ptr[t + k] = o4[k];
+        if constexpr (FOLD) {
+#pragma unroll
+            for (int k = 0; k < 4; ++k)
+                if (t + k == ntc) {
+                    d_scalars[2] = o4[k];
+                    if (wc.on) warm_check(wc, d_scalars, bin_count, flags, (long long)o4[k]);
+                }
+        }
     }
 #pragma unroll
     for (int k = 0; k < 4; ++k) {
@@ -466,7 +496,9 @@
             else
                 PEM_S2_TILES("s2_tiles_kernel", false);
 #undef PEM_S2_TILES
-            PEM_TRY(exclusive_scan_i32(ctx, group_nnz, group_nnz, ngroups, ctx->d_scalars + 2));
+            const bool fold = p->warm_pass && decode && p->opt_s2_tail_fold && ngroups <= (size_t)S2_FOLD_GROUPS;
+            if (!fold) PEM_TRY(exclusive_scan_i32(ctx, group_nnz, group_nnz, ngroups, ctx->d_scalars + 2));
+            p->group_nnz_scanned = !fold;
             if (p->warm_pass) {
                 nnzc = p->w_nnz;
             } else {
@@ -493,9 +525,15 @@
                 p->flags_mirrored = true;
             }
             if (decode) {
-                PEM_LAUNCH(ctx, s2_offsets_kernel, grid_for(((ntc + S2_GROUP) / S2_GROUP) * 64, 256), 256, p->c_tile_cnt.as<uint16_t>(), (long long)ntc,
-                           group_nnz, p->c_tile_nnz_ptr.as<int>(), p->s3_chunk_tile.as<int>(), ctx->d_flags, wc,
-                           reinterpret_cast<const long long *>(ctx->d_scalars), p->bin_count.as<int>());
+#define PEM_S2_OFFSETS(NAME, FOLD)                                                                                                     \
+    PEM_LAUNCH_NAMED(ctx, NAME, (s2_offsets_kernel<FOLD>), grid_for(((ntc + S2_GROUP) / S2_GROUP) * 64, 256), 256, p->c_tile_cnt.as<uint16_t>(), \
+                     (long long)ntc, group_nnz, p->c_tile_nnz_ptr.as<int>(), p->s3_chunk_tile.as<int>(), ctx->d_flags, wc,              \
+                     reinterpret_cast<long long *>(ctx->d_scalars), p->bin_count.as<int>())
+                if (fold)
+                    PEM_S2_OFFSETS("s2_offsets_kernel<fold>", true);
+                else
+                    PEM_S2_OFFSETS("s2_offsets_kernel", false);
+#undef PEM_S2_OFFSETS
                 p->c_rowcolidx_valid = false;
             } else {
                 PEM_TRY(p->c_rowcolidx.reserve((size_t)nnzc + 16));
@@ -574,6 +612,10 @@
     PEM_ENTER(ctx);
     PEM_TRY(p->c_rowcolidx.reserve((size_t)p->nnz_c + 16));
     if (ntc > 0) {
+        if (!p->group_nnz_scanned) {
+            PEM_TRY(exclusive_scan_i32(ctx, p->group_nnz.as<int>(), p->group_nnz.as<int>(), (ntc + S2_GROUP - 1) / S2_GROUP, nullptr));
+            p->group_nnz_scanned = true;
+        }
         WarmCheck wc = {};
         PEM_LAUNCH(ctx, s2_entries_kernel, (unsigned)((ntc + S2_GROUP) / S2_GROUP), S2_GROUP, p->c_mask.as<uint32_t>(), (long long)ntc,
                    p->group_nnz.as<int>(), (long long)p->nnz_c, p->c_tile_nnz_ptr.as<int>(), p->c_rowcolidx.as<uint8_t>(), p->s3_chunk_tile.as<int>(),
```

After: 215.2, median of 6. +5.6%, better.
